# Kumar2421/scrfd_arcface_facerecognition

Hardware: AMD Instinct MI355X
Metric: faces/sec end-to-end (det+align+embed+match) (higher is better)
Workload: dtype f16; 1 GPU; BASELINE configs[1]: SCRFD-10G + ArcFace-R50, 64 synthetic 640x640 frames per GPU per step, F=1 face/frame (max_num), 1000-entry gallery, random-init weights (seed 0); frames_per_gpu=64, gallery=1000, kernel_plan=plans/mi355x.plan, rec_group=2

## Files before the change

scrfd_arcface_facerecognition_amd/csrc/conv.h:

```cpp
#pragma once
#include "common.h"

namespace fid {

enum : int { ACT_NONE = 0, ACT_RELU = 1, ACT_PRELU = 2 };
enum : int {
    CF_RES_UP2 = 1,
    CF_BORDER = 2,
    CF_OUT_F32 = 4,
    CF_ARGMAX = 8,
};

struct ConvArgs {
    const void *in;
    const void *w;
    const void *w_alt;
    const float *bias;
    const float *slope;
    const void *res;
    void *out;
    void *out2;
    float *partial;
    const void *in2;
    unsigned in2_bytes;
    int H2, W2, Cin2_p, T2, kw2, s2, nchunk2, krow;
    unsigned long long *amax;
    int amax_col0;
    int H, W, Cin_p, Ho, Wo, Cout_p, w_rows;
    int kh, kw, stride, pad;
    int M, T, nchunk, ksteps, ksplit, ksteps_per_split;
    int act, flags, nsig;
    int res_H, res_W, res_Cp;
    int tiles_m, tiles_n;
    int rev;
    int tm_fast;
    unsigned in_bytes, w_bytes;
};

struct ConvPlan {
    int bm, bn, bk, ksplit;
    int gen;
    int ns;
    size_t partial_bytes;
};
ConvPlan conv_plan(const ConvArgs &a, int num_cus, bool allow_split);
#include <vector>
std::vector<ConvPlan> conv_candidates(const ConvArgs &a, int num_cus, bool allow_split);
int conv_launch(fid_ctx *ctx, ConvArgs a, const ConvPlan &plan);
float conv_plan_cu_share(const ConvArgs &a, const ConvPlan &plan, int num_cus);
inline bool conv_walks_reverse(const ConvPlan &plan) { return plan.gen == 9; }
int plan_alt_kind(const ConvPlan &plan);
size_t repack_bytes(int kind, int Cout_p, int Cin_p, int taps = 9);
int repack_weights(fid_ctx *ctx, int kind, const void *src, void *dst, int Cout_p, int Cin_p, int taps = 9);

bool conv_direct_applicable(const ConvArgs &a);
int conv_direct_launch(fid_ctx *ctx, const ConvArgs &a);

bool conv_chunked_applicable(const ConvArgs &a);
int conv_chunked_launch(fid_ctx *ctx, const ConvArgs &a, int cb);

bool conv_pp_applicable(const ConvArgs &a);
int conv_pp_launch(fid_ctx *ctx, const ConvArgs &a, int cb);

bool conv_pc_applicable(const ConvArgs &a);
int conv_pc_launch(fid_ctx *ctx, const ConvArgs &a, int cb, int ring);

bool conv_pc2_applicable(const ConvArgs &a);
int conv_pc2_launch(fid_ctx *ctx, const ConvArgs &a);
bool conv_pcr_applicable(const ConvArgs &a);
int conv_pcr_launch(fid_ctx *ctx, const ConvArgs &a);

bool conv_wr_applicable(const ConvArgs &a);
bool conv_wr_resident_ok(const ConvArgs &a);
int conv_wr_launch(fid_ctx *ctx, const ConvArgs &a, int nt, int cb, int resident, int ring, bool strip = false);

bool mbf_block_applicable(int H, int W, int Cin_p, int Gp, int Cout_p, int stride, bool res);
int mbf_block_launch(fid_ctx *ctx, const void *x, const void *w1, const float *b1, const float *s1, int act1, const float *dww, const float *dwb,
                     const float *dws, int dw_act, const void *w2, const float *b2, const float *s2, int act2, bool res, void *out, int B, int H, int W,
                     int Cin_p, int Gp, int Cout_p, int stride);
bool conv_ks_applicable(const ConvArgs &a);
bool conv_ks_mosaic(const ConvArgs &a);
int conv_ks_launch(fid_ctx *ctx, const ConvArgs &a, int per_wg = 1, bool strip = false);
int conv_ks_items(const ConvArgs &a, bool strip = false);
bool conv_strip_ok(const ConvArgs &a);
int conv_strip_rows(const ConvArgs &a);
bool conv_ks_strip_applicable(const ConvArgs &a);

bool conv_s2_applicable(const ConvArgs &a);
int conv_s2_launch(fid_ctx *ctx, const ConvArgs &a);

bool conv_gw_applicable(const ConvArgs &a);
int conv_gw_launch(fid_ctx *ctx, const ConvArgs &a, int bm, int bn);

int conv_bb_launch(fid_ctx *ctx, const void *in, const void *w1, const float *b1, int ncls1, int act1, const float *s1, const void *w2, const float *b2,
                   void *out, int B, int H, int W, int act2, int rev, int Cp = 64);

bool dwpw_applicable(int Gp, int Cout_p);
int dwpw_launch(fid_ctx *ctx, const void *in, const float *dw_w, const float *dw_b, const float *dw_s, int dw_act, const void *pw_w, const float *pw_b,
                const float *pw_s, int pw_act, const void *res, void *out, int B, int H, int W, int Ho, int Wo, int Gp, int Cout_p, int stride);

bool stem_block_applicable(int H, int W);
int stem_block_launch(fid_ctx *ctx, const uint8_t *img, int B, int H, int W, const float *w0, const float *b0, const float *s0, int act0, const void *w1,
                      const float *b1, int ncls1, const float *s1, int act1, void *out, void *xe);

bool lat_fpn_applicable(int Cin_p, int H, int W, int rH, int rW, bool has_res);
int lat_fpn_launch(fid_ctx *ctx, const void *in, int B, int H, int W, int Cin_p, const void *w0, const float *b0, const void *res, int rH, int rW, const void *w1,
                   const float *b1, void *out, void *lat);
bool match_scan256_applicable(int n, int Gp, int dim, int num_cus);
int match_scan256_launch(fid_ctx *ctx, const void *q, const void *g, int n, int Gp, int dim, int col0, unsigned long long *amax);

int stem_fused_launch(fid_ctx *ctx, const uint8_t *img, int B, int H, int W, const void *w0, const float *b0, const void *w1,
                      const float *b1, const void *w2, const float *b2, void *out, int C2p);

int stem_rows_launch(fid_ctx *ctx, const uint8_t *img, int B, int H, int W, const void *w0, const float *b0, const void *w1,
                     const float *b1, const void *w2, const float *b2, void *out, int C2p);

}
```

scrfd_arcface_facerecognition_amd/csrc/conv_pc.hip:

```cpp
#include "epilogue.h"

namespace fid {
namespace {

typedef _Float16 half8 __attribute__((ext_vector_type(8)));
typedef float f32x4 __attribute__((ext_vector_type(4)));
typedef unsigned int u32x4 __attribute__((ext_vector_type(4)));

constexpr unsigned OOB = 0x7FFFFFF0u;
constexpr int TH = 16, TW = 16, PW = TW + 2, NPIX = (TH + 2) * PW;
constexpr int CK = 32;
constexpr int P_BLKS = 21, P_BYTES = P_BLKS * 1024;
constexpr int N_CONS = 8, N_PROD = 4;

__device__ __forceinline__ int swz64(int lin) { return (lin >> 1) & 3; }
__device__ __forceinline__ void raw_barrier() { asm volatile("s_barrier" ::: "memory"); }

struct PCArgs {
    const void *in;
    const void *w;
    const float *bias;
    const float *slope;
    const void *res;
    void *out;
    int H, W, Cin_p, Cout_p;
    int act, flags, res_Cp, nsig;
    int tiles_x, tiles_per_img, n_cblk, n_items, n_chunks;
    FastDiv d_cblk, d_tpi, d_tx;
    unsigned in_bytes, w_bytes;
    int ablate;
};

#ifdef FID_PC_STAMPS
constexpr int STAMP_STEPS = 16, STAMP_K = 6;
__device__ unsigned long long g_pc_stamps[3 * STAMP_STEPS * STAMP_K];
#define STAMP(who, k)                                                                                      \
    do {                                                                                                   \
        if (blockIdx.x == 0 && s < STAMP_STEPS && (wave <= N_CONS)) {                                                          \
            unsigned long long t_;                                                                         \
            __builtin_amdgcn_sched_barrier(0);                                                             \
            asm volatile("s_memtime %0\n\ts_waitcnt lgkmcnt(0)" : "=s"(t_)::"memory");                     \
            __builtin_amdgcn_sched_barrier(0);                                                             \
            if (lane == 0) g_pc_stamps[((who) * STAMP_STEPS + s) * STAMP_K + (k)] = t_;                     \
        }                                                                                                  \
    } while (0)
#else
#define STAMP(who, k)
#endif

template <int N>
__device__ __forceinline__ void wait_vmcnt_n() {
    asm volatile("s_waitcnt vmcnt(%0)" ::"n"(N) : "memory");
}

__device__ __forceinline__ void wait_vmcnt_dyn(int n) {
    switch (n) {
#define FID_W(k) case k: wait_vmcnt_n<k>(); break;
        FID_W(1) FID_W(2) FID_W(3) FID_W(4) FID_W(5) FID_W(6) FID_W(7) FID_W(8) FID_W(9) FID_W(10) FID_W(11) FID_W(12)
        FID_W(13) FID_W(14) FID_W(15) FID_W(16) FID_W(17) FID_W(18) FID_W(19) FID_W(20) FID_W(21) FID_W(22) FID_W(23) FID_W(24)
#undef FID_W
        default: wait_vmcnt_n<0>(); break;
    }
}

template <int NI, int WD, int PD, bool F32 = false, bool RS = false>
__global__ void __launch_bounds__((N_CONS + N_PROD) * 64, 3) conv3x3_pc(const PCArgs a) {
    constexpr int CB = 2 * NI * 16, MI = 4;
    constexpr int W_BLKS = 9 * CB * 64 / 1024, W_BYTES = W_BLKS * 1024;
    constexpr int AW = WD - 1, AP = PD - 1;
    static_assert(WD * W_BYTES + PD * P_BYTES <= 160 * 1024 && !(WD == 3 && PD == 3), "LDS budget");
    extern __shared__ __attribute__((aligned(16))) char smem[];
    char *sWr = smem, *sPr = smem + WD * W_BYTES;

    const int tid = threadIdx.x, lane = tid & 63, wave = __builtin_amdgcn_readfirstlane(tid >> 6);
    const int bid = (a.ablate & 256) ? (int)blockIdx.x : xcd_major_id(blockIdx.x, gridDim.x);
    const int my_items = bid < a.n_items ? (a.n_items - 1 - bid) / gridDim.x + 1 : 0;
    const int n_steps = my_items * a.n_chunks;
    if (n_steps == 0) return;

    auto decode_item = [&](int item, int &n, int &ty, int &tx, int &cb) {
        const int tile = fastdiv(item, a.d_cblk);
        cb = item - tile * a.n_cblk;
        n = fastdiv(tile, a.d_tpi);
        const int r = tile - n * a.tiles_per_img;
        ty = fastdiv(r, a.d_tx); tx = r - ty * a.tiles_x;
    };

    if (wave >= N_CONS) {
        const int pw = wave - N_CONS;
        __builtin_assume(pw >= 0 && pw < N_PROD);
        if (a.ablate & 512) __builtin_amdgcn_s_setprio(3);
        constexpr int MAX_W = (W_BLKS + N_PROD - 1) / N_PROD, MAX_P = (P_BLKS + N_PROD - 1) / N_PROD;
        const auto rs_in = __builtin_amdgcn_make_buffer_rsrc((void *)a.in, 0, a.in_bytes, 0x00020000);
        const auto rs_w = __builtin_amdgcn_make_buffer_rsrc((void *)a.w, 0, a.w_bytes, 0x00020000);
        int w_off[MAX_W];
#pragma unroll
        for (int k = 0; k < MAX_W; k++) {
            const int j = pw + N_PROD * k;
            const int row = j * 16 + (lane >> 2);
            const int t = row / CB, co = row - t * CB;
            w_off[k] = ((co * 9 + t) * a.Cin_p + ((lane & 3) ^ swz64(row)) * 8) * 2;
            if (a.ablate & 4) w_off[k] = j * 1024 + lane * 16;
        }
        constexpr bool KEEP_PK = NI <= 2 && !RS;
        auto patch_pk_calc = [&](int k) {
            int lo = lane;
            asm volatile("" : "+v"(lo));
            const int row = (pw + N_PROD * k) * 16 + (lo >> 2);
            int py = row / PW;
            const int px = row - py * PW;
            if (row >= NPIX) py = 255;
            return py | (px << 8) | ((((lo & 3) ^ swz64(row)) * 8) << 16);
        };
        int p_pk[KEEP_PK ? MAX_P : 1];
        if (KEEP_PK) {
#pragma unroll
            for (int k = 0; k < MAX_P; k++) p_pk[KEEP_PK ? k : 0] = patch_pk_calc(k);
        }
        auto patch_pk = [&](int k) {
            if (!KEEP_PK) return patch_pk_calc(k);
            int pk = p_pk[KEEP_PK ? k : 0];
            asm volatile("" : "+v"(pk));
            return pk;
        };
        const int my_p = (P_BLKS - pw + N_PROD - 1) / N_PROD;
        int p_off[MAX_P];
#pragma unroll
        for (int k = 0; k < (RS ? 0 : MAX_P); k++) {
            const int pk = patch_pk(k), py = pk & 255, px = (pk >> 8) & 255;
            p_off[k] = py == 255 ? -1 : ((py * a.W + px) * (a.Cin_p + ((a.ablate & 32) ? 32 : 0) + ((a.ablate & 64) ? 64 : 0)) + (pk >> 16)) * 2;
        }
        constexpr int OCPP = NI * 2, SK = OCPP, S_BLKS = N_CONS * SK, MAX_S = (S_BLKS + N_PROD - 1) / N_PROD;
        constexpr int OMASK = (OCPP & (OCPP - 1)) == 0 ? OCPP - 1 : 0;
        auto stage_pk_calc = [&](int k) {
            int lo = lane;
            asm volatile("" : "+v"(lo));
            const int b = pw + N_PROD * k, wv = b / SK;
            const int gl = (b - wv * SK) * 64 + lo;
            const int p = gl / OCPP, c = (gl - p * OCPP) ^ (p & OMASK);
            return p | (c << 8) | (wv << 16);
        };
        int s_pk[KEEP_PK ? MAX_S : 1];
        if (KEEP_PK) {
#pragma unroll
            for (int k = 0; k < MAX_S; k++) s_pk[KEEP_PK ? k : 0] = stage_pk_calc(k);
        }
        auto stage_pk = [&](int k) {
            if (!KEEP_PK) return stage_pk_calc(k);
            int pk = s_pk[KEEP_PK ? k : 0];
            asm volatile("" : "+v"(pk));
            return pk;
        };
        int s_off[MAX_S];
#pragma unroll
        for (int k = 0; k < MAX_S; k++) {
            const int pk = stage_pk(k), p = pk & 255, c = (pk >> 8) & 255, wv = pk >> 16;
            s_off[k] = ((((wv & 3) * MI + (p >> 4)) * a.W + (p & 15)) * a.Cout_p + (wv >> 2) * NI * 16 + c * 8) * 2;
        }
        u32x4 sv[MAX_S];
        auto read_tile = [&](char *slot) {
#pragma unroll
            for (int k = 0; k < MAX_S; k++)
                if (pw + N_PROD * k < S_BLKS) sv[k] = *(const u32x4 *)(slot + (pw + N_PROD * k) * 1024 + lane * 16);
            asm volatile("s_waitcnt lgkmcnt(0)" ::: "memory");
        };
        const bool has_res = a.res != nullptr;
        u32x4 rv[MAX_S];
        auto load_residual = [&](int item) {
            int n, ty, tx, cb;
            decode_item(item, n, ty, tx, cb);
            if (ty * TH + TH <= a.H && tx * TW + TW <= a.W && cb * CB + CB <= a.Cout_p) {
                const char *base = (const char *)a.res + ((((size_t)n * a.H + ty * TH) * a.W + tx * TW) * a.Cout_p + cb * CB) * 2;
#pragma unroll
                for (int k = 0; k < MAX_S; k++) rv[k] = *(const u32x4 *)(base + (unsigned)s_off[k]);
                return;
            }
#pragma unroll
            for (int k = 0; k < MAX_S; k++) {
                const int pk = stage_pk(k);
                const int p = pk & 255, c = (pk >> 8) & 255, wv = pk >> 16;
                const int oy = ty * TH + (wv & 3) * MI + (p >> 4), ox = tx * TW + (p & 15);
                const int co = cb * CB + (wv >> 2) * NI * 16 + c * 8;
                rv[k] = u32x4{0u, 0u, 0u, 0u};
                if (oy < a.H && ox < a.W && co < a.Cout_p)
                    rv[k] = *(const u32x4 *)((const char *)a.res + ((((size_t)n * a.H + oy) * a.W + ox) * a.Cout_p + co) * 2);
            }
        };
        auto write_residual = [&](char *slot) {
#pragma unroll
            for (int k = 0; k < MAX_S; k++) *(u32x4 *)(slot + (pw + N_PROD * k) * 1024 + lane * 16) = rv[k];
            asm volatile("s_waitcnt lgkmcnt(0)" ::: "memory");
        };
        static_assert(S_BLKS % N_PROD == 0, "every producer stores the same number of blocks");
        auto store_tile = [&](int item) {
            int n, ty, tx, cb;
            decode_item(item, n, ty, tx, cb);
            if (ty * TH + TH <= a.H && tx * TW + TW <= a.W && cb * CB + CB <= a.Cout_p) {
                char *base = (char *)a.out + ((((size_t)n * a.H + ty * TH) * a.W + tx * TW) * a.Cout_p + cb * CB) * 2;
#pragma unroll
                for (int k = 0; k < MAX_S; k++)
                    if (pw + N_PROD * k < S_BLKS) *(u32x4 *)(base + (unsigned)s_off[k]) = sv[k];
                return true;
            }
#pragma unroll
            for (int k = 0; k < MAX_S; k++) {
                if (pw + N_PROD * k >= S_BLKS) continue;
                const int pk = stage_pk(k);
                const int p = pk & 255, c = (pk >> 8) & 255, wv = pk >> 16;
                const int oy = ty * TH + (wv & 3) * MI + (p >> 4), ox = tx * TW + (p & 15);
                const int co = cb * CB + (wv >> 2) * NI * 16 + c * 8;
                if (oy < a.H && ox < a.W && co < a.Cout_p)
                    *(u32x4 *)((char *)a.out + ((((size_t)n * a.H + oy) * a.W + ox) * a.Cout_p + co) * 2) = sv[k];
            }
            return false;
        };
        struct Cursor {
            int item, ck;
            int w_base;
            int n, y0, x0;
        };
        auto cursor_decode = [&](Cursor &c) {
            int n, ty, tx, cb;
            decode_item(c.item, n, ty, tx, cb);
            c.w_base = cb * CB * 9 * a.Cin_p * 2;
            c.n = (a.ablate & 8) ? 0 : n; c.y0 = ty * TH - 1; c.x0 = tx * TW - 1;
        };
        auto cursor_next = [&](Cursor &c) {
            if (++c.ck == a.n_chunks) {
                c.ck = 0;
                c.item += gridDim.x;
                cursor_decode(c);
            }
        };
        auto issue_weights = [&](const Cursor &c, int slot) {
            if (a.ablate & 1) return;
            const int ubase = (a.ablate & 4) ? c.ck * W_BYTES : c.w_base + c.ck * CK * 2;
            char *dst = sWr + slot * W_BYTES;
#pragma unroll
            for (int k = 0; k < MAX_W; k++) {
                const int j = pw + N_PROD * k;
                if (j < W_BLKS)
                    __builtin_amdgcn_raw_ptr_buffer_load_lds(rs_w, (__attribute__((address_space(3))) void *)(dst + j * 1024), 16,
                                                             (unsigned)(w_off[k] + ubase), 0, 0, 0);
            }
        };
        auto issue_patch = [&](const Cursor &c, int slot) {
            if (a.ablate & 2) return;
            const int c0 = c.ck * CK;
            char *dst = sPr + slot * P_BYTES;
            if ((a.ablate & 16) || (c.y0 >= 0 && c.x0 >= 0 && c.y0 + TH + 2 <= a.H && c.x0 + TW + 2 <= a.W)) {
                const int base = (((c.n * a.H + c.y0) * a.W + c.x0) * a.Cin_p + c0) * 2;
#pragma unroll
                for (int k = 0; k < MAX_P; k++) {
                    const int j = pw + N_PROD * k;
                    if (j >= P_BLKS) continue;
                    const unsigned vo = p_off[k] < 0 ? OOB : (unsigned)(p_off[k] + base);
                    __builtin_amdgcn_raw_ptr_buffer_load_lds(rs_in, (__attribute__((address_space(3))) void *)(dst + j * 1024), 16, vo, 0, 0, 0);
                }
                return;
            }
#pragma unroll
            for (int k = 0; k < MAX_P; k++) {
                const int j = pw + N_PROD * k;
                if (j >= P_BLKS) continue;
                const int pk = patch_pk(k);
                const int py = pk & 255, iy = c.y0 + py, ix = c.x0 + ((pk >> 8) & 255);
                const bool in = py != 255 && (unsigned)iy < (unsigned)a.H && (unsigned)ix < (unsigned)a.W;
                const unsigned vo = in ? (unsigned)((((c.n * a.H + iy) * a.W + ix) * a.Cin_p + c0 + (pk >> 16)) * 2) : OOB;
                __builtin_amdgcn_raw_ptr_buffer_load_lds(rs_in, (__attribute__((address_space(3))) void *)(dst + j * 1024), 16, vo, 0, 0, 0);
            }
        };

        u32x4 wreg[RS ? MAX_W : 1], preg[RS ? MAX_P : 1];
        auto load_weights = [&](const Cursor &c) {
            if (a.ablate & 1) return;
            const int ubase = c.w_base + c.ck * CK * 2;
#pragma unroll
            for (int k = 0; k < MAX_W; k++)
                if (pw + N_PROD * k < W_BLKS) wreg[RS ? k : 0] = __builtin_amdgcn_raw_buffer_load_b128(rs_w, (unsigned)(w_off[k] + ubase), 0, 0);
        };
        auto load_patch = [&](const Cursor &c) {
            if (a.ablate & 2) return;
            const int c0 = c.ck * CK;
            if (c.y0 >= 0 && c.x0 >= 0 && c.y0 + TH + 2 <= a.H && c.x0 + TW + 2 <= a.W) {
                const int base = (((c.n * a.H + c.y0) * a.W + c.x0) * a.Cin_p + c0) * 2;
#pragma unroll
                for (int k = 0; k < MAX_P; k++) {
                    if (pw + N_PROD * k >= P_BLKS) continue;
                    const int pk = patch_pk(k), py = pk & 255;
                    const unsigned vo = py == 255 ? OOB : (unsigned)(((py * a.W + ((pk >> 8) & 255)) * a.Cin_p + (pk >> 16)) * 2 + base);
                    preg[RS ? k : 0] = __builtin_amdgcn_raw_buffer_load_b128(rs_in, vo, 0, 0);
                }
                return;
            }
#pragma unroll
            for (int k = 0; k < MAX_P; k++) {
                if (pw + N_PROD * k >= P_BLKS) continue;
                const int pk = patch_pk(k);
                const int py = pk & 255, iy = c.y0 + py, ix = c.x0 + ((pk >> 8) & 255);
                const bool in = py != 255 && (unsigned)iy < (unsigned)a.H && (unsigned)ix < (unsigned)a.W;
                const unsigned vo = in ? (unsigned)((((c.n * a.H + iy) * a.W + ix) * a.Cin_p + c0 + (pk >> 16)) * 2) : OOB;
                preg[RS ? k : 0] = __builtin_amdgcn_raw_buffer_load_b128(rs_in, vo, 0, 0);
            }
        };
        auto commit_weights = [&](int slot) {
            char *dst = sWr + slot * W_BYTES + lane * 16;
#pragma unroll
            for (int k = 0; k < MAX_W; k++)
                if (pw + N_PROD * k < W_BLKS) *(u32x4 *)(dst + (pw + N_PROD * k) * 1024) = wreg[RS ? k : 0];
        };
        auto commit_patch = [&](int slot) {
            char *dst = sPr + slot * P_BYTES + lane * 16;
#pragma unroll
            for (int k = 0; k < MAX_P; k++)
                if (pw + N_PROD * k < P_BLKS) *(u32x4 *)(dst + (pw + N_PROD * k) * 1024) = preg[RS ? k : 0];
        };
        auto lds_done = [&]() { asm volatile("s_waitcnt lgkmcnt(0)" ::: "memory"); };

        const int my_w = (W_BLKS - pw + N_PROD - 1) / N_PROD;
        Cursor cw, cp;
        cw.item = bid; cw.ck = 0;
        cursor_decode(cw);
        cp = cw;
        if constexpr (RS) {
            auto fetch = [&](bool w, int wslot, bool p_, int pslot) {
                if (p_) { load_patch(cp); cursor_next(cp); }
                if (w) { load_weights(cw); cursor_next(cw); }
                if (w) commit_weights(wslot);
                if (p_) commit_patch(pslot);
            };
            fetch(true, 0, true, 0);
            if (n_steps > 1) fetch(AW == 2, 1, AP == 2, 1);
            lds_done();
            int ck = 0, item = bid;
            for (int s = 0; s < n_steps; s++) {
                STAMP(0, 0);
                STAMP(0, 1);
                raw_barrier();
                STAMP(0, 2);
                if (!F32 && ck == 0 && s > 0) {
                    char *stage = sWr + ((s + WD - 1) % WD) * W_BYTES;
                    if (has_res) {
                        write_residual(stage);
                        raw_barrier();
                    }
                    raw_barrier();
                    read_tile(stage);
                    store_tile(item - gridDim.x);
                }
                STAMP(0, 3);
                fetch(s + AW < n_steps, (s + AW) % WD, s + AP < n_steps, (s + AP) % PD);
                if (has_res && ck == a.n_chunks - 1) load_residual(item);
                lds_done();
                STAMP(0, 4);
                if (++ck == a.n_chunks) { ck = 0; item += gridDim.x; }
            }
            if (F32) return;
            raw_barrier();
            if (has_res) {
                write_residual(sWr + ((n_steps - 1) % WD) * W_BYTES);
                raw_barrier();
            }
            raw_barrier();
            read_tile(sWr + ((n_steps - 1) % WD) * W_BYTES);
            store_tile(item - gridDim.x);
            return;
        }
        issue_weights(cw, 0);
        issue_patch(cp, 0);
        cursor_next(cw);
        cursor_next(cp);
        int young = 0;
        if (n_steps > 1) {
            if (AP == 2) { issue_patch(cp, 1); cursor_next(cp); young = my_p; }
            if (AW == 2) { issue_weights(cw, 1); cursor_next(cw); young = my_w; }
        }
        int ck = 0, item = bid;
        for (int s = 0; s < n_steps; s++) {
            STAMP(0, 0);
            wait_vmcnt_dyn(young);
            STAMP(0, 1);
            raw_barrier();
            STAMP(0, 2);
            const bool flush = !F32 && ck == 0 && s > 0;
            const bool have_w = s + AW < n_steps, have_p = s + AP < n_steps;
            char *stage = sWr + ((s + WD - 1) % WD) * W_BYTES;
            young = 0;
            if (flush) {
                if (has_res) {
                    write_residual(stage);
                    raw_barrier();
                }
                if (have_p) issue_patch(cp, (s + AP) % PD);
                raw_barrier();
                read_tile(stage);
                if (have_w) issue_weights(cw, (s + AW) % WD);
                const bool all_stores = store_tile(item - gridDim.x);
                if (all_stores) young = MAX_S + ((AW == 2 && have_w) ? my_w : 0);
            } else {
                if (AW == 2) {
                    if (have_p) issue_patch(cp, (s + AP) % PD);
                    if (have_w) { issue_weights(cw, (s + AW) % WD); young = my_w; }
                } else {
                    if (have_w) issue_weights(cw, (s + AW) % WD);
                    if (have_p) { issue_patch(cp, (s + AP) % PD); young = AP == 2 ? my_p : 0; }
                }
            }
            if (has_res && ck == a.n_chunks - 1) {
                load_residual(item);
                young = 0;
            }
            STAMP(0, 3);
            if (have_w && s + AW + 1 < n_steps) cursor_next(cw);
            if (have_p && s + AP + 1 < n_steps) cursor_next(cp);
            STAMP(0, 4);
            if (++ck == a.n_chunks) { ck = 0; item += gridDim.x; }
        }
        if (F32) return;
        raw_barrier();
        if (has_res) {
            wait_vmcnt_n<0>();
            write_residual(sWr + ((n_steps - 1) % WD) * W_BYTES);
            raw_barrier();
        }
        raw_barrier();
        read_tile(sWr + ((n_steps - 1) % WD) * W_BYTES);
        store_tile(item - gridDim.x);
        return;
    }

    const int grp = wave >> 2, wg = wave & 3;
    const int frow = lane & 15, fq = lane >> 4;
    const int lin0 = (wg * MI) * PW + frow;
    EpiArgs ep{a.bias, a.slope, a.res, a.out, a.Cout_p, a.H, a.W, a.act, a.flags, 0, a.H, a.W, a.res_Cp};

    constexpr int OROWB = NI * 32, OCPP = NI * 2;
    constexpr int OMASK = (OCPP & (OCPP - 1)) == 0 ? OCPP - 1 : 0;
    static_assert(F32 || N_CONS * 64 * OROWB <= W_BYTES, "staging must fit a weight slot");
    EpiPix px[MI];
    int co0[NI];
    EpiRegs<NI, MI> R;
    ep_half4 hv[NI][MI];
    int bias_cb = -1;
    auto epi_prefetch = [&](int item) {
        int n, ty, tx, cb;
        decode_item(item, n, ty, tx, cb);
        int lo = lane;
        asm volatile("" : "+v"(lo));
        const int frow = lo & 15, fq = lo >> 4;
        const int co_w = cb * CB + grp * NI * 16;
        if (a.flags & CF_BORDER) {
#pragma unroll
            for (int mi = 0; mi < MI; mi++) {
                const int oy = ty * TH + wg * MI + mi, ox = tx * TW + frow;
                px[mi].valid = oy < a.H && ox < a.W;
                px[mi].n = n; px[mi].oy = oy; px[mi].ox = ox;
                px[mi].m = px[mi].valid ? ((long long)n * a.H + oy) * a.W + ox : 0;
            }
        }
#pragma unroll
        for (int ni = 0; ni < NI; ni++) co0[ni] = co_w + ni * 16 + fq * 4;
        if (cb != bias_cb) {
            bias_cb = cb;
#pragma unroll
            for (int ni = 0; ni < NI; ni++) {
                const int c = co0[ni] < a.Cout_p ? co0[ni] : 0;
                R.bb[ni] = (a.bias != nullptr && !(a.flags & CF_BORDER)) ? *(const ep_f32x4 *)(a.bias + c) : ep_f32x4{0.f, 0.f, 0.f, 0.f};
                if (a.act == ACT_PRELU) R.sl[ni] = *(const ep_f32x4 *)(a.slope + c);
            }
        }
    };
    f32x4 acc[NI][MI];
    const bool has_res = a.res != nullptr;
    auto epi_residual_values = [&](char *slot) {
        int lo = lane;
        asm volatile("" : "+v"(lo));
        const int frow = lo & 15, fq = lo >> 4;
        const char *sS = slot + wave * (64 * OROWB);
#pragma unroll
        for (int mi = 0; mi < MI; mi++)
#pragma unroll
            for (int ni = 0; ni < NI; ni++) {
                const int p = mi * 16 + frow, c = ni * 2 + (fq >> 1);
                R.rr[ni][mi] = *(const ep_half4 *)(sS + p * OROWB + ((c ^ (p & OMASK)) << 4) + (fq & 1) * 8);
            }
        epilogue_values_fast<NI, MI>(ep, acc, px, co0, R, hv);
    };
    auto epi_stage = [&](char *slot) {
        int lo = lane;
        asm volatile("" : "+v"(lo));
        const int frow = lo & 15, fq = lo >> 4;
        char *sS = slot + wave * (64 * OROWB);
#pragma unroll
        for (int mi = 0; mi < MI; mi++)
#pragma unroll
            for (int ni = 0; ni < NI; ni++) {
                const int p = mi * 16 + frow, c = ni * 2 + (fq >> 1);
                *(ep_half4 *)(sS + p * OROWB + ((c ^ (p & OMASK)) << 4) + (fq & 1) * 8) = hv[ni][mi];
            }
        asm volatile("s_waitcnt lgkmcnt(0)" ::: "memory");
    };

    int li = 0, ck = 0;
    for (int s = 0; s < n_steps; s++) {
        const int item = bid + li * gridDim.x;
        [[maybe_unused]] const int who = wave == 0 ? 1 : 2;
        if (wave == 0 || wave == 7) STAMP(who, 0);
        raw_barrier();
        if (wave == 0 || wave == 7) STAMP(who, 1);
        if (!F32 && ck == 0 && s > 0) {
            char *slot = sWr + ((s + WD - 1) % WD) * W_BYTES;
            if (has_res) {
                raw_barrier();
                epi_residual_values(slot);
            }
            epi_stage(slot);
            raw_barrier();
        }
        if (wave == 0 || wave == 7) STAMP(who, 2);
        const bool last_chunk = ck == a.n_chunks - 1;
        if (last_chunk && !F32) epi_prefetch(item);
        if (wave == 0 || wave == 7) STAMP(who, 3);
        if (ck == 0) {
#pragma unroll
            for (int ni = 0; ni < NI; ni++)
#pragma unroll
                for (int mi = 0; mi < MI; mi++) acc[ni][mi] = f32x4{0.f, 0.f, 0.f, 0.f};
        }
        const char *sW = sWr + (s % WD) * W_BYTES, *sP = sPr + (s % PD) * P_BYTES;
        {
            int plin = lin0, wlane = ((grp * NI) * 16 + frow) * 64 + ((fq ^ swz64(frow)) << 4);
            asm volatile("" : "+v"(plin), "+v"(wlane));
            half8 wq[3][NI], pq[3];
            auto load_w = [&](int dy, int dx) {
#pragma unroll
                for (int ni = 0; ni < NI; ni++) wq[dy][ni] = *(const half8 *)(sW + wlane + ((dy * 3 + dx) * CB + ni * 16) * 64);
            };
            auto load_p = [&](int q, int set) {
                const int lin = plin + (q % 6) * PW + q / 6;
                pq[set] = *(const half8 *)(sP + lin * 64 + ((fq ^ swz64(lin)) << 4));
            };
            load_w(0, 0); load_p(0, 0); load_w(1, 0); load_p(1, 1); load_w(2, 0);
#pragma unroll
            for (int q = 0; q < 18; q++) {
                const int dx = q / 6, r = q % 6;
                if (q + 2 < 18) load_p(q + 2, (q + 2) % 3);
                __builtin_amdgcn_sched_barrier(0);
#pragma unroll
                for (int dy = 0; dy < 3; dy++) {
                    const int mi = r - dy;
                    if (mi < 0 || mi >= MI) continue;
#pragma unroll
                    for (int ni = 0; ni < NI; ni++)
                        acc[ni][mi] = __builtin_amdgcn_mfma_f32_16x16x32_f16(wq[dy][ni], pq[q % 3], acc[ni][mi], 0, 0, 0);
                }
                __builtin_amdgcn_sched_barrier(0);
                if (dx < 2 && r >= 3) load_w(r - 3, dx + 1);
            }
        }
        if (wave == 0 || wave == 7) STAMP(who, 4);
        if (F32) {
            if (last_chunk) {
                int n, ty, tx, cb;
                decode_item(item, n, ty, tx, cb);
                int lo = lane;
                asm volatile("" : "+v"(lo));
                const int frow = lo & 15, fq = lo >> 4;
#pragma unroll
                for (int ni = 0; ni < NI; ni++) {
                    const int co = cb * CB + (grp * NI + ni) * 16 + fq * 4;
                    const f32x4 b = (a.bias != nullptr && co < a.Cout_p) ? *(const f32x4 *)(a.bias + co) : f32x4{0.f, 0.f, 0.f, 0.f};
#pragma unroll
                    for (int mi = 0; mi < MI; mi++) {
                        f32x4 v = acc[ni][mi] + b;
                        if (co < a.nsig) {
#pragma unroll
                            for (int i = 0; i < 4; i++)
                                if (co + i < a.nsig) v[i] = 1.f / (1.f + expf(-v[i]));
                        }
                        const int oy = ty * TH + wg * MI + mi, ox = tx * TW + frow;
                        if (oy < a.H && ox < a.W && co < a.Cout_p)
                            *(f32x4 *)((float *)a.out + (((size_t)n * a.H + oy) * a.W + ox) * a.Cout_p + co) = v;
                    }
                }
            }
        } else if (last_chunk && !has_res) epilogue_values_fast<NI, MI>(ep, acc, px, co0, R, hv);
        if (wave == 0 || wave == 7) STAMP(who, 5);
        if (++ck == a.n_chunks) { ck = 0; li++; }
    }
    if (F32) return;
    raw_barrier();
    if (has_res) {
        raw_barrier();
        epi_residual_values(sWr + ((n_steps - 1) % WD) * W_BYTES);
    }
    epi_stage(sWr + ((n_steps - 1) % WD) * W_BYTES);
    raw_barrier();
}

template <int NI, int WD, int PD, bool F32 = false, bool RS = false>
int launch_pc(fid_ctx *ctx, const PCArgs &a) {
    constexpr size_t lds = (size_t)WD * 9 * 2 * NI * 16 * 64 + (size_t)PD * P_BYTES;
    FID_TRY(ensure_dyn_lds(ctx, (const void *)conv3x3_pc<NI, WD, PD, F32, RS>, (int)((int)lds)));
    const int grid = std::min(a.n_items, ctx->num_cus);
    hipLaunchKernelGGL((conv3x3_pc<NI, WD, PD, F32, RS>), dim3(grid), dim3((N_CONS + N_PROD) * 64), lds, ctx->stream, a);
    FID_HIP(hipGetLastError());
#ifdef FID_PC_STAMPS
    if (const char *e = getenv("FID_PC_STAMP_DUMP")) {
        static int countdown = atoi(e);
        if (--countdown == 0) {
            FID_HIP(hipStreamSynchronize(ctx->stream));
            static unsigned long long h[3 * STAMP_STEPS * STAMP_K];
            FID_HIP(hipMemcpyFromSymbol(h, HIP_SYMBOL(g_pc_stamps), sizeof(h)));
            const int steps = std::min(STAMP_STEPS, ((a.n_items - 1) / grid + 1) * a.n_chunks);
            fprintf(stderr, "[pc-stamps] NI=%d H=%d W=%d Cin_p=%d Cout_p=%d items=%d chunks=%d\n", NI, a.H, a.W, a.Cin_p, a.Cout_p, a.n_items, a.n_chunks);
            const unsigned long long t0 = h[0];
            for (int s = 0; s < steps; s++) {
                const unsigned long long *p = h + s * STAMP_K, *c0 = h + (STAMP_STEPS + s) * STAMP_K, *c7 = h + (2 * STAMP_STEPS + s) * STAMP_K;
                fprintf(stderr, "[pc-stamps] step %2d | producer: +%6lld wait %5lld barrier %5lld issue %5lld next %4lld | cons0: arrive +%6lld barrier %5lld flush %5lld pref %5lld mfma %5lld values %5lld | cons7: arrive +%6lld barrier %5lld mfma %5lld\n",
                        s, (long long)(p[0] - t0), (long long)(p[1] - p[0]), (long long)(p[2] - p[1]), (long long)(p[3] - p[2]), (long long)(p[4] - p[3]),
                        (long long)(c0[0] - t0), (long long)(c0[1] - c0[0]), (long long)(c0[2] - c0[1]), (long long)(c0[3] - c0[2]), (long long)(c0[4] - c0[3]), (long long)(c0[5] - c0[4]),
                        (long long)(c7[0] - t0), (long long)(c7[1] - c7[0]), (long long)(c7[4] - c7[3]));
            }
        }
    }
#endif
    return FID_OK;
}

}

bool conv_pc_applicable(const ConvArgs &a) {
    if (getenv("FID_NO_PC")) return false;
    const bool shape = a.kh == 3 && a.kw == 3 && a.stride == 1 && a.pad == 1 && a.Cin_p % 32 == 0 && a.Cin_p >= 64 &&
                       a.w_rows == a.Cout_p && a.H == a.Ho && a.W == a.Wo && a.H >= 12 && a.W >= 12 && !(a.flags & (CF_RES_UP2 | CF_ARGMAX));
    if (!shape) return false;
    if (a.flags & CF_OUT_F32)
        return a.Cout_p == 32 && a.act == ACT_NONE && a.res == nullptr && !(a.flags & CF_BORDER);
    return a.Cout_p >= 64 && a.nsig == 0 && (a.res == nullptr || (a.res_H == a.Ho && a.res_W == a.Wo));
}

int conv_pc_launch(fid_ctx *ctx, const ConvArgs &c, int cb, int ring) {
    PCArgs a{};
    a.in = c.in; a.w = c.w; a.bias = c.bias; a.slope = c.slope; a.res = c.res; a.out = c.out;
    a.H = c.H; a.W = c.W; a.Cin_p = c.Cin_p; a.Cout_p = c.Cout_p;
    a.act = c.act; a.flags = c.flags; a.res_Cp = c.res_Cp; a.nsig = c.nsig;
    const int B = c.M / (c.Ho * c.Wo);
    a.tiles_x = cdiv(c.W, TW);
    a.tiles_per_img = a.tiles_x * cdiv(c.H, TH);
    a.n_cblk = cdiv(c.Cout_p, cb);
    a.n_items = B * a.tiles_per_img * a.n_cblk;
    a.n_chunks = c.Cin_p / CK;
    a.d_cblk = fastdiv_make(a.n_cblk); a.d_tpi = fastdiv_make(a.tiles_per_img); a.d_tx = fastdiv_make(a.tiles_x);
    a.in_bytes = c.in_bytes;
    a.w_bytes = (unsigned)std::min<size_t>(c.w_bytes, (size_t)c.w_rows * 9 * c.Cin_p * 2);
    if (const char *e = getenv("FID_PC_ABLATE")) a.ablate = atoi(e);
    FID_REQUIRE(a.in_bytes <= OOB && a.w_bytes <= OOB, "conv: tensor larger than 2 GiB");
    const bool dma = getenv("FID_PC_RS") == nullptr;
    if (cb == 32) return dma ? launch_pc<1, 2, 3, true>(ctx, a) : launch_pc<1, 2, 3, true, true>(ctx, a);
    if (cb == 64 && ring == 1) return launch_pc<2, 3, 2>(ctx, a);
    if (cb == 64) return dma ? launch_pc<2, 2, 3>(ctx, a) : launch_pc<2, 2, 3, false, true>(ctx, a);
    if (cb == 96) return launch_pc<3, 2, 2>(ctx, a);
    set_error("producer/consumer conv: cb=%d unsupported", cb);
    return FID_E_INVALID;
}

}
```

scrfd_arcface_facerecognition_amd/csrc/net.h:

```cpp
#pragma once
#include "conv.h"

namespace fid {

enum : int { OP_STEM = 1, OP_CONV = 2, OP_MAXPOOL = 3, OP_DWCONV = 4, OP_STEMFUSED = 5, OP_BBLOCK = 6, OP_DWPW = 7, OP_MBBLOCK = 8, OP_STEMBLOCK = 9, OP_LATFPN = 10 };

enum : int {
    W_TYPE = 0,
    W_SRC = 1,
    W_DST = 2,
    W_RES = 3,
    W_KH = 4,
    W_KW = 5,
    W_STRIDE = 6,
    W_PAD = 7,
    W_CIN = 8,
    W_COUT = 9,
    W_ACT = 10,
    W_FLAGS = 11,
    W_NSIG = 12,
    W_WOFF = 13,
    W_WBYTES = 14,
    W_BOFF = 15,
    W_SOFF = 16,
    W_WROWS = 17,
    W_GROUPS = 18,
    W_F_W0 = 20, W_F_B0 = 21, W_F_W1 = 22, W_F_B1 = 23, W_F_W2 = 24, W_F_B2 = 25,
    W_F_MACS_LO = 26, W_F_MACS_HI = 27,
    W_B_W1 = 20, W_B_B1 = 21, W_B_W2 = 22, W_B_B2 = 23, W_B_S1 = 24, W_B_ACT1 = 25,
    W_D_WOFF = 20, W_D_BOFF = 21, W_D_SOFF = 22, W_D_ACT = 23,
    W_M_W1 = 20, W_M_B1 = 21, W_M_S1 = 22, W_M_ACT1 = 23, W_M_DW = 24, W_M_DWB = 25, W_M_DWS = 28, W_M_DWACT = 29, W_M_GP = 30,
    W_S_W1 = 20, W_S_B1 = 21, W_S_S1 = 22, W_S_ACT0 = 23, W_S_DST2 = 24,
    W_L_W0 = 20, W_L_B0 = 21, W_L_LAT = 22,
    W_X_DST2 = 20, W_X_ACT2 = 21, W_X_COUT1P = 22,
    W_X_SRC2 = 23, W_X_T2 = 24, W_X_KW2 = 25, W_X_S2 = 28,
    W_X_W2OFF = 29, W_X_B2OFF = 30, W_X_SCOP = 31,
};

enum : int { T_C = 0, T_CP = 1, T_H = 2, T_W = 3, T_DTYPE = 4, T_SLOT = 5, T_FLAGS = 6 };

}
```

scrfd_arcface_facerecognition_amd/csrc/net.hip:

```cpp
#include "net.h"

#include <map>
#include <set>

struct fid_net {
    int n_ops = 0, n_tensors = 0, in_h = 0, in_w = 0, max_batch = 0;
    std::vector<int32_t> ops, tensors;
    void *blob = nullptr;
    size_t blob_bytes = 0;
    std::vector<void *> slots;
    std::vector<size_t> slot_bytes_per_image;
    double macs_per_image = 0;
    int sub_batch = 0;
    std::vector<std::map<int, fid::ConvPlan>> tuned;
    std::vector<char> tdir;
    int alternate = 1;
    std::vector<std::set<int>> plan_ok;
    int autotune = 1;
    bool tuned_now = false;
    size_t partial_cap = 0;
    hipEvent_t *prof_events = nullptr;
    int n_prof_events = 0;
    struct Replay { hipGraphExec_t exec = nullptr; int seen = 0; unsigned long long last_use = 0; const void *partial = nullptr; };
    std::map<std::pair<const void *, int>, Replay> replays;
    unsigned long long run_counter = 0;
    int graphs = 0;
    unsigned long long table_hash = 0;
    std::string device_key, plan_path;
    std::map<std::pair<int, int>, void *> alt_w;
};

namespace fid {
namespace {

typedef _Float16 half8 __attribute__((ext_vector_type(8)));

template <int CPW, int SPLIT = 4>
__global__ void __launch_bounds__(256) stem_conv3x3(const uint8_t *__restrict__ img, const float *__restrict__ w,
                                                    const float *__restrict__ bias, const float *__restrict__ slope,
                                                    _Float16 *__restrict__ out, int H, int W, int Ho, int Wo, int Cout_p,
                                                    int stride, int act, long long total_pix) {
    const int wv = __builtin_amdgcn_readfirstlane(threadIdx.x >> 6);
    const long long pix = ((long long)blockIdx.x * (4 / SPLIT) + wv / SPLIT) * 64 + (threadIdx.x & 63);
    const int cg = wv % SPLIT;
    if (pix >= total_pix) return;
    const int hw = Ho * Wo;
    const int n = (int)(pix / hw);
    const int r = (int)(pix - (long long)n * hw);
    const int oy = r / Wo, ox = r - oy * Wo;
    const int iy0 = oy * stride - 1, ix0 = ox * stride - 1;
    float x[27];
    const uint8_t *base = img + (size_t)n * H * W * 3;
#pragma unroll
    for (int dy = 0; dy < 3; dy++) {
#pragma unroll
        for (int dx = 0; dx < 3; dx++) {
            const int iy = iy0 + dy, ix = ix0 + dx;
            const bool in = (unsigned)iy < (unsigned)H && (unsigned)ix < (unsigned)W;
            const uint8_t *p = base + ((size_t)(in ? iy : 0) * W + (in ? ix : 0)) * 3;
#pragma unroll
            for (int c = 0; c < 3; c++) x[(dy * 3 + dx) * 3 + c] = in ? (float)(2 * (int)p[c] - 255) : 0.f;
        }
    }
    _Float16 res[CPW];
#pragma unroll
    for (int c = 0; c < CPW; c++) {
        const int co = cg * CPW + c;
        const float *wr = w + co * 27;
        float acc = bias[co];
#pragma unroll
        for (int k = 0; k < 27; k++) acc = fmaf(x[k], wr[k], acc);
        if (act == ACT_RELU) acc = fmaxf(acc, 0.f);
        else if (act == ACT_PRELU) acc = acc > 0.f ? acc : acc * slope[co];
        res[c] = (_Float16)acc;
    }
    _Float16 *o = out + (size_t)pix * Cout_p + cg * CPW;
#pragma unroll
    for (int c = 0; c < CPW; c += 8) *(half8 *)(o + c) = *(half8 *)(res + c);
}

typedef _Float16 sm_half8 __attribute__((ext_vector_type(8)));
typedef _Float16 sm_half4 __attribute__((ext_vector_type(4)));
typedef float sm_f32x4 __attribute__((ext_vector_type(4)));
typedef unsigned int sm_u32x4 __attribute__((ext_vector_type(4)));

template <int NI, int STRIDE>
__global__ void __launch_bounds__(256) stem_conv_mfma(const uint8_t *__restrict__ img, const float *__restrict__ w,
                                                      const float *__restrict__ bias, const float *__restrict__ slope,
                                                      _Float16 *__restrict__ out, int H, int W, int Ho, int Wo, int act,
                                                      int tiles_x, int tiles_y, int n_tiles, int ablate) {
    constexpr int CP = NI * 16, TS = 16;
    constexpr int PR = (TS - 1) * STRIDE + 3;
    constexpr int ND = (PR * 3 + 1 + 3) / 4;
    constexpr int RSH = ND * 4;
    constexpr int OROWB = CP * 2, CPP = OROWB / 16;
    __shared__ __attribute__((aligned(16))) _Float16 sIn[PR * RSH + 8];
    __shared__ __attribute__((aligned(16))) _Float16 sWt[CP * 32];
    __shared__ __attribute__((aligned(16))) char sSt[4 * 4 * TS * OROWB];
    const int tid = threadIdx.x, lane = tid & 63, wave = __builtin_amdgcn_readfirstlane(tid >> 6);
    const int frow = lane & 15, fq = lane >> 4;

    for (int i = tid; i < CP * 32; i += 256) {
        const int co = i >> 5, k = i & 31;
        sWt[i] = k < 27 ? (_Float16)w[co * 27 + k] : (_Float16)0.f;
    }
    if (tid < 8) sIn[PR * RSH + tid] = (_Float16)0.f;
    __syncthreads();
    sm_half8 wf[NI];
    sm_f32x4 bv[NI], sl[NI];
#pragma unroll
    for (int ni = 0; ni < NI; ni++) {
        wf[ni] = *(const sm_half8 *)(sWt + (ni * 16 + frow) * 32 + fq * 8);
        bv[ni] = bias ? *(const sm_f32x4 *)(bias + ni * 16 + fq * 4) : sm_f32x4{0.f, 0.f, 0.f, 0.f};
        sl[ni] = act == ACT_PRELU ? *(const sm_f32x4 *)(slope + ni * 16 + fq * 4) : sm_f32x4{1.f, 1.f, 1.f, 1.f};
    }
    int koff[8];
#pragma unroll
    for (int j = 0; j < 8; j++) {
        const int k = fq * 8 + j, dy = k / 9, rem = k - dy * 9;
        koff[j] = k < 27 ? dy * RSH + rem : -1;
    }
    const int tiles_per_img = tiles_x * tiles_y, rowbytes = W * 3;
    for (int tile = blockIdx.x; tile < n_tiles; tile += gridDim.x) {
        const int n = tile / tiles_per_img, r = tile - n * tiles_per_img;
        const int ty = r / tiles_x, tx = r - ty * tiles_x;
        const int iy0 = ty * TS * STRIDE - 1, ix0 = tx * TS * STRIDE - 1;
        const int bx0 = ix0 * 3 - 1;
        const uint8_t *base = img + (size_t)n * H * rowbytes;
        const int elo = 1 + 3 * max(0, -ix0), ehi = 1 + 3 * min(PR, W - ix0);
        for (int d = tid; d < PR * ND; d += 256) {
            const int pr = d / ND, dc = d - pr * ND;
            const int iy = iy0 + pr, bx = bx0 + dc * 4;
            const bool rin = (unsigned)iy < (unsigned)H;
            unsigned v4 = 0u;
            if (rin && bx >= 0 && bx + 4 <= rowbytes && !(ablate & 2)) v4 = *(const unsigned *)(base + (size_t)iy * rowbytes + bx);
            sm_half4 h;
#pragma unroll
            for (int j = 0; j < 4; j++) {
                const int e = dc * 4 + j, v = (v4 >> (8 * j)) & 0xFF;
                h[j] = (rin && e >= elo && e < ehi) ? (_Float16)(float)(2 * v - 255) : (_Float16)0.f;
            }
            *(sm_half4 *)(sIn + pr * RSH + dc * 4) = h;
        }
        __syncthreads();
        char *sS = sSt + wave * (4 * TS * OROWB);
        sm_half8 pf[4];
#pragma unroll
        for (int rr = 0; rr < 4; rr++) {
            const int pbase = ((wave * 4 + rr) * STRIDE) * RSH + 1 + frow * STRIDE * 3;
#pragma unroll
            for (int j = 0; j < 8; j++) pf[rr][j] = sIn[koff[j] >= 0 ? pbase + koff[j] : PR * RSH];
        }
#pragma unroll
        for (int rr = 0; rr < 4; rr++) {
#pragma unroll
            for (int ni = 0; ni < NI; ni++) {
                sm_f32x4 acc = {0.f, 0.f, 0.f, 0.f};
                acc = __builtin_amdgcn_mfma_f32_16x16x32_f16(wf[ni], pf[rr], acc, 0, 0, 0);
                sm_f32x4 v = acc + bv[ni];
                if (act == ACT_RELU) {
#pragma unroll
                    for (int i = 0; i < 4; i++) v[i] = fmaxf(v[i], 0.f);
                } else if (act == ACT_PRELU) {
#pragma unroll
                    for (int i = 0; i < 4; i++) v[i] = v[i] > 0.f ? v[i] : v[i] * sl[ni][i];
                }
                const int ch = ni * 2 + (fq >> 1);
                *(sm_half4 *)(sS + (rr * TS + frow) * OROWB + (((ch + frow) % CPP) << 4) + (fq & 1) * 8) = __builtin_convertvector(v, sm_half4);
            }
        }
        asm volatile("s_waitcnt lgkmcnt(0)" ::: "memory");
#pragma unroll
        for (int g = lane; g < 4 * TS * CPP; g += 64) {
            const int p = g / CPP, c = g - p * CPP;
            const sm_u32x4 o = *(const sm_u32x4 *)(sS + p * OROWB + (((c + (p & 15)) % CPP) << 4));
            const int oy = ty * TS + wave * 4 + (p >> 4), ox = tx * TS + (p & 15);
            if (oy < Ho && ox < Wo && !(ablate & 1)) *(sm_u32x4 *)((char *)out + (((size_t)n * Ho + oy) * Wo + ox) * OROWB + c * 16) = o;
        }
        __syncthreads();
    }
}

__global__ void __launch_bounds__(256) maxpool_nhwc(const _Float16 *__restrict__ in, _Float16 *__restrict__ out, int H, int W,
                                                    int Ho, int Wo, int Cp, int k, int stride, int pad, long long total) {
    const long long idx = (long long)blockIdx.x * blockDim.x + threadIdx.x;
    if (idx >= total) return;
    const int c8 = Cp >> 3;
    const int cg = (int)(idx % c8);
    const long long pix = idx / c8;
    const int hw = Ho * Wo;
    const int n = (int)(pix / hw);
    const int r = (int)(pix - (long long)n * hw);
    const int oy = r / Wo, ox = r - oy * Wo;
    half8 m;
#pragma unroll
    for (int i = 0; i < 8; i++) m[i] = (_Float16)(-65504.f);
    for (int dy = 0; dy < k; dy++) {
        const int iy = oy * stride - pad + dy;
        if ((unsigned)iy >= (unsigned)H) continue;
        for (int dx = 0; dx < k; dx++) {
            const int ix = ox * stride - pad + dx;
            if ((unsigned)ix >= (unsigned)W) continue;
            const half8 v = *(const half8 *)(in + ((size_t)(n * H + iy) * W + ix) * Cp + cg * 8);
#pragma unroll
            for (int i = 0; i < 8; i++) m[i] = v[i] > m[i] ? v[i] : m[i];
        }
    }
    *(half8 *)(out + (size_t)pix * Cp + cg * 8) = m;
}

__global__ void __launch_bounds__(256) dwconv_nhwc(const _Float16 *__restrict__ in, const float *__restrict__ w,
                                                   const float *__restrict__ bias, const float *__restrict__ slope,
                                                   _Float16 *__restrict__ out, int H, int W, int Ho, int Wo, int Cp, int k,
                                                   int stride, int pad, int act, long long total) {
    const long long idx = (long long)blockIdx.x * blockDim.x + threadIdx.x;
    if (idx >= total) return;
    const int c8 = Cp >> 3;
    const int cg = (int)(idx % c8);
    const long long pix = idx / c8;
    const int hw = Ho * Wo;
    const int n = (int)(pix / hw);
    const int r = (int)(pix - (long long)n * hw);
    const int oy = r / Wo, ox = r - oy * Wo;
    float acc[8];
#pragma unroll
    for (int i = 0; i < 8; i++) acc[i] = bias[cg * 8 + i];
    for (int dy = 0; dy < k; dy++) {
        const int iy = oy * stride - pad + dy;
        if ((unsigned)iy >= (unsigned)H) continue;
        for (int dx = 0; dx < k; dx++) {
            const int ix = ox * stride - pad + dx;
            if ((unsigned)ix >= (unsigned)W) continue;
            const half8 v = *(const half8 *)(in + ((size_t)(n * H + iy) * W + ix) * Cp + cg * 8);
            const float *wr = w + (size_t)(dy * k + dx) * Cp + cg * 8;
#pragma unroll
            for (int i = 0; i < 8; i++) acc[i] = fmaf((float)v[i], wr[i], acc[i]);
        }
    }
    half8 o;
#pragma unroll
    for (int i = 0; i < 8; i++) {
        float a = acc[i];
        if (act == ACT_RELU) a = fmaxf(a, 0.f);
        else if (act == ACT_PRELU) a = a > 0.f ? a : a * slope[cg * 8 + i];
        o[i] = (_Float16)a;
    }
    *(half8 *)(out + (size_t)pix * Cp + cg * 8) = o;
}

constexpr int DW_TR = 14, DW_TC = 16, DW_PR = DW_TR + 2, DW_PC = DW_TC + 2;
__global__ void __launch_bounds__(256) dwconv3x3_lds(const _Float16 *__restrict__ in, const float *__restrict__ w, const float *__restrict__ bias,
                                                     const float *__restrict__ slope, _Float16 *__restrict__ out, int H, int W, int Cp, int act,
                                                     int tiles_x, int tiles_y, int cblks) {
    __shared__ __attribute__((aligned(16))) char sP[DW_PR * DW_PC * 128];
    const int tid = threadIdx.x;
    int item = blockIdx.x;
    const int cb = item % cblks; item /= cblks;
    const int tx = item % tiles_x; item /= tiles_x;
    const int ty = item % tiles_y, n = item / tiles_y;
    const int y0 = ty * DW_TR - 1, x0 = tx * DW_TC - 1, c0 = cb * 64;
    for (int i = tid; i < DW_PR * DW_PC * 8; i += 256) {
        const int p = i >> 3, c = i & 7;
        const int py = p / DW_PC, px = p - py * DW_PC;
        const int iy = y0 + py, ix = x0 + px;
        if ((unsigned)iy < (unsigned)H && (unsigned)ix < (unsigned)W)
            *(uint4 *)(sP + p * 128 + c * 16) = *(const uint4 *)(in + ((size_t)(n * H + iy) * W + ix) * Cp + c0 + c * 8);
    }
    const int cg = tid & 7, col = (tid >> 3) & 15, rh = tid >> 7;
    float wv[9][8], bv[8], sv[8];
#pragma unroll
    for (int t = 0; t < 9; t++)
#pragma unroll
        for (int i = 0; i < 8; i++) wv[t][i] = w[(size_t)t * Cp + c0 + cg * 8 + i];
#pragma unroll
    for (int i = 0; i < 8; i++) {
        bv[i] = bias[c0 + cg * 8 + i];
        sv[i] = act == ACT_PRELU ? slope[c0 + cg * 8 + i] : 1.f;
    }
    __syncthreads();
    const int ox = tx * DW_TC + col;
    const bool okc[3] = {(unsigned)(ox - 1) < (unsigned)W, ox < W, (unsigned)(ox + 1) < (unsigned)W};
    if (ox >= W) return;
    half8 win[3][3];
    const char *base = sP + col * 128 + cg * 16;
    auto load_row = [&](int pr, int slot) {
#pragma unroll
        for (int dx = 0; dx < 3; dx++) win[slot][dx] = *(const half8 *)(base + (pr * DW_PC + dx) * 128);
    };
    const int r0 = rh * (DW_TR / 2);
    load_row(r0, 0); load_row(r0 + 1, 1);
#pragma unroll
    for (int r = 0; r < DW_TR / 2; r++) {
        load_row(r0 + r + 2, (r + 2) % 3);
        const int oy = ty * DW_TR + r0 + r;
        if (oy >= H) break;
        float acc[8];
#pragma unroll
        for (int i = 0; i < 8; i++) acc[i] = bv[i];
#pragma unroll
        for (int dy = 0; dy < 3; dy++) {
            if ((unsigned)(oy - 1 + dy) >= (unsigned)H) continue;
#pragma unroll
            for (int dx = 0; dx < 3; dx++) {
                if (!okc[dx]) continue;
                const half8 v = win[(r + dy) % 3][dx];
#pragma unroll
                for (int i = 0; i < 8; i++) acc[i] = fmaf((float)v[i], wv[dy * 3 + dx][i], acc[i]);
            }
        }
        half8 o;
#pragma unroll
        for (int i = 0; i < 8; i++) {
            float a = acc[i];
            if (act == ACT_RELU) a = fmaxf(a, 0.f);
            else if (act == ACT_PRELU) a = a > 0.f ? a : a * sv[i];
            o[i] = (_Float16)a;
        }
        *(half8 *)(out + ((size_t)(n * H + oy) * W + ox) * Cp + c0 + cg * 8) = o;
    }
}

__global__ void __launch_bounds__(256) gdc_rows(const _Float16 *__restrict__ in, const float *__restrict__ w, const float *__restrict__ bias,
                                                const float *__restrict__ slope, _Float16 *__restrict__ out, int k, int Cp, int act, int total) {
    const int idx = blockIdx.x * blockDim.x + threadIdx.x;
    const int g = idx >> 3, r = idx & 7;
    const int c8 = Cp >> 3;
    const bool live = g < total;
    const int n = live ? g / c8 : 0, cg = live ? g - n * c8 : 0;
    float acc[8];
#pragma unroll
    for (int i = 0; i < 8; i++) acc[i] = 0.f;
    if (live && r < k) {
        for (int dx = 0; dx < k; dx++) {
            const half8 v = *(const half8 *)(in + ((size_t)(n * k + r) * k + dx) * Cp + cg * 8);
            const float *wr = w + (size_t)(r * k + dx) * Cp + cg * 8;
#pragma unroll
            for (int i = 0; i < 8; i++) acc[i] = fmaf((float)v[i], wr[i], acc[i]);
        }
    }
    float sum[8];
#pragma unroll
    for (int i = 0; i < 8; i++) sum[i] = live ? bias[cg * 8 + i] : 0.f;
    for (int rr = 0; rr < k; rr++)
#pragma unroll
        for (int i = 0; i < 8; i++) sum[i] += __shfl(acc[i], (threadIdx.x & 63 & ~7) + rr, 64);
    if (live && r == 0) {
        half8 o;
#pragma unroll
        for (int i = 0; i < 8; i++) {
            float a = sum[i];
            if (act == ACT_RELU) a = fmaxf(a, 0.f);
            else if (act == ACT_PRELU) a = a > 0.f ? a : a * slope[cg * 8 + i];
            o[i] = (_Float16)a;
        }
        *(half8 *)(out + (size_t)n * Cp + cg * 8) = o;
    }
}

__global__ void __launch_bounds__(256) touch_kernel(const uint4 *__restrict__ p, size_t n16, unsigned *sink) {
    unsigned acc = 0;
    for (size_t i = (size_t)blockIdx.x * 256 + threadIdx.x; i < n16; i += (size_t)gridDim.x * 256) {
        const uint4 v = p[i];
        acc ^= v.x ^ v.y ^ v.z ^ v.w;
    }
    if (acc == 0x9E3779B9u && sink) *sink = acc;
}

struct TensorView {
    void *ptr;
    int C, Cp, H, W, dtype;
};

TensorView view(const fid_net *net, int id, int first = 0) {
    const int32_t *t = &net->tensors[(size_t)id * FID_TENSOR_WORDS];
    const size_t per_image = (size_t)t[T_H] * t[T_W] * t[T_CP] * (t[T_DTYPE] == 1 ? 4 : 2);
    return TensorView{(char *)net->slots[t[T_SLOT]] + per_image * first, t[T_C], t[T_CP], t[T_H], t[T_W], t[T_DTYPE]};
}

constexpr int FID_PLAN_REV = 5;

unsigned long long fnv1a(const void *p, size_t n, unsigned long long h = 1469598103934665603ull) {
    const unsigned char *b = (const unsigned char *)p;
    for (size_t i = 0; i < n; i++) { h ^= b[i]; h *= 1099511628211ull; }
    return h;
}

void plan_line(const fid_net *net, int oi, int batch, const ConvPlan &c, char *buf, size_t cap) {
    snprintf(buf, cap, "%s|%016llx|%d|%d|%d %d %d %d %d %d %zu\n", net->device_key.c_str(), net->table_hash, oi, batch, c.gen, c.bm, c.bn,
             c.bk, c.ksplit, c.ns, c.partial_bytes);
}

int plan_load(fid_net *net, const char *path, int *n_loaded) {
    FILE *f = fopen(path, "r");
    int n = 0;
    if (f) {
        char line[512];
        while (fgets(line, sizeof(line), f)) {
            char dev[256];
            unsigned long long h = 0;
            int oi = 0, batch = 0;
            ConvPlan c{};
            if (sscanf(line, "%255[^|]|%llx|%d|%d|%d %d %d %d %d %d %zu", dev, &h, &oi, &batch, &c.gen, &c.bm, &c.bn, &c.bk, &c.ksplit, &c.ns,
                       &c.partial_bytes) != 11)
                continue;
            if (h != net->table_hash || net->device_key != dev || oi < 0 || oi >= net->n_ops || batch <= 0) continue;
            net->tuned[oi][batch] = c;
            net->plan_ok[oi].erase(batch);
            n++;
        }
        fclose(f);
    }
    if (n_loaded) *n_loaded = n;
    return FID_OK;
}

bool same_kernel(const ConvPlan &x, const ConvPlan &y) {
    return x.gen == y.gen && x.bm == y.bm && x.bn == y.bn && x.bk == y.bk && x.ksplit == y.ksplit && x.ns == y.ns;
}

void drop_unused_alt_weights(fid_ctx *ctx, fid_net *net, int oi) {
    bool used[4] = {false, false, false, false};
    for (const auto &kv : net->tuned[oi]) used[plan_alt_kind(kv.second) & 3] = true;
    bool synced = false;
    for (auto it = net->alt_w.begin(); it != net->alt_w.end();) {
        if (it->first.first == oi && !used[it->first.second & 3]) {
            if (!synced) { (void)hipStreamSynchronize(ctx->stream); synced = true; }
            (void)hipFree(it->second);
            it = net->alt_w.erase(it);
        } else ++it;
    }
}

int set_alt_weights(fid_ctx *ctx, fid_net *net, int oi, ConvArgs &a, const ConvPlan &plan) {
    const int kind = plan_alt_kind(plan);
    a.w_alt = nullptr;
    if (kind == 0) return FID_OK;
    auto key = std::make_pair(oi, kind);
    auto it = net->alt_w.find(key);
    if (it == net->alt_w.end()) {
        void *p = nullptr;
        FID_HIP(hipMalloc(&p, repack_bytes(kind, a.w_rows, a.Cin_p, a.kh * a.kw) + 256));
        const int rc = repack_weights(ctx, kind, a.w, p, a.w_rows, a.Cin_p, a.kh * a.kw);
        if (rc != FID_OK) { (void)hipFree(p); return rc; }
        it = net->alt_w.emplace(key, p).first;
    }
    a.w_alt = it->second;
    return FID_OK;
}

int run_op(fid_ctx *ctx, fid_net *net, int oi, const uint8_t *images, int first, int batch, void *partial_ws) {
    const int32_t *op = &net->ops[(size_t)oi * FID_OP_WORDS];
    const char *blob = (const char *)net->blob;
    static const bool klog = getenv("FID_KLOG") != nullptr;
    if (klog) fprintf(stderr, "[klog] op %d\n", oi);
    const TensorView dst = view(net, op[W_DST], first);
    images += (size_t)first * net->in_h * net->in_w * 3;
    const float *bias = op[W_BOFF] >= 0 ? (const float *)(blob + op[W_BOFF]) : nullptr;
    const float *slope = op[W_SOFF] >= 0 ? (const float *)(blob + op[W_SOFF]) : nullptr;
    if (op[W_TYPE] != OP_CONV && op[W_TYPE] != OP_BBLOCK) net->tdir[op[W_DST]] = 0;
    switch (op[W_TYPE]) {
        case OP_STEM: {
            const long long total = (long long)batch * dst.H * dst.W;
            const int cpw = dst.Cp / 4;
            const float *w = (const float *)(blob + op[W_WOFF]);
            dim3 grid((unsigned)cdiv64(total, 64));
            static const bool valu = getenv("FID_STEM_VALU") != nullptr;
            const int st = op[W_STRIDE];
            if (!valu && net->in_w % 4 == 0 && (st == 1 || st == 2) && (dst.Cp == 16 || dst.Cp == 32 || dst.Cp == 64 || dst.Cp == 128)) {
                const int tx = cdiv(dst.W, 16), ty = cdiv(dst.H, 16), nt = batch * tx * ty;
                static const int abl = getenv("FID_STEMM_ABLATE") ? atoi(getenv("FID_STEMM_ABLATE")) : 0;
                const int g = std::min(nt, ctx->num_cus * (dst.Cp == 128 ? 2 : (dst.Cp == 64 ? 3 : 4)));
#define STEMM(NI, ST) hipLaunchKernelGGL((stem_conv_mfma<NI, ST>), dim3(g), dim3(256), 0, ctx->stream, images, w, bias, slope, (_Float16 *)dst.ptr, net->in_h, net->in_w, dst.H, dst.W, op[W_ACT], tx, ty, nt, abl)
                if (dst.Cp == 128) { if (st == 1) STEMM(8, 1); else STEMM(8, 2); }
                else if (dst.Cp == 64) { if (st == 1) STEMM(4, 1); else STEMM(4, 2); }
                else if (dst.Cp == 32) { if (st == 1) STEMM(2, 1); else STEMM(2, 2); }
                else { if (st == 1) STEMM(1, 1); else STEMM(1, 2); }
#undef STEMM
                break;
            }
            static const int split = getenv("FID_STEM_SPLIT") ? atoi(getenv("FID_STEM_SPLIT")) : 2;
#define STEM(CPW) hipLaunchKernelGGL(stem_conv3x3<CPW>, grid, dim3(256), 0, ctx->stream, images, w, bias, slope, (_Float16 *)dst.ptr, net->in_h, net->in_w, dst.H, dst.W, dst.Cp, op[W_STRIDE], op[W_ACT], total)
#define STEMS(CPW, SP) hipLaunchKernelGGL((stem_conv3x3<CPW, SP>), dim3((unsigned)cdiv64(total, 64 * (4 / SP))), dim3(256), 0, ctx->stream, images, w, bias, slope, (_Float16 *)dst.ptr, net->in_h, net->in_w, dst.H, dst.W, dst.Cp, op[W_STRIDE], op[W_ACT], total)
            if (split == 1 && dst.Cp == 64) STEMS(64, 1);
            else if (split == 2 && dst.Cp == 64) STEMS(32, 2);
            else if (split == 1 && dst.Cp == 32) STEMS(32, 1);
            else if (cpw == 8) STEM(8);
            else if (cpw == 16) STEM(16);
            else if (cpw == 32) STEM(32);
            else { set_error("stem: Cout_p=%d unsupported", dst.Cp); return FID_E_INVALID; }
#undef STEM
#undef STEMS
            break;
        }
        case OP_CONV: {
            if (op[W_X_SRC2] == 0 && op[W_X_W2OFF] > 0) {
                const int cons = op[W_X_W2OFF] - 1;
                auto itc = net->tuned[cons].find(batch);
                if (itc != net->tuned[cons].end() && itc->second.gen == 12 && net->plan_ok[cons].count(batch)) break;
            }
            const TensorView src = view(net, op[W_SRC], first);
            ConvArgs a{}, af{};
            bool has_sc = false;
            a.in = src.ptr;
            a.w = blob + op[W_WOFF];
            a.bias = bias;
            a.slope = slope;
            a.out = dst.ptr;
            if (op[W_X_DST2] > 0) {
                const TensorView d2 = view(net, op[W_X_DST2] - 1, first);
                FID_REQUIRE(d2.H == dst.H && d2.W == dst.W && d2.Cp == dst.Cp && d2.dtype == dst.dtype && op[W_X_ACT2] == ACT_NONE &&
                            op[W_X_COUT1P] == dst.Cp, "op %d: bad fused shortcut record", oi);
                a.out2 = d2.ptr;
            }
            a.H = src.H; a.W = src.W; a.Cin_p = src.Cp;
            a.Ho = dst.H; a.Wo = dst.W; a.Cout_p = dst.Cp;
            a.w_rows = op[W_WROWS];
            a.kh = op[W_KH]; a.kw = op[W_KW]; a.stride = op[W_STRIDE]; a.pad = op[W_PAD];
            a.M = batch * dst.H * dst.W;
            a.act = op[W_ACT]; a.flags = op[W_FLAGS]; a.nsig = op[W_NSIG];
            if (dst.dtype == 1) a.flags |= CF_OUT_F32;
            if (op[W_RES] >= 0) {
                const TensorView r = view(net, op[W_RES], first);
                a.res = r.ptr; a.res_H = r.H; a.res_W = r.W; a.res_Cp = r.Cp;
            }
            a.in_bytes = (unsigned)((size_t)batch * src.H * src.W * src.Cp * 2);
            a.w_bytes = (unsigned)op[W_WBYTES];
            if (op[W_X_SRC2] > 0) {
                const TensorView x2 = view(net, op[W_X_SRC2] - 1, first);
                FID_REQUIRE(x2.dtype == 0 && op[W_X_T2] >= 1 && op[W_X_KW2] >= 1 && op[W_X_S2] >= 1 && op[W_X_DST2] == 0 &&
                            (dst.H - 1) * op[W_X_S2] + (op[W_X_T2] / op[W_X_KW2] - 1) < x2.H && (dst.W - 1) * op[W_X_S2] + op[W_X_KW2] - 1 < x2.W,
                            "op %d: bad fused shortcut-conv record", oi);
                FID_REQUIRE(op[W_X_W2OFF] > 0 && op[W_X_B2OFF] > 0 && op[W_X_SCOP] > 0 && op[W_X_SCOP] <= oi && op[W_RES] >= 0, "op %d: fused shortcut-conv record without its second image", oi);
                af = a;
                af.in2 = x2.ptr; af.H2 = x2.H; af.W2 = x2.W; af.Cin2_p = x2.Cp; af.T2 = op[W_X_T2]; af.kw2 = op[W_X_KW2]; af.s2 = op[W_X_S2];
                af.in2_bytes = (unsigned)((size_t)batch * x2.H * x2.W * x2.Cp * 2);
                af.w = blob + op[W_X_W2OFF];
                af.bias = (const float *)(blob + op[W_X_B2OFF]);
                af.w_bytes = (unsigned)((size_t)op[W_WROWS] * (op[W_KH] * op[W_KW] * src.Cp + op[W_X_T2] * x2.Cp) * 2);
                af.res = nullptr;
                has_sc = true;
            }
            a.partial = af.partial = (float *)partial_ws;
            a.rev = af.rev = net->alternate && op[W_SRC] >= 0 && !net->tdir[op[W_SRC]];
            auto all_candidates = [&]() {
                std::vector<ConvPlan> v = conv_candidates(a, ctx->num_cus, true);
                static const bool no_sc = getenv("FID_NO_SC_RUNTIME") != nullptr;
                if (has_sc && !no_sc)
                    for (ConvPlan c : conv_candidates(af, ctx->num_cus, true)) { c.gen = 12; v.push_back(c); }
                return v;
            };
            auto launch_plan = [&](const ConvPlan &c) -> int {
                if (c.gen != 12) return conv_launch(ctx, a, c);
                ConvPlan c2 = c;
                c2.gen = c.ns == 10 ? 10 : 2;
                af.w_alt = a.w_alt;
                return conv_launch(ctx, af, c2);
            };
            ConvPlan plan;
            auto &cache = net->tuned[oi];
            auto it = cache.find(batch);
            if (it != cache.end() && !net->plan_ok[oi].count(batch)) {
                bool ok = false;
                for (const ConvPlan &c : all_candidates())
                    if (same_kernel(c, it->second) && c.partial_bytes <= net->partial_cap && (c.ksplit == 1 || partial_ws)) { it->second = c; ok = true; break; }
                if (!ok && it->second.ksplit == 1) {
                    const ConvPlan h = conv_plan(a, ctx->num_cus, false);
                    if (same_kernel(h, it->second)) { it->second = h; ok = true; }
                }
                if (ok) net->plan_ok[oi].insert(batch);
                else { cache.erase(it); it = cache.end(); }
            }
            if (it != cache.end()) {
                plan = it->second;
            } else if (net->autotune && partial_ws) {
                std::vector<ConvPlan> cands = all_candidates();
                if (const char *fg = getenv("FID_FORCE_GEN")) {
                    std::vector<ConvPlan> only;
                    for (const ConvPlan &c : cands)
                        if (c.gen == atoi(fg)) only.push_back(c);
                    if (!only.empty()) cands = only;
                }
                if (const char *fn = getenv("FID_FORCE_NS")) {
                    std::vector<ConvPlan> only;
                    for (const ConvPlan &c : cands)
                        if (((c.gen == 2 || c.gen == 5 || c.gen == 12) && c.ns == atoi(fn)) || (c.gen == 9 && (c.ns == 1 ? 3 : (c.ns == 4 ? 4 : (c.ns == 6 ? (c.bm == 512 ? 7 : 6) : (c.ns >= 7 ? c.ns + 1 + (c.ns == 8 && c.bm == 512 ? 20 : 0) + (c.ns == 8 && c.bm == 256 && c.bn == 128 ? 30 : 0) : c.bm / 256)))) == atoi(fn))) only.push_back(c);
                    if (!only.empty()) cands = only;
                }
                const float pc2_bias = getenv("FID_PC2_BIAS") ? (float)atof(getenv("FID_PC2_BIAS")) : 1.f;
                hipEvent_t e0, e1;
                FID_HIP(hipEventCreate(&e0));
                FID_HIP(hipEventCreate(&e1));
                static const bool cold_tune = !getenv("FID_TUNE_HOT");
                void *flush = nullptr;
                constexpr size_t FLUSH_BYTES = 320ull << 20;
                if (cold_tune) { FID_TRY(get_scratch(ctx, 4, FLUSH_BYTES, &flush)); net->tuned_now = true; }
                float best = 1e30f;
                if (cands.empty()) { set_error("op %d: no kernel candidate", oi); return FID_E_STATE; }
                plan = cands[0];
                float t_sc = 0.f;
                if (has_sc) {
                    t_sc = 1e30f;
                    for (int rep = 0; rep < 4; rep++) {
                        if (flush) {
                            FID_HIP(hipMemsetAsync(flush, rep & 1, FLUSH_BYTES, ctx->stream));
                            if (af.in2_bytes <= (128u << 20))
                                hipLaunchKernelGGL(touch_kernel, dim3(ctx->num_cus * 4), dim3(256), 0, ctx->stream, (const uint4 *)af.in2, (size_t)af.in2_bytes / 16, (unsigned *)nullptr);
                        }
                        FID_HIP(hipEventRecord(e0, ctx->stream));
                        FID_TRY(run_op(ctx, net, op[W_X_SCOP] - 1, images - (size_t)first * net->in_h * net->in_w * 3, first, batch, partial_ws));
                        FID_HIP(hipEventRecord(e1, ctx->stream));
                        FID_HIP(hipEventSynchronize(e1));
                        float ms = 0;
                        FID_HIP(hipEventElapsedTime(&ms, e0, e1));
                        if (rep > 0 || !flush) t_sc = std::min(t_sc, ms);
                    }
                }
                for (const ConvPlan &c : cands) {
                    if (c.partial_bytes > net->partial_cap) continue;
                    float tmin = 1e30f;
                    static const int tune_reps = getenv("FID_TUNE_REPS") ? std::max(2, atoi(getenv("FID_TUNE_REPS"))) : 5;
                    for (int rep = 0; rep < tune_reps; rep++) {
                        FID_TRY(set_alt_weights(ctx, net, oi, a, c));
                        if (flush) {
                            FID_HIP(hipMemsetAsync(flush, rep & 1, FLUSH_BYTES, ctx->stream));
                            if (a.in_bytes <= (128u << 20))
                                hipLaunchKernelGGL(touch_kernel, dim3(ctx->num_cus * 4), dim3(256), 0, ctx->stream, (const uint4 *)a.in, (size_t)a.in_bytes / 16, (unsigned *)nullptr);
                        }
                        FID_HIP(hipEventRecord(e0, ctx->stream));
                        FID_TRY(launch_plan(c));
                        FID_HIP(hipEventRecord(e1, ctx->stream));
                        FID_HIP(hipEventSynchronize(e1));
                        float ms = 0;
                        FID_HIP(hipEventElapsedTime(&ms, e0, e1));
                        if (rep > 0) tmin = std::min(tmin, ms);
                    }
                    float score = c.ksplit > 1 ? tmin * 1.1f : tmin;
                    if (has_sc && c.gen != 12) score += t_sc;
                    static const float tune_share = getenv("FID_TUNE_SHARE") ? (float)atof(getenv("FID_TUNE_SHARE")) : 0.f;
                    if (tune_share > 0.f) score *= 1.f - tune_share * (1.f - conv_plan_cu_share(a, c, ctx->num_cus));
                    if (c.gen == 8) score *= pc2_bias;
                    static const int tune_verbose = getenv("FID_TUNE_LOG") ? atoi(getenv("FID_TUNE_LOG")) : 0;
                    if (tune_verbose >= 2)
                        fprintf(stderr, "[cand] op %d gen %d tile %dx%dx%d ns %d split %d: %.1f us\n", oi, c.gen, c.bm, c.bn, c.bk, c.ns, c.ksplit, tmin * 1e3f);
                    if (score < best) { best = score; plan = c; }
                }
                (void)hipEventDestroy(e0);
                (void)hipEventDestroy(e1);
                cache[batch] = plan;
                net->plan_ok[oi].insert(batch);
                drop_unused_alt_weights(ctx, net, oi);
                if (!net->plan_path.empty()) {
                    if (FILE *pf = fopen(net->plan_path.c_str(), "a")) {
                        char line[512];
                        plan_line(net, oi, batch, plan, line, sizeof(line));
                        fputs(line, pf);
                        fclose(pf);
                    }
                }
                if (getenv("FID_TUNE_LOG"))
                    fprintf(stderr, "[tune] op %d M=%d Cin_p=%d Cout_p=%d k=%d s=%d -> gen %d tile %dx%dx%d ns %d split %d (%.1f us)\n", oi, a.M,
                            a.Cin_p, a.Cout_p, a.kh, a.stride, plan.gen, plan.bm, plan.bn, plan.bk, plan.ns, plan.ksplit, best * 1e3f);
            } else {
                plan = conv_direct_applicable(a) ? ConvPlan{} : conv_plan(a, ctx->num_cus, partial_ws != nullptr);
                if (conv_direct_applicable(a)) { plan.gen = 0; plan.ksplit = 1; }
            }
            FID_TRY(set_alt_weights(ctx, net, oi, a, plan));
            FID_TRY(launch_plan(plan));
            net->tdir[op[W_DST]] = (char)(a.rev && conv_walks_reverse(plan));
            if (op[W_X_DST2] > 0) net->tdir[op[W_X_DST2] - 1] = net->tdir[op[W_DST]];
            break;
        }
        case OP_STEMFUSED: {
            const bool old_stem = getenv("FID_STEM_OLD") != nullptr;
            FID_TRY((old_stem ? stem_fused_launch : stem_rows_launch)(ctx, images, batch, net->in_h, net->in_w, blob + op[W_F_W0], (const float *)(blob + op[W_F_B0]),
                                      blob + op[W_F_W1], (const float *)(blob + op[W_F_B1]), blob + op[W_F_W2],
                                      (const float *)(blob + op[W_F_B2]), dst.ptr, dst.Cp));
            break;
        }
        case OP_STEMBLOCK: {
            FID_REQUIRE(dst.Cp == 64 && dst.dtype == 0 && dst.H == net->in_h && dst.W == net->in_w && stem_block_applicable(dst.H, dst.W), "op %d: bad fused stem-block record", oi);
            void *xe = nullptr;
            if (op[W_S_DST2] > 0) {
                const TensorView d2 = view(net, op[W_S_DST2] - 1, first);
                FID_REQUIRE(d2.Cp == 64 && d2.dtype == 0 && d2.H == (dst.H + 1) / 2 && d2.W == (dst.W + 1) / 2, "op %d: second output of the fused stem block", oi);
                xe = d2.ptr;
            }
            FID_TRY(stem_block_launch(ctx, images, batch, dst.H, dst.W, (const float *)(blob + op[W_WOFF]), bias, slope, op[W_S_ACT0], blob + op[W_S_W1],
                                      (const float *)(blob + op[W_S_B1]), (op[W_FLAGS] & CF_BORDER) ? 9 : 1,
                                      op[W_S_S1] >= 0 ? (const float *)(blob + op[W_S_S1]) : nullptr, op[W_ACT], dst.ptr, xe));
            break;
        }
        case OP_LATFPN: {
            const TensorView src = view(net, op[W_SRC], first);
            const void *res = nullptr;
            int rH = 0, rW = 0;
            if (op[W_RES] >= 0) {
                const TensorView r = view(net, op[W_RES], first);
                FID_REQUIRE(r.Cp == 64 && r.dtype == 0, "op %d: coarser lateral", oi);
                res = r.ptr; rH = r.H; rW = r.W;
            }
            FID_REQUIRE(src.dtype == 0 && dst.dtype == 0 && dst.Cp == 64 && src.H == dst.H && src.W == dst.W && lat_fpn_applicable(src.Cp, src.H, src.W, rH, rW, res != nullptr),
                        "op %d: bad fused lateral + fpn record", oi);
            void *lat = nullptr;
            if (op[W_L_LAT] > 0) {
                const TensorView l = view(net, op[W_L_LAT] - 1, first);
                FID_REQUIRE(l.Cp == 64 && l.dtype == 0 && l.H == dst.H && l.W == dst.W, "op %d: lateral output of the fused lateral + fpn op", oi);
                lat = l.ptr;
            }
            FID_TRY(lat_fpn_launch(ctx, src.ptr, batch, src.H, src.W, src.Cp, blob + op[W_L_W0], (const float *)(blob + op[W_L_B0]), res, rH, rW, blob + op[W_WOFF], bias, dst.ptr, lat));
            break;
        }
        case OP_BBLOCK: {
            const TensorView src = view(net, op[W_SRC], first);
            FID_REQUIRE((src.Cp == 64 || src.Cp == 32) && dst.Cp == src.Cp && src.H == dst.H && src.W == dst.W && src.dtype == 0 && dst.dtype == 0, "op %d: bad fused block record", oi);
            const int rev = net->alternate && !net->tdir[op[W_SRC]];
            FID_TRY(conv_bb_launch(ctx, src.ptr, blob + op[W_B_W1], (const float *)(blob + op[W_B_B1]), (op[W_FLAGS] & CF_BORDER) ? 9 : 1, op[W_B_ACT1],
                                   op[W_B_S1] >= 0 ? (const float *)(blob + op[W_B_S1]) : nullptr, blob + op[W_B_W2], (const float *)(blob + op[W_B_B2]), dst.ptr,
                                   batch, dst.H, dst.W, op[W_ACT], rev, src.Cp));
            net->tdir[op[W_DST]] = (char)rev;
            break;
        }
        case OP_DWPW: {
            const TensorView src = view(net, op[W_SRC], first);
            const void *res = nullptr;
            if (op[W_RES] >= 0) {
                const TensorView r = view(net, op[W_RES], first);
                FID_REQUIRE(r.H == dst.H && r.W == dst.W && r.Cp == dst.Cp && r.dtype == 0, "op %d: residual shape", oi);
                res = r.ptr;
            }
            FID_REQUIRE(src.dtype == 0 && dst.dtype == 0 && op[W_D_WOFF] >= 0 && op[W_D_BOFF] >= 0 && op[W_WOFF] >= 0, "op %d: bad depthwise + pointwise record", oi);
            FID_TRY(dwpw_launch(ctx, src.ptr, (const float *)(blob + op[W_D_WOFF]), (const float *)(blob + op[W_D_BOFF]),
                                op[W_D_SOFF] >= 0 ? (const float *)(blob + op[W_D_SOFF]) : nullptr, op[W_D_ACT], blob + op[W_WOFF], bias, slope, op[W_ACT], res,
                                dst.ptr, batch, src.H, src.W, dst.H, dst.W, src.Cp, dst.Cp, op[W_STRIDE]));
            break;
        }
        case OP_MBBLOCK: {
            const TensorView src = view(net, op[W_SRC], first);
            FID_REQUIRE(src.dtype == 0 && dst.dtype == 0 && op[W_M_W1] >= 0 && op[W_M_B1] >= 0 && op[W_M_DW] >= 0 && op[W_M_DWB] >= 0 && op[W_WOFF] >= 0 &&
                        op[W_M_GP] > 0 && (op[W_RES] < 0 || op[W_RES] == op[W_SRC]), "op %d: bad bottleneck record", oi);
            FID_REQUIRE(dst.H == (src.H - 1) / op[W_STRIDE] + 1 && dst.W == (src.W - 1) / op[W_STRIDE] + 1, "op %d: bottleneck output shape", oi);
            FID_TRY(mbf_block_launch(ctx, src.ptr, blob + op[W_M_W1], (const float *)(blob + op[W_M_B1]),
                                     op[W_M_S1] >= 0 ? (const float *)(blob + op[W_M_S1]) : nullptr, op[W_M_ACT1], (const float *)(blob + op[W_M_DW]),
                                     (const float *)(blob + op[W_M_DWB]), op[W_M_DWS] >= 0 ? (const float *)(blob + op[W_M_DWS]) : nullptr, op[W_M_DWACT],
                                     blob + op[W_WOFF], bias, slope, op[W_ACT], op[W_RES] >= 0, dst.ptr, batch, src.H, src.W, src.Cp, op[W_M_GP], dst.Cp,
                                     op[W_STRIDE]));
            break;
        }
        case OP_MAXPOOL: {
            const TensorView src = view(net, op[W_SRC], first);
            const long long total = (long long)batch * dst.H * dst.W * (dst.Cp / 8);
            hipLaunchKernelGGL(maxpool_nhwc, dim3((unsigned)cdiv64(total, 256)), dim3(256), 0, ctx->stream, (const _Float16 *)src.ptr,
                               (_Float16 *)dst.ptr, src.H, src.W, dst.H, dst.W, dst.Cp, op[W_KH], op[W_STRIDE], op[W_PAD], total);
            break;
        }
        case OP_DWCONV: {
            const TensorView src = view(net, op[W_SRC], first);
            const long long total = (long long)batch * dst.H * dst.W * (dst.Cp / 8);
            static const bool gdc_serial = getenv("FID_GDC_SERIAL") != nullptr;
            if (op[W_KH] == op[W_KW] && op[W_KH] <= 8 && op[W_PAD] == 0 && src.H == op[W_KH] && src.W == op[W_KW] && dst.H == 1 && dst.W == 1 && !gdc_serial) {
                const int groups = batch * (dst.Cp / 8);
                hipLaunchKernelGGL(gdc_rows, dim3((unsigned)cdiv(groups * 8, 256)), dim3(256), 0, ctx->stream, (const _Float16 *)src.ptr,
                                   (const float *)(blob + op[W_WOFF]), bias, slope, (_Float16 *)dst.ptr, op[W_KH], dst.Cp, op[W_ACT], groups);
                break;
            }
            static const bool dw_global = getenv("FID_DW_GLOBAL") != nullptr;
            if (!dw_global && op[W_KH] == 3 && op[W_KW] == 3 && op[W_STRIDE] == 1 && op[W_PAD] == 1 && dst.Cp % 64 == 0 && src.H >= 12 && src.W >= 12 &&
                (long long)batch * src.H * src.W >= 50000) {
                const int tx = cdiv(src.W, DW_TC), ty = cdiv(src.H, DW_TR), cbs = dst.Cp / 64;
                hipLaunchKernelGGL(dwconv3x3_lds, dim3((unsigned)(batch * ty * tx * cbs)), dim3(256), 0, ctx->stream, (const _Float16 *)src.ptr,
                                   (const float *)(blob + op[W_WOFF]), bias, slope, (_Float16 *)dst.ptr, src.H, src.W, dst.Cp, op[W_ACT], tx, ty, cbs);
                break;
            }
            hipLaunchKernelGGL(dwconv_nhwc, dim3((unsigned)cdiv64(total, 256)), dim3(256), 0, ctx->stream, (const _Float16 *)src.ptr,
                               (const float *)(blob + op[W_WOFF]), bias, slope, (_Float16 *)dst.ptr, src.H, src.W, dst.H, dst.W,
                               dst.Cp, op[W_KH], op[W_STRIDE], op[W_PAD], op[W_ACT], total);
            break;
        }
        default:
            set_error("net: unknown op type %d at %d", op[W_TYPE], oi);
            return FID_E_INVALID;
    }
    return FID_OK;
}

size_t partial_need(fid_ctx *ctx, fid_net *net, int batch) {
    size_t need = 0;
    for (int oi = 0; oi < net->n_ops; oi++) {
        const int32_t *op = &net->ops[(size_t)oi * FID_OP_WORDS];
        if (op[W_TYPE] != OP_CONV || op[W_X_DST2] > 0) continue;
        const TensorView src = view(net, op[W_SRC]), dst = view(net, op[W_DST]);
        ConvArgs a{};
        a.Cin_p = src.Cp; a.Cout_p = dst.Cp; a.kh = op[W_KH]; a.kw = op[W_KW];
        a.M = batch * dst.H * dst.W; a.flags = op[W_FLAGS];
        need = std::max(need, conv_plan(a, ctx->num_cus, true).partial_bytes);
        a.H = src.H; a.W = src.W; a.Ho = dst.H; a.Wo = dst.W; a.stride = op[W_STRIDE]; a.pad = op[W_PAD]; a.w_rows = op[W_WROWS];
        for (const ConvPlan &c : conv_candidates(a, ctx->num_cus, true)) need = std::max(need, c.partial_bytes);
    }
    return std::max<size_t>(need, 256);
}

static int run_all_impl(fid_ctx *ctx, fid_net *net, const uint8_t *images, int batch, float *op_ms);

int run_all(fid_ctx *ctx, fid_net *net, const uint8_t *images, int batch, float *op_ms) {
    const int rc = run_all_impl(ctx, net, images, batch, op_ms);
    if (rc != FID_OK && ctx && net && net->tuned_now) {
        net->tuned_now = false;
        (void)release_scratch(ctx, 4);
    }
    return rc;
}

static int run_all_impl(fid_ctx *ctx, fid_net *net, const uint8_t *images, int batch, float *op_ms) {
    FID_REQUIRE(ctx && net && images, "NULL argument");
    FID_REQUIRE(batch > 0 && batch <= net->max_batch, "batch %d outside [1, %d]", batch, net->max_batch);
    FID_REQUIRE((int)net->tuned.size() == net->n_ops, "net: plan table has %zu entries for %d ops", net->tuned.size(), net->n_ops);
    std::lock_guard<std::mutex> lk(ctx->mu);
    FID_HIP(hipSetDevice(ctx->device));
    void *partial_ws = nullptr;
    const int sbq = (!op_ms && net->sub_batch > 0) ? std::min(net->sub_batch, batch) : batch;
    const size_t need = std::max(partial_need(ctx, net, sbq), partial_need(ctx, net, batch % sbq ? batch % sbq : sbq));
    if (need) FID_TRY(get_scratch(ctx, 1, need, &partial_ws));
    net->partial_cap = need;
    if (op_ms) {
        if (net->n_prof_events < net->n_ops + 1) {
            net->prof_events = new hipEvent_t[net->n_ops + 1];
            for (int i = 0; i <= net->n_ops; i++) FID_HIP(hipEventCreate(&net->prof_events[i]));
            net->n_prof_events = net->n_ops + 1;
        }
        FID_HIP(hipEventRecord(net->prof_events[0], ctx->stream));
    }
    if (op_ms) {
        for (int oi = 0; oi < net->n_ops; oi++) {
            FID_TRY(run_op(ctx, net, oi, images, 0, batch, need ? partial_ws : nullptr));
            FID_HIP(hipEventRecord(net->prof_events[oi + 1], ctx->stream));
        }
    } else {
        const int sb = net->sub_batch > 0 ? net->sub_batch : batch;
        auto issue = [&]() -> int {
            for (int first = 0; first < batch; first += sb) {
                const int nb = std::min(sb, batch - first);
                for (int oi = 0; oi < net->n_ops; oi++) FID_TRY(run_op(ctx, net, oi, images, first, nb, need ? partial_ws : nullptr));
            }
            return FID_OK;
        };
        constexpr int MAX_REPLAYS = 8;
        net->run_counter++;
        fid_net::Replay *rp = nullptr;
        if (net->graphs) {
            auto key = std::make_pair((const void *)images, batch);
            auto it = net->replays.find(key);
            if (it == net->replays.end()) {
                if ((int)net->replays.size() >= MAX_REPLAYS) {
                    auto victim = net->replays.begin();
                    for (auto j = net->replays.begin(); j != net->replays.end(); ++j)
                        if (j->second.last_use < victim->second.last_use) victim = j;
                    if (victim->second.exec) (void)hipGraphExecDestroy(victim->second.exec);
                    net->replays.erase(victim);
                }
                it = net->replays.emplace(key, fid_net::Replay{}).first;
            }
            rp = &it->second;
            rp->last_use = net->run_counter;
            rp->seen++;
            if (rp->exec && rp->partial != partial_ws) {
                (void)hipGraphExecDestroy(rp->exec);
                rp->exec = nullptr;
            }
        }
        if (rp && rp->exec) {
            FID_HIP(hipGraphLaunch(rp->exec, ctx->stream));
        } else if (rp && rp->seen > 2) {
            hipGraph_t g = nullptr;
            FID_HIP(hipStreamBeginCapture(ctx->stream, hipStreamCaptureModeRelaxed));
            const int rc = issue();
            const hipError_t ce = hipStreamEndCapture(ctx->stream, &g);
            if (rc != FID_OK) {
                if (g) (void)hipGraphDestroy(g);
                return rc;
            }
            FID_HIP(ce);
            FID_HIP(hipGraphInstantiate(&rp->exec, g, nullptr, nullptr, 0));
            (void)hipGraphDestroy(g);
            rp->partial = partial_ws;
            FID_HIP(hipGraphLaunch(rp->exec, ctx->stream));
        } else {
            FID_TRY(issue());
        }
    }
    FID_HIP(hipGetLastError());
    if (op_ms) {
        FID_HIP(hipEventSynchronize(net->prof_events[net->n_ops]));
        for (int oi = 0; oi < net->n_ops; oi++) FID_HIP(hipEventElapsedTime(&op_ms[oi], net->prof_events[oi], net->prof_events[oi + 1]));
    }
    if (net->tuned_now) {
        net->tuned_now = false;
        FID_TRY(release_scratch(ctx, 4));
    }
    return FID_OK;
}

}
}

extern "C" {

int fid_net_create(fid_ctx *ctx, const int32_t *ops, int n_ops, const int32_t *tensors, int n_tensors, const void *blob,
                   size_t blob_bytes, int in_h, int in_w, int max_batch, fid_net **out) {
    using namespace fid;
    FID_REQUIRE(ctx && ops && tensors && blob && out, "NULL argument");
    FID_REQUIRE(n_ops > 0 && n_tensors > 0 && max_batch > 0 && in_h > 0 && in_w > 0, "bad sizes");
    std::lock_guard<std::mutex> lk(ctx->mu);
    FID_HIP(hipSetDevice(ctx->device));
    fid_net *net = new fid_net();
    net->n_ops = n_ops; net->n_tensors = n_tensors; net->in_h = in_h; net->in_w = in_w; net->max_batch = max_batch;
    net->ops.assign(ops, ops + (size_t)n_ops * FID_OP_WORDS);
    net->tensors.assign(tensors, tensors + (size_t)n_tensors * FID_TENSOR_WORDS);
    int n_slots = 0;
    for (int t = 0; t < n_tensors; t++) {
        const int32_t *tt = &net->tensors[(size_t)t * FID_TENSOR_WORDS];
        if (tt[T_SLOT] < 0 || tt[T_CP] % 8 != 0 || tt[T_H] <= 0 || tt[T_W] <= 0) {
            delete net;
            set_error("tensor %d: bad record", t);
            return FID_E_INVALID;
        }
        n_slots = std::max(n_slots, tt[T_SLOT] + 1);
    }
    net->slot_bytes_per_image.assign(n_slots, 0);
    for (int t = 0; t < n_tensors; t++) {
        const int32_t *tt = &net->tensors[(size_t)t * FID_TENSOR_WORDS];
        const size_t b = (size_t)tt[T_H] * tt[T_W] * tt[T_CP] * (tt[T_DTYPE] == 1 ? 4 : 2);
        net->slot_bytes_per_image[tt[T_SLOT]] = std::max(net->slot_bytes_per_image[tt[T_SLOT]], b);
    }
    for (int oi = 0; oi < n_ops; oi++) {
        const int32_t *op = &net->ops[(size_t)oi * FID_OP_WORDS];
        auto in_blob = [&](long long off, size_t bytes) { return off >= 0 && (size_t)off + bytes <= blob_bytes; };
        auto opt_in_blob = [&](long long off, size_t bytes) { return off < 0 || (size_t)off + bytes <= blob_bytes; };
        bool ok = op[W_DST] >= 0 && op[W_DST] < n_tensors && op[W_SRC] >= -1 && op[W_SRC] < n_tensors && op[W_RES] >= -1 && op[W_RES] < n_tensors &&
                  op[W_WOFF] >= -1 && opt_in_blob(op[W_WOFF], (size_t)std::max(0, op[W_WBYTES])) &&
                  (op[W_TYPE] == OP_STEM || op[W_TYPE] == OP_STEMFUSED || op[W_TYPE] == OP_STEMBLOCK) == (op[W_SRC] == -1) && op[W_WROWS] >= 0;
        if (ok) {
            const int cp_src = op[W_SRC] >= 0 ? net->tensors[(size_t)op[W_SRC] * FID_TENSOR_WORDS + T_CP] : 0;
            const int cp_dst = net->tensors[(size_t)op[W_DST] * FID_TENSOR_WORDS + T_CP];
            const size_t rows = (size_t)op[W_WROWS];
            switch (op[W_TYPE]) {
            case OP_CONV: {
                const int ncls = (op[W_FLAGS] & CF_BORDER) ? 9 : 1;
                ok = opt_in_blob(op[W_BOFF], (size_t)ncls * rows * 4) && opt_in_blob(op[W_SOFF], rows * 4);
                if (ok && op[W_X_SRC2] != 0) {
                    ok = op[W_X_SRC2] > 0 && op[W_X_SRC2] <= n_tensors && op[W_X_T2] >= 1 && op[W_X_KW2] >= 1 && op[W_X_T2] % op[W_X_KW2] == 0 &&
                         op[W_X_S2] >= 1 && op[W_X_DST2] == 0 && op[W_X_W2OFF] > 0 && op[W_X_B2OFF] > 0 && op[W_X_SCOP] >= 1 && op[W_X_SCOP] <= oi;
                    if (ok) {
                        const int cp2 = net->tensors[(size_t)(op[W_X_SRC2] - 1) * FID_TENSOR_WORDS + T_CP];
                        const size_t row_halfs = (size_t)op[W_KH] * op[W_KW] * cp_src + (size_t)op[W_X_T2] * cp2;
                        ok = in_blob(op[W_X_W2OFF], rows * row_halfs * 2) && in_blob(op[W_X_B2OFF], rows * 4);
                    }
                } else if (ok && op[W_X_W2OFF] != 0) {
                    ok = op[W_X_W2OFF] > oi + 1 && op[W_X_W2OFF] <= n_ops;
                }
                break;
            }
            case OP_STEM:
            case OP_DWCONV:
                ok = opt_in_blob(op[W_BOFF], rows * 4) && opt_in_blob(op[W_SOFF], rows * 4);
                break;
            case OP_STEMBLOCK:
                ok = cp_dst == 64 && op[W_WOFF] >= 0 && (size_t)op[W_WBYTES] >= 64 * 27 * 4 && in_blob(op[W_BOFF], 64 * 4) && opt_in_blob(op[W_SOFF], 64 * 4) &&
                     in_blob(op[W_S_W1], (size_t)2 * 73728) && in_blob(op[W_S_B1], (size_t)((op[W_FLAGS] & CF_BORDER) ? 9 : 1) * 64 * 4) &&
                     opt_in_blob(op[W_S_S1], 64 * 4) && (op[W_S_ACT0] == ACT_RELU || (op[W_S_ACT0] == ACT_PRELU && op[W_SOFF] >= 0)) &&
                     (op[W_ACT] == ACT_RELU || (op[W_ACT] == ACT_PRELU && op[W_S_S1] >= 0)) && op[W_S_DST2] >= 0 && op[W_S_DST2] <= n_tensors &&
                     (op[W_S_DST2] == 0 || net->tensors[(size_t)(op[W_S_DST2] - 1) * FID_TENSOR_WORDS + T_CP] == 64);
                break;
            case OP_LATFPN:
                ok = cp_dst == 64 && (cp_src == 64 || cp_src == 96) && op[W_WOFF] >= 0 && (size_t)op[W_WBYTES] >= (size_t)2 * 73728 && in_blob(op[W_BOFF], 64 * 4) &&
                     in_blob(op[W_L_W0], (size_t)64 * cp_src * 2) && in_blob(op[W_L_B0], 64 * 4) && op[W_L_LAT] >= 0 && op[W_L_LAT] <= n_tensors &&
                     (op[W_L_LAT] == 0 || net->tensors[(size_t)(op[W_L_LAT] - 1) * FID_TENSOR_WORDS + T_CP] == 64) &&
                     (op[W_RES] < 0 || net->tensors[(size_t)op[W_RES] * FID_TENSOR_WORDS + T_CP] == 64);
                break;
            case OP_STEMFUSED:
                ok = in_blob(op[W_F_W0], 32 * 32 * 2) && in_blob(op[W_F_B0], 32 * 4) && in_blob(op[W_F_W1], (size_t)32 * 9 * 32 * 2) && in_blob(op[W_F_B1], 32 * 4) &&
                     in_blob(op[W_F_W2], (size_t)cp_dst * 9 * 32 * 2) && in_blob(op[W_F_B2], (size_t)cp_dst * 4);
                break;
            case OP_BBLOCK: {
                const size_t image = (size_t)(cp_src / 32) * 73728;
                ok = (cp_src == 32 || cp_src == 64) && in_blob(op[W_B_W1], image) && in_blob(op[W_B_W2], image) &&
                     in_blob(op[W_B_B1], (size_t)((op[W_FLAGS] & CF_BORDER) ? 9 : 1) * cp_src * 4) && in_blob(op[W_B_B2], (size_t)cp_src * 4) &&
                     (op[W_B_ACT1] == ACT_RELU || (op[W_B_ACT1] == ACT_PRELU && in_blob(op[W_B_S1], (size_t)cp_src * 4)));
                break;
            }
            case OP_DWPW:
                ok = op[W_WOFF] >= 0 && in_blob(op[W_D_WOFF], (size_t)9 * cp_src * 4) && in_blob(op[W_D_BOFF], (size_t)cp_src * 4) &&
                     (op[W_D_ACT] != ACT_PRELU || in_blob(op[W_D_SOFF], (size_t)cp_src * 4)) && opt_in_blob(op[W_BOFF], rows * 4) && opt_in_blob(op[W_SOFF], rows * 4);
                break;
            case OP_MBBLOCK: {
                const size_t gp = (size_t)std::max(0, op[W_M_GP]);
                ok = op[W_WOFF] >= 0 && gp > 0 && gp % 32 == 0 && (op[W_STRIDE] == 1 || op[W_STRIDE] == 2) && in_blob(op[W_M_W1], gp * cp_src * 2) &&
                     in_blob(op[W_M_B1], gp * 4) && (op[W_M_ACT1] != ACT_PRELU || in_blob(op[W_M_S1], gp * 4)) && in_blob(op[W_M_DW], 9 * gp * 4) &&
                     in_blob(op[W_M_DWB], gp * 4) && (op[W_M_DWACT] != ACT_PRELU || in_blob(op[W_M_DWS], gp * 4)) && (size_t)op[W_WBYTES] >= rows * gp * 2 &&
                     opt_in_blob(op[W_BOFF], rows * 4) && opt_in_blob(op[W_SOFF], rows * 4);
                break;
            }
            default: break;
            }
        }
        if (!ok) {
            delete net;
            set_error("op %d: bad record", oi);
            return FID_E_INVALID;
        }
        const int32_t *dt = &net->tensors[(size_t)op[W_DST] * FID_TENSOR_WORDS];
        if (op[W_TYPE] == OP_STEMFUSED || op[W_TYPE] == OP_BBLOCK || op[W_TYPE] == OP_DWPW || op[W_TYPE] == OP_MBBLOCK || op[W_TYPE] == OP_STEMBLOCK || op[W_TYPE] == OP_LATFPN)
            net->macs_per_image += (double)(((unsigned long long)(unsigned)op[W_F_MACS_HI] << 32) | (unsigned)op[W_F_MACS_LO]);
        if (op[W_TYPE] == OP_CONV && op[W_X_DST2] > 0) net->macs_per_image += (double)(unsigned)op[W_F_MACS_LO];
        if (op[W_TYPE] == OP_CONV || op[W_TYPE] == OP_STEM || op[W_TYPE] == OP_DWCONV)
            net->macs_per_image += (double)dt[T_H] * dt[T_W] * op[W_COUT] * (op[W_CIN] / std::max(1, op[W_GROUPS])) * op[W_KH] * op[W_KW];
    }
    for (int s = 0; s < n_slots; s++) {
        const size_t bytes = net->slot_bytes_per_image[s] * (size_t)max_batch;
        if (bytes > 0x7FFFFFF0ull) {
            delete net;
            set_error("activation slot %d needs %zu bytes at max_batch=%d (> 2 GiB addressable per tensor): lower max_batch", s, bytes, max_batch);
            return FID_E_INVALID;
        }
    }
    net->slots.assign(n_slots, nullptr);
    for (int s = 0; s < n_slots; s++) FID_HIP(hipMalloc(&net->slots[s], net->slot_bytes_per_image[s] * (size_t)max_batch + 256));
    FID_HIP(hipMalloc(&net->blob, blob_bytes + 256));
    net->blob_bytes = blob_bytes;
    FID_HIP(hipMemcpy(net->blob, blob, blob_bytes, hipMemcpyHostToDevice));
    if (const char *e = getenv("FID_SUB_BATCH")) net->sub_batch = atoi(e);
    if (const char *e = getenv("FID_AUTOTUNE")) net->autotune = atoi(e);
    if (const char *e = getenv("FID_GRAPH")) net->graphs = atoi(e);
    net->tuned.resize(n_ops);
    net->plan_ok.resize(n_ops);
    net->tdir.assign(n_tensors, 0);
    if (getenv("FID_NO_REV")) net->alternate = 0;
    {
        hipDeviceProp_t prop;
        FID_HIP(hipGetDeviceProperties(&prop, ctx->device));
        char arch[128];
        snprintf(arch, sizeof(arch), "%s", prop.gcnArchName);
        if (char *c = strchr(arch, ':')) *c = 0;
        char key[256];
        snprintf(key, sizeof(key), "%s/cus%d", arch, prop.multiProcessorCount);
        for (char *c = key; *c; c++)
            if (*c == '|' || *c == '\n') *c = '_';
        net->device_key = key;
        unsigned long long h = fnv1a(net->ops.data(), net->ops.size() * sizeof(int32_t));
        h = fnv1a(net->tensors.data(), net->tensors.size() * sizeof(int32_t), h);
        h = fnv1a(&blob_bytes, sizeof(blob_bytes), h);
        const int rev = FID_PLAN_REV;
        h = fnv1a(&rev, sizeof(rev), h);
        net->table_hash = h;
    }
    int n_plan = -1;
    const char *plan_file = nullptr;
    if (const char *e = getenv("FID_PLAN")) {
        net->plan_path = e;
        plan_file = e;
        (void)plan_load(net, e, &n_plan);
    } else if (const char *e = getenv("FID_PLAN_RO")) {
        plan_file = e;
        (void)plan_load(net, e, &n_plan);
    }
    if (getenv("FID_TUNE_LOG"))
        fprintf(stderr, "[plan] device key %s, table %016llx: %d picks from %s\n", net->device_key.c_str(), net->table_hash, n_plan, plan_file ? plan_file : "(no plan file)");
    *out = net;
    return FID_OK;
}

int fid_net_plan_save(fid_net *net, const char *path) {
    FID_REQUIRE(net && path, "NULL argument");
    FILE *f = fopen(path, "a");
    FID_REQUIRE(f, "cannot open %s for appending", path);
    char line[512];
    for (int oi = 0; oi < net->n_ops; oi++)
        for (const auto &kv : net->tuned[oi]) {
            fid::plan_line(net, oi, kv.first, kv.second, line, sizeof(line));
            fputs(line, f);
        }
    fclose(f);
    return FID_OK;
}

int fid_net_plan_load(fid_net *net, const char *path, int *n_loaded) {
    FID_REQUIRE(net && path, "NULL argument");
    for (auto &kv : net->replays)
        if (kv.second.exec) (void)hipGraphExecDestroy(kv.second.exec);
    net->replays.clear();
    return fid::plan_load(net, path, n_loaded);
}

int fid_net_set_sub_batch(fid_net *net, int sub_batch) {
    FID_REQUIRE(net && sub_batch >= 0, "bad args");
    net->sub_batch = sub_batch;
    for (auto &kv : net->replays)
        if (kv.second.exec) (void)hipGraphExecDestroy(kv.second.exec);
    net->replays.clear();
    return FID_OK;
}

int fid_net_destroy(fid_ctx *ctx, fid_net *net) {
    if (!net) return FID_OK;
    if (ctx) (void)hipStreamSynchronize(ctx->stream);
    for (void *p : net->slots)
        if (p) (void)hipFree(p);
    if (net->blob) (void)hipFree(net->blob);
    for (auto &kv : net->alt_w)
        if (kv.second) (void)hipFree(kv.second);
    for (auto &kv : net->replays)
        if (kv.second.exec) (void)hipGraphExecDestroy(kv.second.exec);
    if (net->prof_events) {
        for (int i = 0; i < net->n_prof_events; i++) (void)hipEventDestroy(net->prof_events[i]);
        delete[] net->prof_events;
    }
    delete net;
    return FID_OK;
}

int fid_net_run(fid_ctx *ctx, fid_net *net, const uint8_t *images_dev, int batch) {
    return fid::run_all(ctx, net, images_dev, batch, nullptr);
}

int fid_net_run_profiled(fid_ctx *ctx, fid_net *net, const uint8_t *images_dev, int batch, float *op_ms) {
    FID_REQUIRE(op_ms, "op_ms is NULL");
    return fid::run_all(ctx, net, images_dev, batch, op_ms);
}

int fid_net_tensor(fid_net *net, int tensor_id, void **dptr, int dims[4], int *dtype) {
    FID_REQUIRE(net && tensor_id >= 0 && tensor_id < net->n_tensors, "bad tensor id %d", tensor_id);
    const fid::TensorView v = fid::view(net, tensor_id);
    if (dptr) *dptr = v.ptr;
    if (dims) { dims[0] = v.H; dims[1] = v.W; dims[2] = v.C; dims[3] = v.Cp; }
    if (dtype) *dtype = v.dtype;
    return FID_OK;
}

int fid_net_macs(fid_net *net, double *macs_per_image) {
    FID_REQUIRE(net && macs_per_image, "NULL argument");
    *macs_per_image = net->macs_per_image;
    return FID_OK;
}

}
```

scrfd_arcface_facerecognition_amd/engine.py:

```python
from __future__ import annotations

import ctypes as C
from typing import Dict, List, Optional, Sequence

import numpy as np

from . import _lib
from ._lib import Context, DeviceBuffer, check
from .archs import ARCHS, ONNX_BASENAMES, Net, synth_params
from .lower import Lowered, lower


class CompiledNet:

    def __init__(self, ctx: Context, net: Net, params: Dict[str, np.ndarray], max_batch: int = 64):
        self.ctx = ctx
        self.net = net
        self.low: Lowered = lower(net, params)
        self.max_batch = int(max_batch)
        ops = np.ascontiguousarray(self.low.ops, dtype=np.int32)
        tens = np.ascontiguousarray(self.low.tensors, dtype=np.int32)
        h = C.c_void_p()
        blob = self.low.blob
        check(ctx.lib.fid_net_create(ctx.handle, ops.ctypes.data_as(_lib.c_i32_p), ops.shape[0],
                                     tens.ctypes.data_as(_lib.c_i32_p), tens.shape[0], blob, len(blob),
                                     net.in_hw[0], net.in_hw[1], self.max_batch, C.byref(h)))
        self.handle = h
        self.in_hw = tuple(net.in_hw)
        self._in_buf: Optional[DeviceBuffer] = None

    def run_device(self, images_dev, batch: int):
        check(self.ctx.lib.fid_net_run(self.ctx.handle, self.handle, _lib._ptr(images_dev), int(batch)))

    def run(self, images: np.ndarray):
        images = np.ascontiguousarray(images, dtype=np.uint8)
        assert images.ndim == 4 and images.shape[1:3] == self.in_hw and images.shape[3] == 3, images.shape
        if self._in_buf is None or self._in_buf.nbytes < images.nbytes:
            self._in_buf = self.ctx.empty((self.max_batch,) + images.shape[1:], np.uint8)
        check(self.ctx.lib.fid_memcpy_h2d(self.ctx.handle, C.c_void_p(self._in_buf.ptr),
                                          images.ctypes.data_as(C.c_void_p), images.nbytes))
        self.ctx.sync()
        self.run_device(self._in_buf, images.shape[0])
        return images.shape[0]

    def run_profiled(self, images_dev, batch: int) -> np.ndarray:
        ms = np.zeros(len(self.low.op_names), dtype=np.float32)
        check(self.ctx.lib.fid_net_run_profiled(self.ctx.handle, self.handle, _lib._ptr(images_dev), int(batch),
                                                ms.ctypes.data_as(_lib.c_f32_p)))
        return ms

    def tensor(self, name: str):
        p = C.c_void_p()
        dims = (C.c_int * 4)()
        dt = C.c_int()
        check(self.ctx.lib.fid_net_tensor(self.handle, self.low.tensor_id[name], C.byref(p), dims, C.byref(dt)))
        return p.value, tuple(dims), (np.float32 if dt.value == 1 else np.float16)

    def read(self, name: str, batch: int) -> np.ndarray:
        ptr, (H, W, Cc, Cp), dt = self.tensor(name)
        buf = self.ctx.borrow(ptr, (batch, H, W, Cp), dt)
        return buf.download()[..., :Cc].astype(np.float32)

    def save_plan(self, path: str):
        check(self.ctx.lib.fid_net_plan_save(self.handle, str(path).encode()))

    def load_plan(self, path: str) -> int:
        n = C.c_int()
        check(self.ctx.lib.fid_net_plan_load(self.handle, str(path).encode(), C.byref(n)))
        return n.value

    def plans(self) -> List[dict]:
        import os
        import tempfile
        fd, path = tempfile.mkstemp(suffix=".plan")
        os.close(fd)
        try:
            self.save_plan(path)
            out = []
            with open(path) as f:
                for line in f:
                    parts = line.rstrip("\n").split("|")
                    if len(parts) != 5:
                        continue
                    v = [int(x) for x in parts[4].split()]
                    oi = int(parts[2])
                    out.append(dict(op=oi, name=self.low.op_names[oi], batch=int(parts[3]), gen=v[0], bm=v[1], bn=v[2], bk=v[3],
                                    ksplit=v[4], ns=v[5]))
            return out
        finally:
            os.unlink(path)

    def macs_per_image(self) -> float:
        v = C.c_double()
        check(self.ctx.lib.fid_net_macs(self.handle, C.byref(v)))
        return v.value

    def close(self):
        if self.handle:
            self.ctx.lib.fid_net_destroy(self.ctx.handle, self.handle)
            self.handle = None


def resolve_model(model_path: str, in_hw=None):
    import os
    if model_path is None:
        raise ValueError("model_path is required")
    if model_path.startswith("synthetic:"):
        spec = model_path[len("synthetic:"):]
        arch, _, q = spec.partition("?")
        seed = 0
        for kv in q.split("&"):
            if kv.startswith("seed="):
                seed = int(kv[5:])
        if arch not in ARCHS:
            raise ValueError(f"unknown architecture {arch!r}; known: {sorted(ARCHS)}")
        net = ARCHS[arch](in_hw) if in_hw else ARCHS[arch]()
        return net, synth_params(net, seed)
    if not os.path.exists(model_path):
        raise FileNotFoundError(f"model file not found: {model_path}")
    if model_path.endswith(".npz"):
        z = np.load(model_path, allow_pickle=False)
        arch = str(z["__arch__"])
        net = ARCHS[arch](in_hw) if in_hw else ARCHS[arch]()
        return net, {k: z[k] for k in z.files if k != "__arch__"}
    if model_path.endswith(".onnx"):
        from .onnx_reader import load_onnx_model
        return load_onnx_model(model_path, in_hw)
    raise ValueError(f"unsupported model file {model_path}")


def save_params(path: str, arch: str, params: Dict[str, np.ndarray]):
    np.savez(path, __arch__=np.array(arch), **params)


class HeadViews:

    def __init__(self, ptrs: Sequence[int], pix: Sequence[int], anc: Sequence[int], bstride: Sequence[int]):
        self.ptrs = (C.c_void_p * 9)(*[C.c_void_p(int(p)) for p in ptrs])
        self.pix = (C.c_int32 * 9)(*[int(v) for v in pix])
        self.anc = (C.c_int32 * 9)(*[int(v) for v in anc])
        self.bstride = (C.c_int64 * 9)(*[int(v) for v in bstride])

    @staticmethod
    def from_onnx_layout(bufs: Sequence[DeviceBuffer], A: int = 2):
        ptrs, pix, anc, bs = [], [], [], []
        for k, b in enumerate(bufs):
            c = (1, 4, 10)[k // 3]
            ptrs.append(b.ptr)
            pix.append(A * c)
            anc.append(c)
            bs.append(b.shape[1] * c)
        return HeadViews(ptrs, pix, anc, bs)

    @staticmethod
    def from_fused(cnet: CompiledNet):
        ptrs, pix, anc, bs = [None] * 9, [0] * 9, [0] * 9, [0] * 9
        for li, name in enumerate(cnet.low.outputs):
            h = cnet.low.heads[name]
            base, (H, W, _, Cp), dt = cnet.tensor(name)
            assert dt == np.float32
            for part, (off, c) in enumerate((h["score"], h["bbox"], h["kps"])):
                k = part * 3 + li
                ptrs[k] = base + off * 4
                pix[k] = Cp
                anc[k] = c
                bs[k] = H * W * Cp
        return HeadViews(ptrs, pix, anc, bs)


class PostProcessor:

    def __init__(self, ctx: Context, max_batch: int, cap: int = 256, cand_cap: int = 4096):
        self.ctx, self.cap, self.max_batch = ctx, int(cap), int(max_batch)
        self.det = ctx.empty((max_batch, cap, 5), np.float32)
        self.kps = ctx.empty((max_batch, cap, 10), np.float32)
        self.counts = ctx.empty((max_batch,), np.int32)
        self.cand_cap = int(cand_cap)
        check(ctx.lib.fid_scrfd_set_candidate_capacity(ctx.handle, self.cand_cap))

    def run(self, hv: HeadViews, B, in_hw, img_hw, conf, iou, max_num=0, metric=0, A=2):
        assert B <= self.max_batch
        check(self.ctx.lib.fid_scrfd_postprocess(
            self.ctx.handle, C.cast(hv.ptrs, _lib.c_void_pp), hv.pix, hv.anc, hv.bstride, int(B), int(in_hw[0]),
            int(in_hw[1]), int(A), int(img_hw[0]), int(img_hw[1]), float(conf), float(iou), int(max_num),
            int(metric), C.c_void_p(self.det.ptr), C.c_void_p(self.kps.ptr), C.c_void_p(self.counts.ptr), self.cap))

    def check(self) -> int:
        m = C.c_int()
        check(self.ctx.lib.fid_scrfd_check(self.ctx.handle, C.byref(m)))
        return m.value

    def fetch(self, B) -> List:
        self.check()
        counts = self.counts.download()[:B]
        det = self.det.download()
        kps = self.kps.download()
        return [(det[b, :counts[b]].copy(), kps[b, :counts[b]].reshape(-1, 5, 2).copy()) for b in range(B)]


class Gallery:

    def __init__(self, ctx: Context, embeddings: np.ndarray, names: Optional[Sequence[str]] = None):
        emb = np.ascontiguousarray(embeddings, dtype=np.float32)
        assert emb.ndim == 2
        self.ctx = ctx
        self.G, self.dim = emb.shape
        self.names = list(names) if names is not None else [str(i) for i in range(self.G)]
        h = C.c_void_p()
        check(ctx.lib.fid_gallery_create(ctx.handle, emb.ctypes.data_as(C.c_void_p), self.G, self.dim, C.byref(h)))
        self.handle = h
        gp = C.c_int()
        check(ctx.lib.fid_gallery_info(h, None, C.byref(gp), None))
        self.Gp = gp.value

    def match_device(self, q_f16_dev, n, thresh, idx_dev, score_dev):
        check(self.ctx.lib.fid_match(self.ctx.handle, self.handle, _lib._ptr(q_f16_dev), int(n), float(thresh),
                                     _lib._ptr(idx_dev), _lib._ptr(score_dev)))

    def close(self):
        if self.handle:
            self.ctx.lib.fid_gallery_destroy(self.ctx.handle, self.handle)
            self.handle = None


class VectorGallery:

    def __init__(self, ctx: Context, dim: int = 512, capacity: int = 1024):
        self.ctx, self.dim = ctx, int(dim)
        self._gal = Gallery(ctx, np.zeros((int(capacity), dim), np.float32))
        self.row_of: Dict[object, int] = {}
        self.id_of: Dict[int, object] = {}
        self._free = list(range(int(capacity) - 1, -1, -1))

    def __len__(self):
        return len(self.row_of)

    def _grow(self):
        old = self._gal
        cap = old.G * 2
        rows = self.ctx.borrow(_gallery_ptr(old), (old.Gp, self.dim), np.float16).download()[:old.G].astype(np.float32)
        new = Gallery(self.ctx, np.concatenate([rows, np.zeros((cap - old.G, self.dim), np.float32)]))
        self._free = list(range(cap - 1, old.G - 1, -1)) + self._free
        old.close()
        self._gal = new

    def upsert(self, ids, embeddings):
        emb = np.ascontiguousarray(embeddings, dtype=np.float32).reshape(len(ids), self.dim)
        rows = []
        for i in ids:
            if i not in self.row_of:
                if not self._free:
                    self._grow()
                r = self._free.pop()
                self.row_of[i], self.id_of[r] = r, i
            rows.append(self.row_of[i])
        rows = np.asarray(rows, dtype=np.int32)
        check(self.ctx.lib.fid_gallery_set_rows(self.ctx.handle, self._gal.handle, rows.ctypes.data_as(_lib.c_i32_p),
                                                emb.ctypes.data_as(C.c_void_p), len(rows)))

    def delete(self, ids):
        rows = np.asarray([self.row_of.pop(i) for i in ids], dtype=np.int32)
        for r in rows:
            self.id_of.pop(int(r))
            self._free.append(int(r))
        zeros = np.zeros((len(rows), self.dim), np.float32)
        check(self.ctx.lib.fid_gallery_set_rows(self.ctx.handle, self._gal.handle, rows.ctypes.data_as(_lib.c_i32_p),
                                                zeros.ctypes.data_as(C.c_void_p), len(rows)))

    def search(self, embeddings, k: int = 5, score_threshold: float = 0.0):
        emb = np.ascontiguousarray(embeddings, dtype=np.float32).reshape(-1, self.dim)
        n = emb.shape[0]
        e = self.ctx.to_device(emb)
        q = self.ctx.empty((n, self.dim), np.float16)
        check(self.ctx.lib.fid_l2_normalize_f16(self.ctx.handle, C.c_void_p(e.ptr), n, self.dim, C.c_void_p(q.ptr)))
        idx, sc = self.ctx.empty((n, k), np.int32), self.ctx.empty((n, k), np.float32)
        check(self.ctx.lib.fid_gallery_topk(self.ctx.handle, self._gal.handle, C.c_void_p(q.ptr), n, int(k), float(score_threshold),
                                            C.c_void_p(idx.ptr), C.c_void_p(sc.ptr)))
        I, S = idx.download(), sc.download()
        return [[(self.id_of[int(j)], float(s)) for j, s in zip(I[r], S[r]) if j >= 0] for r in range(n)]


    def is_duplicate(self, embedding, duplicate_threshold: float = 0.95) -> bool:
        return len(self) > 0 and len(self.search(np.asarray(embedding, np.float32).reshape(1, self.dim), k=1, score_threshold=duplicate_threshold)[0]) > 0

    def similarity_rows(self, ids) -> np.ndarray:
        gal = self._gal
        base = _gallery_ptr(gal)
        out = np.empty((len(ids), gal.G), np.float32)
        rows = np.asarray([self.row_of[i] for i in ids], dtype=np.int64)
        stage = self.ctx.empty((min(1024, max(1, len(ids))), self.dim), np.float16)
        cm = self.ctx.empty((stage.shape[0], gal.Gp), np.float32)
        unit = self.ctx.borrow(base, (gal.Gp, self.dim), np.float16).download()
        for c0 in range(0, len(ids), stage.shape[0]):
            blk = rows[c0:c0 + stage.shape[0]]
            q = np.zeros(stage.shape, np.float16)
            q[:len(blk)] = unit[blk]
            stage.upload(q)
            check(self.ctx.lib.fid_cosine_matrix(self.ctx.handle, gal.handle, C.c_void_p(stage.ptr), len(blk), C.c_void_p(cm.ptr)))
            out[c0:c0 + len(blk)] = cm.download()[:len(blk), :gal.G]
        return out

    def find_and_merge_duplicates(self, similarity_threshold: float = 0.8):
        ids = sorted(self.row_of)
        if len(ids) < 2:
            return []
        sims = self.similarity_rows(ids)
        col = np.asarray([self.row_of[i] for i in ids])
        alive = {i: True for i in ids}
        merges = []
        for a, p1 in enumerate(ids):
            if not alive[p1]:
                continue
            s = sims[a, col]
            for b in np.argsort(-s, kind="stable"):
                if s[b] < similarity_threshold:
                    break
                p2 = ids[int(b)]
                if p2 <= p1 or not alive[p2]:
                    continue
                alive[p2] = False
                merges.append((p1, p2, float(s[b])))
        if merges:
            self.delete([m[1] for m in merges])
        return merges


def _gallery_ptr(gal: Gallery) -> int:
    p = C.c_void_p()
    check(gal.ctx.lib.fid_gallery_data(gal.handle, C.byref(p)))
    return int(p.value)
```

scrfd_arcface_facerecognition_amd/lower.py:

```python
from __future__ import annotations

from typing import Dict, List, Tuple

import numpy as np

from .archs import BN_EPS, Net, infer_shapes

OP_WORDS, TENSOR_WORDS = 32, 8
OP_STEM, OP_CONV, OP_MAXPOOL, OP_DWCONV, OP_STEMFUSED, OP_BBLOCK, OP_DWPW, OP_MBBLOCK, OP_STEMBLOCK, OP_LATFPN = 1, 2, 3, 4, 5, 6, 7, 8, 9, 10
ACT = {"none": 0, "relu": 1, "prelu": 2}
CF_RES_UP2, CF_BORDER, CF_OUT_F32 = 1, 2, 4
CPAD = 32


def _rup(x, m):
    return (x + m - 1) // m * m


def _bn_affine(P, prefix):
    a = P[prefix + ".gamma"].astype(np.float64) / np.sqrt(P[prefix + ".var"].astype(np.float64) + BN_EPS)
    b = P[prefix + ".beta"].astype(np.float64) - P[prefix + ".mean"].astype(np.float64) * a
    return a, b


class _Blob:
    def __init__(self):
        self.parts: List[bytes] = []
        self.size = 0

    def add(self, arr: np.ndarray) -> Tuple[int, int]:
        raw = np.ascontiguousarray(arr).tobytes()
        off = self.size
        pad = (-len(raw)) % 256
        self.parts.append(raw + b"\0" * pad)
        self.size += len(raw) + pad
        return off, len(raw)

    def bytes(self) -> bytes:
        return b"".join(self.parts)


class Lowered:

    def __init__(self):
        self.ops: np.ndarray = None
        self.tensors: np.ndarray = None
        self.blob: bytes = b""
        self.tensor_id: Dict[str, int] = {}
        self.op_names: List[str] = []
        self.op_nodes: List[List[str]] = []
        self.outputs: List[str] = []
        self.in_hw = (0, 0)
        self.macs = 0
        self.heads: Dict[str, dict] = {}
        self.fused_groups: Dict[str, list] = {}


def _dual_ok(net, i, tensors, tid, shp):
    import os
    n = net.nodes[i]
    nxt = net.nodes[i + 1] if i + 1 < len(net.nodes) else None
    return (n.kind == "conv" and n.groups == 1 and n.pre_avgpool and not os.environ.get("FID_NO_DOWN_FUSE")
            and nxt is not None and nxt.kind == "conv" and nxt.groups == 1 and nxt.src == n.src and nxt.k == 3 and nxt.stride == 2
            and nxt.pad == 1 and nxt.res is None and not nxt.pre_bn and not n.pre_bn and not nxt.pre_avgpool
            and nxt.act in ("none", "relu") and n.act == "none" and n.res is None and not n.res_up2 and not nxt.res_up2
            and tensors[tid[n.src]][1] == 64 and _rup(n.cout, CPAD) == 96 and _rup(nxt.cout, CPAD) == 96
            and shp[n.name][1:] == shp[nxt.name][1:])


def _shortcut_target(net, i, tensors, tid, shp):
    n = net.nodes[i]
    if not (n.k == 1 and n.pad == 0 and n.act == "none" and n.res is None and not n.pre_bn and not n.res_up2 and n.src != "input"
            and n.name not in net.outputs and n.groups == 1):
        return None
    avg = bool(n.pre_avgpool)
    if (avg and n.stride != 1) or (not avg and n.stride not in (1, 2)) or (avg and _dual_ok(net, i, tensors, tid, shp)):
        return None
    s_eff, taps = (2, 2) if avg else (n.stride, 1)
    users = [x for x in net.nodes if getattr(x, "src", None) == n.name or getattr(x, "res", None) == n.name]
    if len(users) != 1:
        return None
    m = users[0]
    if not (m.kind == "conv" and m.res == n.name and m.src != n.name and m.groups == 1 and m.k == 3 and m.pad == 1 and not m.pre_bn
            and m.stride == (1 if avg else 2) and not m.pre_avgpool and not m.res_up2 and net.nodes.index(m) > i and shp[m.name] == shp[n.name]):
        return None
    x_t = tensors[tid[n.src]]
    if m.src not in tid:
        src_node = next(x for x in net.nodes if x.name == m.src)
        cin_p = _rup(src_node.cout, CPAD)
    else:
        cin_p = tensors[tid[m.src]][1]
    _, ho, wo = shp[m.name]
    if x_t[4] != 0 or x_t[1] % 32 or cin_p % 32 or (ho - 1) * s_eff + taps - 1 >= x_t[2] or (wo - 1) * s_eff + taps - 1 >= x_t[3]:
        return None
    if not avg and n.stride != m.stride and not getattr(n, "_even_src", False):
        return None
    return m


def _mbf_block(net, i, tensors, tid, shp):
    if i + 2 >= len(net.nodes):
        return None
    n, d, m = net.nodes[i], net.nodes[i + 1], net.nodes[i + 2]
    if not (d.kind == "conv" and m.kind == "conv" and n.k == 1 and n.pad == 0 and n.stride == 1 and n.src != "input" and n.res is None
            and not n.pre_bn and not n.pre_avgpool and not n.res_up2
            and d.groups == d.cin == d.cout == n.cout and d.groups > 1 and d.k == 3 and d.pad == 1 and d.stride in (1, 2) and d.src == n.name
            and d.res is None and not d.pre_bn and not d.pre_avgpool
            and m.groups == 1 and m.k == 1 and m.pad == 0 and m.stride == 1 and m.src == d.name and m.res in (None, n.src)
            and not m.pre_bn and not m.pre_avgpool and not m.res_up2):
        return None
    if n.name in net.outputs or d.name in net.outputs:
        return None
    for x in net.nodes:
        if x is not d and (getattr(x, "src", None) == n.name or getattr(x, "res", None) == n.name):
            return None
        if x is not m and (getattr(x, "src", None) == d.name or getattr(x, "res", None) == d.name):
            return None
    src_t = tensors[tid[n.src]]
    cin_p, gp, cout_p, H, W = src_t[1], _rup(n.cout, CPAD), _rup(m.cout, CPAD), src_t[2], src_t[3]
    if src_t[4] != 0 or cin_p % 32 or cin_p > 256 or gp % 32 or cout_p % 16 or cout_p > 256:
        return None
    if m.res is not None and (d.stride != 1 or cin_p != cout_p):
        return None
    if gp > 512:
        return None
    to = 7 if d.stride == 1 else 4
    rup = lambda v: (v + 1023) // 1024 * 1024
    if rup(81 * (cin_p * 2 + 16)) + rup(81 * (gp * 2 + 16)) + ((to * to + 15) // 16 * 16) * (gp * 2 + 16) > 160 * 1024:
        return None
    return d, m


def _latfpn(net, i, tensors, tid):
    import os
    n = net.nodes[i]
    if os.environ.get("FID_NO_LATFPN_FUSE") or not (n.kind == "conv" and n.k == 1 and n.pad == 0 and n.stride == 1 and n.groups == 1 and n.act == "none"
                                                    and not n.pre_bn and not n.pre_avgpool and n.src != "input" and n.name not in net.outputs
                                                    and (n.res is None or n.res_up2) and _rup(n.cout, CPAD) == 64):
        return None
    src_t = tensors[tid[n.src]]
    if src_t[4] != 0 or src_t[1] not in (64, 96) or src_t[2] < 3 or src_t[3] < 3:
        return None
    if n.res is not None:
        r_t = tensors[tid[n.res]]
        if r_t[4] != 0 or r_t[1] != 64 or src_t[2] != 2 * r_t[2] or src_t[3] != 2 * r_t[3]:
            return None
    convs, adders = [], 0
    for j, x in enumerate(net.nodes):
        if getattr(x, "src", None) == n.name:
            convs.append((j, x))
        if getattr(x, "res", None) == n.name:
            if not (x.kind == "conv" and x.res_up2 and x.src != n.name):
                return None
            adders += 1
    if len(convs) != 1:
        return None
    j, m = convs[0]
    if not (j > i and m.kind == "conv" and m.k == 3 and m.stride == 1 and m.pad == 1 and m.groups == 1 and m.act == "none" and m.res is None and not m.pre_bn
            and not m.pre_avgpool and m.cin == n.cout and _rup(m.cout, CPAD) == 64):
        return None
    return j, m, adders > 0


def lower(net: Net, P: Dict[str, np.ndarray]) -> Lowered:
    shp = infer_shapes(net)
    blob = _Blob()
    ops: List[List[int]] = []
    op_names: List[str] = []
    op_nodes: List[List[str]] = []
    tensors: List[List[int]] = []
    tid: Dict[str, int] = {}
    out = Lowered()

    def new_tensor(name, C, H, W, dtype=0, Cp=None):
        Cp = _rup(C, CPAD) if Cp is None else Cp
        tid[name] = len(tensors)
        tensors.append([C, Cp, H, W, dtype, -1, 0, 0])
        return tid[name]

    def emit(name, **kw):
        rec = [0] * OP_WORDS
        rec[3] = -1
        rec[13] = rec[15] = rec[16] = -1
        rec[18] = 1
        idx = dict(type=0, src=1, dst=2, res=3, kh=4, kw=5, stride=6, pad=7, cin=8, cout=9, act=10, flags=11,
                   nsig=12, woff=13, wbytes=14, boff=15, soff=16, wrows=17, groups=18)
        for k, v in kw.items():
            rec[idx[k]] = int(v)
        ops.append(rec)
        op_names.append(name)
        op_nodes.append([name])

    def pack_weights(W4, cin_p, cout_p):
        cout, cin, kh, kw = W4.shape
        Wp = np.zeros((cout_p, kh * kw, cin_p), dtype=np.float32)
        Wp[:cout, :, :cin] = W4.transpose(0, 2, 3, 1).reshape(cout, kh * kw, cin)
        h = Wp.astype(np.float16)
        if not np.isfinite(h).all():
            raise ValueError("weights overflow fp16")
        return h

    def repack_kind2(Wp):
        cout_p, taps, cin_p = Wp.shape
        assert taps == 9 and cout_p <= 128 and cin_p % 32 == 0
        full = np.zeros((128, 9, cin_p), dtype=np.float16)
        full[:cout_p] = Wp
        x = full.reshape(8, 16, 3, 3, cin_p // 32, 4, 8)
        return np.ascontiguousarray(x.transpose(4, 0, 3, 2, 5, 1, 6))

    def padded(vec, n, fill=0.0):
        o = np.full(n, fill, dtype=np.float32)
        o[: len(vec)] = vec
        return o

    def folded(n):
        W = P[n.wname + ".weight"].astype(np.float64)
        b = P[n.wname + ".bias"].astype(np.float64) if n.bias else np.zeros(n.cout)
        if n.post_bn:
            a2, b2 = _bn_affine(P, n.wname + ".post_bn")
            W = W * a2[:, None, None, None]
            b = b * a2 + b2
        return W, b

    def fold_conv(n, src_hw):
        W = P[n.wname + ".weight"].astype(np.float64)
        b = P[n.wname + ".bias"].astype(np.float64) if n.bias else np.zeros(n.cout)
        k, stride, pad = n.k, n.stride, n.pad
        if n.pre_avgpool:
            assert k == 1 and pad == 0 and stride == 1
            W = np.repeat(np.repeat(W, 2, axis=2), 2, axis=3) / 4.0
            k, stride = 2, 2
        bias_tab = None
        if n.pre_bn:
            a1, b1 = _bn_affine(P, n.wname + ".pre_bn")
            shift = np.einsum("oikl,i->okl", W, b1)
            W = W * a1[None, :, None, None]
            if pad == 0:
                b = b + shift.sum(axis=(1, 2))
            else:
                assert k == 3 and pad == 1 and stride == 1 and src_hw[0] >= 2 and src_hw[1] >= 2, n.name
                bias_tab = np.zeros((9, n.cout))
                for yc in range(3):
                    for xc in range(3):
                        m = np.ones((3, 3))
                        if yc == 0: m[0, :] = 0
                        if yc == 2: m[2, :] = 0
                        if xc == 0: m[:, 0] = 0
                        if xc == 2: m[:, 2] = 0
                        bias_tab[yc * 3 + xc] = b + (shift * m[None]).sum(axis=(1, 2))
        if bias_tab is None:
            bias_tab = b[None, :]
        if n.post_bn:
            a2, b2 = _bn_affine(P, n.wname + ".post_bn")
            W = W * a2[:, None, None, None]
            bias_tab = bias_tab * a2[None, :] + b2[None, :]
        return W, bias_tab, k, stride

    import os
    fused_upto = 0
    nd = net.nodes
    if (len(nd) >= 4 and not os.environ.get("FID_NO_STEM_FUSE") and nd[0].kind == "conv" and nd[0].src == "input"
            and all(x.kind == "conv" and x.k == 3 and x.pad == 1 and x.groups == 1 and x.act == "relu" and not x.pre_bn
                    and x.res is None and not x.pre_avgpool for x in nd[0:3])
            and nd[0].stride == 2 and nd[1].stride == 1 and nd[2].stride == 1 and nd[1].src == nd[0].name
            and nd[2].src == nd[1].name and nd[3].kind == "maxpool" and nd[3].src == nd[2].name
            and (nd[3].k, nd[3].stride, nd[3].pad) == (3, 2, 1) and nd[0].cout <= 32 and nd[1].cout <= 32
            and nd[2].cout <= 64 and net.in_hw[0] % 4 == 0 and net.in_hw[1] % 4 == 0
            and not any(getattr(x, "src", None) in (nd[0].name, nd[1].name, nd[2].name) or getattr(x, "res", None) in
                        (nd[0].name, nd[1].name, nd[2].name) for x in nd[4:])
            and not any(o in (nd[0].name, nd[1].name, nd[2].name) for o in net.outputs)):
        c0, c1, c2, pool = nd[0], nd[1], nd[2], nd[3]
        W0, b0 = folded(c0)
        W1, b1 = folded(c1)
        W2, b2 = folded(c2)
        w0 = np.zeros((32, 32), dtype=np.float32)
        w0[: c0.cout, :27] = (W0[:, ::-1] * (net.in_scale / 2.0)).transpose(0, 2, 3, 1).reshape(c0.cout, 27)
        c2p = _rup(c2.cout, CPAD)
        offs = [blob.add(w0.astype(np.float16))[0], blob.add(padded(b0, 32))[0],
                blob.add(pack_weights(W1, 32, 32))[0], blob.add(padded(b1, 32))[0],
                blob.add(pack_weights(W2, 32, c2p))[0], blob.add(padded(b2, c2p))[0]]
        _, hp, wp = shp[pool.name]
        dst = new_tensor(pool.name, c2.cout, hp, wp)
        rec = [0] * OP_WORDS
        rec[0], rec[1], rec[2], rec[3] = OP_STEMFUSED, -1, dst, -1
        rec[4] = rec[5] = 3
        rec[13] = rec[15] = rec[16] = -1
        rec[18] = 1
        rec[20:26] = offs
        macs = sum(shp[x.name][1] * shp[x.name][2] * x.cout * x.cin * 9 for x in (c0, c1, c2))
        rec[26], rec[27] = macs & 0xFFFFFFFF, macs >> 32
        if rec[26] >= 2 ** 31:
            rec[26] -= 2 ** 32
        ops.append(rec)
        op_names.append("stem.fused")
        op_nodes.append([c0.name, c1.name, c2.name, pool.name])
        out.fused_groups = {"stem.fused": [c0.name, c1.name, c2.name, pool.name]}
        fused_upto = 4

    skip = set()
    if fused_upto == 0 and not os.environ.get("FID_NO_STEMBLOCK_FUSE") and len(nd) >= 2:
        st = nd[0]
        users = [(i, x) for i, x in enumerate(nd) if getattr(x, "src", None) == st.name or getattr(x, "res", None) == st.name]
        c1s = [(i, x) for i, x in users if x.kind == "conv" and x.src == st.name and x.k == 3 and x.stride == 1 and x.pad == 1 and x.groups == 1
               and x.cin == 64 and x.cout == 64 and x.res is None and x.act in ("relu", "prelu") and not x.pre_avgpool and not x.res_up2]
        others = [(i, x) for i, x in users if not c1s or x is not c1s[0][1]]
        sc_ok = all(x.kind == "conv" and x.src == st.name and x.res != st.name and x.k == 1 and x.stride == 2 and x.pad == 0 and x.groups == 1
                    and not x.pre_bn and not x.pre_avgpool for _, x in others)
        H0, W0 = net.in_hw
        if (st.kind == "conv" and st.src == "input" and st.k == 3 and st.stride == 1 and st.pad == 1 and st.groups == 1 and st.cout == 64
                and st.act in ("relu", "prelu") and st.res is None and not st.pre_bn and len(c1s) == 1 and sc_ok and len(others) <= 1
                and st.name not in net.outputs and W0 % 4 == 0 and H0 >= 3 and abs(net.in_mean - 127.5) < 1e-12):
            import copy
            import dataclasses
            ci, c1 = c1s[0]
            W = P[st.wname + ".weight"].astype(np.float64)
            b = P[st.wname + ".bias"].astype(np.float64) if st.bias else np.zeros(64)
            if st.post_bn:
                a2, b2 = _bn_affine(P, st.wname + ".post_bn")
                W = W * a2[:, None, None, None]
                b = b * a2 + b2
            Wd = np.ascontiguousarray((W[:, ::-1] * (net.in_scale / 2.0)).transpose(0, 2, 3, 1), dtype=np.float32)
            w0off, w0bytes = blob.add(Wd)
            b0off = blob.add(padded(b, 64))[0]
            s0off = blob.add(padded(P[st.wname + ".prelu"], 64))[0] if st.act == "prelu" else -1
            W1, bt1, _, _ = fold_conv(c1, (H0, W0))
            for nm_, arr_ in (("stem weights", Wd), ("stem bias", b), ("conv1 weights", W1), ("conv1 bias", bt1)):
                if not np.isfinite(np.asarray(arr_, dtype=np.float64)).all() or np.abs(np.asarray(arr_, dtype=np.float64)).max() > 65504.0:
                    raise ValueError(f"{st.name} / {c1.name}: folded {nm_} are not finite fp16 values; the fused stem block cannot take them")
            b1t = np.zeros((bt1.shape[0], 64), dtype=np.float32)
            b1t[:, :64] = bt1
            w1off = blob.add(repack_kind2(pack_weights(W1, 64, 64)))[0]
            b1off = blob.add(b1t)[0]
            s1off = blob.add(padded(P[c1.wname + ".prelu"], 64))[0] if c1.act == "prelu" else -1
            dst = new_tensor(c1.name, 64, H0, W0)
            dst2 = 0
            if others:
                even = st.name + ".even"
                dst2 = new_tensor(even, 64, (H0 + 1) // 2, (W0 + 1) // 2) + 1
                shp[even] = (64, (H0 + 1) // 2, (W0 + 1) // 2)
                oi_, sc_node = others[0]
                sc2 = dataclasses.replace(sc_node, src=even, stride=1)
                sc2._even_src = True
                net = copy.copy(net)
                net.nodes = list(nd)
                net.nodes[oi_] = sc2
                nd = net.nodes
            rec = [0] * OP_WORDS
            rec[0], rec[1], rec[2], rec[3] = OP_STEMBLOCK, -1, dst, -1
            rec[4] = rec[5] = 3
            rec[6], rec[7], rec[8], rec[9], rec[10] = 1, 1, 3, 64, ACT[c1.act]
            rec[11] = CF_BORDER if bt1.shape[0] == 9 else 0
            rec[13], rec[14], rec[15], rec[16], rec[17], rec[18] = w0off, w0bytes, b0off, s0off, 64, 1
            rec[20], rec[21], rec[22], rec[23], rec[24] = w1off, b1off, s1off, ACT[st.act], dst2
            macs = H0 * W0 * 64 * 27 + H0 * W0 * 64 * 64 * 9
            rec[26], rec[27] = macs & 0xFFFFFFFF, macs >> 32
            if rec[26] >= 2 ** 31:
                rec[26] -= 2 ** 32
            ops.append(rec)
            op_names.append(c1.name)
            op_nodes.append([st.name, c1.name])
            out.fused_groups[c1.name] = [st.name, c1.name]
            skip.update({0, ci})
    pending_sc = {}
    for ni_, n in enumerate(net.nodes):
        if ni_ < fused_upto or ni_ in skip:
            continue
        nxt = net.nodes[ni_ + 1] if ni_ + 1 < len(net.nodes) else None
        if (n.kind == "conv" and n.groups == 1 and n.src != "input" and not os.environ.get("FID_NO_SC_FUSE")
                and _shortcut_target(net, ni_, tensors, tid, shp) is not None):
            pending_sc[_shortcut_target(net, ni_, tensors, tid, shp).name] = (n, len(ops))
        if n.kind == "conv" and n.src == "input":
            assert n.k == 3 and n.pad == 1 and n.groups == 1 and not n.pre_bn and n.res is None
            cout, (_, ho, wo) = n.cout, shp[n.name]
            cp = _rup(cout, CPAD)
            assert cp in (32, 64, 128), cp
            W = P[n.wname + ".weight"].astype(np.float64)
            b = P[n.wname + ".bias"].astype(np.float64) if n.bias else np.zeros(cout)
            if n.post_bn:
                a2, b2 = _bn_affine(P, n.wname + ".post_bn")
                W = W * a2[:, None, None, None]
                b = b * a2 + b2
            Wd = np.zeros((cp, 3, 3, 3), dtype=np.float32)
            Wd[:cout] = (W[:, ::-1] * (net.in_scale / 2.0)).transpose(0, 2, 3, 1)
            assert abs(net.in_mean - 127.5) < 1e-12
            woff, wbytes = blob.add(Wd)
            boff, _ = blob.add(padded(b, cp))
            soff = blob.add(padded(P[n.wname + ".prelu"], cp))[0] if n.act == "prelu" else -1
            dst = new_tensor(n.name, cout, ho, wo)
            emit(n.name, type=OP_STEM, src=-1, dst=dst, kh=3, kw=3, stride=n.stride, pad=1, cin=3, cout=cout,
                 act=ACT[n.act], woff=woff, wbytes=wbytes, boff=boff, soff=soff, wrows=cp)
        elif _dual_ok(net, ni_, tensors, tid, shp):
            m = nxt
            src_t = tensors[tid[n.src]]
            cin_p = src_t[1]
            _, ho, wo = shp[m.name]

            def folded_w(c, W):
                b = P[c.wname + ".bias"].astype(np.float64) if c.bias else np.zeros(c.cout)
                if c.post_bn:
                    a2, b2 = _bn_affine(P, c.wname + ".post_bn")
                    W = W * a2[:, None, None, None]
                    b = b * a2 + b2
                return W, b
            W1, b1 = folded_w(m, P[m.wname + ".weight"].astype(np.float64))
            Wd = P[n.wname + ".weight"].astype(np.float64)
            Wd = np.repeat(np.repeat(Wd, 2, axis=2), 2, axis=3) / 4.0
            Wd, b2 = folded_w(n, Wd)
            W2 = np.zeros((n.cout, n.cin, 3, 3))
            W2[:, :, 1:3, 1:3] = Wd
            Wp = np.concatenate([pack_weights(W1, cin_p, 96), pack_weights(W2, cin_p, 96)], axis=0)
            woff, wbytes = blob.add(Wp)
            bt = np.zeros((1, 192), dtype=np.float32)
            bt[0, :m.cout] = b1
            bt[0, 96:96 + n.cout] = b2
            boff, _ = blob.add(bt)
            dst2 = new_tensor(n.name, n.cout, ho, wo)
            dst = new_tensor(m.name, m.cout, ho, wo)
            emit(m.name, type=OP_CONV, src=tid[n.src], dst=dst, res=-1, kh=3, kw=3, stride=2, pad=1, cin=m.cin, cout=m.cout,
                 act=ACT[m.act], flags=0, woff=woff, wbytes=wbytes, boff=boff, soff=-1, wrows=192)
            ops[-1][20], ops[-1][21], ops[-1][22] = dst2 + 1, ACT[n.act], 96
            macs2 = ho * wo * n.cout * n.cin * 4
            assert macs2 < 2 ** 31
            ops[-1][26], ops[-1][27] = macs2, 0
            op_nodes[-1] = [n.name, m.name]
            out.fused_groups[m.name] = [n.name, m.name]
            skip.add(ni_ + 1)
        elif (n.kind == "conv" and n.groups == 1 and not os.environ.get("FID_NO_BB_FUSE") and nxt is not None and nxt.kind == "conv"
              and nxt.groups == 1 and n.k == 3 and nxt.k == 3 and n.stride == 1 and nxt.stride == 1 and n.pad == 1 and nxt.pad == 1
              and n.act in ("relu", "prelu") and nxt.act in ("relu", "none") and n.res is None and nxt.res == n.src and nxt.src == n.name
              and not n.res_up2 and not nxt.res_up2 and not nxt.pre_bn and not n.pre_avgpool and not nxt.pre_avgpool
              and n.src != "input" and tensors[tid[n.src]][1] in (32, 64) and tensors[tid[n.src]][4] == 0 and _rup(n.cout, CPAD) == tensors[tid[n.src]][1]
              and _rup(nxt.cout, CPAD) == tensors[tid[n.src]][1] and (tensors[tid[n.src]][1] == 64 or (n.act == "relu" and not n.pre_bn))
              and n.name not in net.outputs and tensors[tid[n.src]][2] >= 3 and tensors[tid[n.src]][3] >= 3
              and not any(getattr(x, "src", None) == n.name or getattr(x, "res", None) == n.name for x in net.nodes if x is not nxt)):
            m = nxt
            src_t = tensors[tid[n.src]]
            W1, bt1, _, _ = fold_conv(n, (src_t[2], src_t[3]))
            W2, bt2, _, _ = fold_conv(m, (src_t[2], src_t[3]))
            assert bt2.shape[0] == 1
            cpb = src_t[1]
            b1t = np.zeros((bt1.shape[0], cpb), dtype=np.float32)
            b1t[:, :n.cout] = bt1
            offs = [blob.add(repack_kind2(pack_weights(W1, cpb, cpb)))[0], blob.add(b1t)[0],
                    blob.add(repack_kind2(pack_weights(W2, cpb, cpb)))[0], blob.add(padded(bt2[0], cpb))[0]]
            s1_off = blob.add(padded(P[n.wname + ".prelu"], cpb))[0] if n.act == "prelu" else -1
            _, ho, wo = shp[m.name]
            dst = new_tensor(m.name, m.cout, ho, wo)
            rec = [0] * OP_WORDS
            rec[0], rec[1], rec[2], rec[3] = OP_BBLOCK, tid[n.src], dst, -1
            rec[4] = rec[5] = 3
            rec[6], rec[7] = 1, 1
            rec[8], rec[9], rec[10] = n.cin, m.cout, ACT[m.act]
            rec[13] = rec[15] = rec[16] = -1
            rec[18] = 1
            rec[20:24] = offs
            rec[24], rec[25] = s1_off, ACT[n.act]
            rec[11] = CF_BORDER if bt1.shape[0] == 9 else 0
            macs = ho * wo * 9 * (n.cout * n.cin + m.cout * m.cin)
            rec[26], rec[27] = macs & 0xFFFFFFFF, macs >> 32
            if rec[26] >= 2 ** 31:
                rec[26] -= 2 ** 32
            ops.append(rec)
            op_names.append(m.name)
            op_nodes.append([n.name, m.name])
            out.fused_groups[m.name] = [n.name, m.name]
            skip.add(ni_ + 1)
        elif (n.kind == "conv" and n.groups == 1 and not os.environ.get("FID_NO_MBF_FUSE") and _mbf_block(net, ni_, tensors, tid, shp) is not None):
            d, m = _mbf_block(net, ni_, tensors, tid, shp)
            src_t = tensors[tid[n.src]]
            cin_p, gp, cout_p = src_t[1], _rup(n.cout, CPAD), _rup(m.cout, CPAD)
            W1, b1 = folded(n)
            w1_off = blob.add(pack_weights(W1, cin_p, gp))[0]
            b1_off = blob.add(padded(b1, gp))[0]
            s1_off = blob.add(padded(P[n.wname + ".prelu"], gp))[0] if n.act == "prelu" else -1
            Wdw = P[d.wname + ".weight"].astype(np.float64)[:, 0]
            bdw = P[d.wname + ".bias"].astype(np.float64) if d.bias else np.zeros(d.cout)
            if d.post_bn:
                a2, b2 = _bn_affine(P, d.wname + ".post_bn")
                Wdw = Wdw * a2[:, None, None]
                bdw = bdw * a2 + b2
            Wd = np.zeros((9, gp), dtype=np.float32)
            Wd[:, :d.cout] = Wdw.reshape(d.cout, 9).T
            dw_off = blob.add(Wd)[0]
            dwb_off = blob.add(padded(bdw, gp))[0]
            dws_off = blob.add(padded(P[d.wname + ".prelu"], gp))[0] if d.act == "prelu" else -1
            W2, b2 = folded(m)
            w2_off, w2_bytes = blob.add(pack_weights(W2, gp, cout_p))
            b2_off = blob.add(padded(b2, cout_p)[None, :])[0]
            s2_off = blob.add(padded(P[m.wname + ".prelu"], cout_p))[0] if m.act == "prelu" else -1
            _, ho, wo = shp[m.name]
            dst = new_tensor(m.name, m.cout, ho, wo)
            emit(m.name, type=OP_MBBLOCK, src=tid[n.src], dst=dst, res=tid[m.res] if m.res else -1, kh=3, kw=3, stride=d.stride, pad=1, cin=n.cin,
                 cout=m.cout, act=ACT[m.act], flags=0, woff=w2_off, wbytes=w2_bytes, boff=b2_off, soff=s2_off, wrows=cout_p)
            r = ops[-1]
            r[20], r[21], r[22], r[23], r[24], r[25], r[28], r[29], r[30] = w1_off, b1_off, s1_off, ACT[n.act], dw_off, dwb_off, dws_off, ACT[d.act], gp
            _, h1, w1_ = shp[n.name]
            macs = h1 * w1_ * n.cout * n.cin + ho * wo * d.cout * 9 + ho * wo * m.cout * m.cin
            r[26], r[27] = macs & 0xFFFFFFFF, macs >> 32
            if r[26] >= 2 ** 31:
                r[26] -= 2 ** 32
            op_nodes[-1] = [n.name, d.name, m.name]
            out.fused_groups[m.name] = [n.name, d.name, m.name]
            skip.add(ni_ + 1)
            skip.add(ni_ + 2)
        elif n.kind == "conv" and n.groups == 1 and _latfpn(net, ni_, tensors, tid) is not None:
            mj, m, keep_lat = _latfpn(net, ni_, tensors, tid)
            src_t = tensors[tid[n.src]]
            W0, b0 = folded(n)
            w0off = blob.add(pack_weights(W0, src_t[1], 64).reshape(64, src_t[1]))[0]
            b0off = blob.add(padded(b0, 64))[0]
            W1, b1 = folded(m)
            w1off, w1bytes = blob.add(repack_kind2(pack_weights(W1, 64, 64)))
            b1off = blob.add(padded(b1, 64)[None, :])[0]
            _, ho, wo = shp[m.name]
            lat_t = new_tensor(n.name, n.cout, ho, wo) + 1 if keep_lat else 0
            dst = new_tensor(m.name, m.cout, ho, wo)
            emit(m.name, type=OP_LATFPN, src=tid[n.src], dst=dst, res=tid[n.res] if n.res else -1, kh=3, kw=3, stride=1, pad=1, cin=m.cin, cout=m.cout,
                 act=0, flags=0, woff=w1off, wbytes=w1bytes, boff=b1off, soff=-1, wrows=64)
            r = ops[-1]
            r[20], r[21], r[22] = w0off, b0off, lat_t
            macs = ho * wo * (n.cout * n.cin + m.cout * m.cin * 9)
            r[26], r[27] = macs & 0xFFFFFFFF, macs >> 32
            if r[26] >= 2 ** 31:
                r[26] -= 2 ** 32
            op_nodes[-1] = [n.name, m.name]
            out.fused_groups[m.name] = [n.name, m.name]
            skip.add(mj)
        elif n.kind == "conv" and n.groups == 1:
            cin, cout = n.cin, n.cout
            _, ho, wo = shp[n.name]
            src_t = tensors[tid[n.src]]
            cin_p, cout_p = src_t[1], _rup(cout, CPAD)
            W, bias_tab, k, stride = fold_conv(n, (src_t[2], src_t[3]))
            pad = n.pad
            ncls = bias_tab.shape[0]
            Wp = pack_weights(W, cin_p, cout_p)
            sc, sc_op = pending_sc.pop(n.name, (None, -1))
            woff, wbytes = blob.add(Wp)
            bt = np.zeros((ncls, cout_p), dtype=np.float32)
            bt[:, :cout] = bias_tab
            boff, _ = blob.add(bt)
            if sc is not None:
                Wsc, bsc = folded(sc)
                if sc.pre_avgpool:
                    Wsc = np.repeat(np.repeat(Wsc, 2, axis=2), 2, axis=3) / 4.0
                x_t = tensors[tid[sc.src]]
                assert ncls == 1 and ops[sc_op][2] == tid[sc.name]
                W2p = np.concatenate([Wp.reshape(cout_p, -1), pack_weights(Wsc, x_t[1], cout_p).reshape(cout_p, -1)], axis=1)
                w2off = blob.add(W2p)[0]
                bt2 = np.zeros((1, cout_p), dtype=np.float32)
                bt2[0, :cout] = bias_tab[0] + bsc
                b2off = blob.add(bt2)[0]
            soff = blob.add(padded(P[n.wname + ".prelu"], cout_p))[0] if n.act == "prelu" else -1
            flags = (CF_BORDER if ncls == 9 else 0) | (CF_RES_UP2 if n.res_up2 else 0)
            if n.res_up2:
                r_t = tensors[tid[n.res]]
                if (ho, wo) != (2 * r_t[2], 2 * r_t[3]):
                    raise ValueError(f"{n.name}: top-down add of a {r_t[2]}x{r_t[3]} level onto {ho}x{wo}: only exact 2x levels are supported "
                                     "(input sizes that are multiples of 32)")
            dst = new_tensor(n.name, cout, ho, wo)
            emit(n.name, type=OP_CONV, src=tid[n.src], dst=dst, res=tid[n.res] if n.res else -1, kh=k, kw=k,
                 stride=stride, pad=pad, cin=cin, cout=cout, act=ACT[n.act], flags=flags, woff=woff,
                 wbytes=wbytes, boff=boff, soff=soff, wrows=cout_p)
            if sc is not None:
                r = ops[-1]
                t2, kw2, s2 = (4, 2, 2) if sc.pre_avgpool else (1, 1, sc.stride)
                r[23], r[24], r[25], r[28], r[29], r[30], r[31] = tid[sc.src] + 1, t2, kw2, s2, w2off, b2off, sc_op + 1
                ops[sc_op][29] = len(ops)
        elif n.kind == "conv":
            assert n.groups == n.cin == n.cout and not n.pre_bn and not n.pre_avgpool and n.res is None
            c = n.cin
            _, ho, wo = shp[n.name]
            cp = tensors[tid[n.src]][1]
            W = P[n.wname + ".weight"].astype(np.float64)[:, 0]
            b = P[n.wname + ".bias"].astype(np.float64) if n.bias else np.zeros(c)
            if n.post_bn:
                a2, b2 = _bn_affine(P, n.wname + ".post_bn")
                W = W * a2[:, None, None]
                b = b * a2 + b2
            Wd = np.zeros((n.k * n.k, cp), dtype=np.float32)
            Wd[:, :c] = W.reshape(c, -1).T
            woff, wbytes = blob.add(Wd)
            boff, _ = blob.add(padded(b, cp))
            soff = blob.add(padded(P[n.wname + ".prelu"], cp))[0] if n.act == "prelu" else -1
            m = nxt
            if (os.environ.get("FID_DWPW_FUSE") and m is not None and m.kind == "conv" and m.groups == 1 and m.k == 1 and m.pad == 0
                    and m.stride == 1 and m.src == n.name and not m.pre_bn and not m.pre_avgpool and not m.res_up2 and n.k == 3 and n.pad == 1
                    and n.stride in (1, 2) and cp in (32, 64, 128, 256, 512) and n.name not in net.outputs and m.res != n.name
                    and not any(getattr(x, "src", None) == n.name or getattr(x, "res", None) == n.name for x in net.nodes if x is not m)):
                Wm, bm = folded(m)
                cout_p = _rup(m.cout, CPAD)
                pw_off, pw_bytes = blob.add(pack_weights(Wm, cp, cout_p))
                pb_off, _ = blob.add(padded(bm, cout_p)[None, :])
                ps_off = blob.add(padded(P[m.wname + ".prelu"], cout_p))[0] if m.act == "prelu" else -1
                _, mho, mwo = shp[m.name]
                dst = new_tensor(m.name, m.cout, mho, mwo)
                emit(m.name, type=OP_DWPW, src=tid[n.src], dst=dst, res=tid[m.res] if m.res else -1, kh=3, kw=3, stride=n.stride, pad=1, cin=c,
                     cout=m.cout, act=ACT[m.act], flags=0, woff=pw_off, wbytes=pw_bytes, boff=pb_off, soff=ps_off, wrows=cout_p)
                ops[-1][20], ops[-1][21], ops[-1][22], ops[-1][23] = woff, boff, soff, ACT[n.act]
                macs = ho * wo * c * n.k * n.k + mho * mwo * m.cout * m.cin
                ops[-1][26], ops[-1][27] = macs & 0xFFFFFFFF, macs >> 32
                if ops[-1][26] >= 2 ** 31:
                    ops[-1][26] -= 2 ** 32
                op_nodes[-1] = [n.name, m.name]
                out.fused_groups[m.name] = [n.name, m.name]
                skip.add(ni_ + 1)
                continue
            dst = new_tensor(n.name, c, ho, wo, Cp=cp)
            emit(n.name, type=OP_DWCONV, src=tid[n.src], dst=dst, kh=n.k, kw=n.k, stride=n.stride, pad=n.pad,
                 cin=c, cout=c, act=ACT[n.act], woff=woff, wbytes=wbytes, boff=boff, soff=soff, wrows=cp, groups=c)
        elif n.kind == "maxpool":
            c, ho, wo = shp[n.name]
            dst = new_tensor(n.name, c, ho, wo, Cp=tensors[tid[n.src]][1])
            emit(n.name, type=OP_MAXPOOL, src=tid[n.src], dst=dst, kh=n.k, kw=n.k, stride=n.stride, pad=n.pad,
                 cin=c, cout=c)
        elif n.kind == "fc":
            src_t = tensors[tid[n.src]]
            C_, Cp_, H_, W_ = src_t[0], src_t[1], src_t[2], src_t[3]
            assert (C_, H_, W_) == (n.c, n.h, n.w)
            Wm = P[n.wname + ".weight"].astype(np.float64).reshape(n.cout, n.c, n.h, n.w)
            b = P[n.wname + ".bias"].astype(np.float64) if n.bias else np.zeros(n.cout)
            if n.pre_bn:
                a1, b1 = _bn_affine(P, n.wname + ".pre_bn")
                b = b + np.einsum("ochw,c->o", Wm, b1)
                Wm = Wm * a1[None, :, None, None]
            if n.post_bn:
                a2, b2 = _bn_affine(P, n.wname + ".post_bn")
                Wm = Wm * a2[:, None, None, None]
                b = b * a2 + b2
            K = H_ * W_ * Cp_
            cout_p = _rup(n.cout, CPAD)
            Wk = np.zeros((cout_p, H_, W_, Cp_), dtype=np.float32)
            Wk[: n.cout, :, :, : n.c] = Wm.transpose(0, 2, 3, 1)
            h = Wk.reshape(cout_p, 1, K).astype(np.float16)
            woff, wbytes = blob.add(h)
            boff, _ = blob.add(padded(b, cout_p)[None, :])
            view = new_tensor(n.name + ".in_view", K, 1, 1, Cp=K)
            tensors[view][5] = -2 - tid[n.src]
            dst = new_tensor(n.name, n.cout, 1, 1, dtype=1)
            emit(n.name, type=OP_CONV, src=view, dst=dst, kh=1, kw=1, stride=1, pad=0, cin=n.c * n.h * n.w,
                 cout=n.cout, act=0, flags=0, woff=woff, wbytes=wbytes, boff=boff, wrows=cout_p)
        elif n.kind == "dethead":
            A = n.num_anchors
            _, h_, w_ = shp[n.name]
            src_t = tensors[tid[n.src]]
            s = float(P[n.wname + ".bbox.scale"][0])
            W = np.concatenate([P[n.wname + ".cls.weight"], P[n.wname + ".bbox.weight"] * s,
                                P[n.wname + ".kps.weight"]], axis=0).astype(np.float64)
            b = np.concatenate([P[n.wname + ".cls.bias"], P[n.wname + ".bbox.bias"] * s,
                                P[n.wname + ".kps.bias"]]).astype(np.float64)
            cout = 15 * A
            cout_p = _rup(cout, CPAD)
            Wp = pack_weights(W, src_t[1], cout_p)
            woff, wbytes = blob.add(Wp)
            boff, _ = blob.add(padded(b, cout_p)[None, :])
            dst = new_tensor(n.name, cout, h_, w_, dtype=1)
            emit(n.name, type=OP_CONV, src=tid[n.src], dst=dst, kh=n.k, kw=n.k, stride=1, pad=n.k // 2, cin=n.cin,
                 cout=cout, act=0, flags=0, nsig=A, woff=woff, wbytes=wbytes, boff=boff, wrows=cout_p)
            out.heads[n.name] = dict(stride=n.stride, anchors=A, cp=cout_p, h=h_, w=w_,
                                     score=(0, 1), bbox=(A, 4), kps=(5 * A, 10))
        else:
            raise ValueError(f"cannot lower node {n}")

    n_t = len(tensors)
    base = list(range(n_t))
    for t in range(n_t):
        if tensors[t][5] <= -2:
            base[t] = -2 - tensors[t][5]
    last_use = [-1] * n_t
    for oi, rec in enumerate(ops):
        for w in (1, 3):
            if rec[w] >= 0:
                last_use[base[rec[w]]] = oi
        if rec[0] == OP_CONV and rec[23] > 0:
            last_use[base[rec[23] - 1]] = oi
    keep = {tid[o] for o in net.outputs}
    slot_of = [-1] * n_t
    slot_size: List[int] = []
    free: List[int] = []

    def nbytes(t):
        return tensors[t][1] * tensors[t][2] * tensors[t][3] * (4 if tensors[t][4] == 1 else 2)

    for oi, rec in enumerate(ops):
        dsts = [rec[2]] + ([rec[20] - 1] if rec[0] == OP_CONV and rec[20] > 0 else [])
        if rec[0] == OP_STEMBLOCK and rec[24] > 0:
            dsts.append(rec[24] - 1)
        if rec[0] == OP_LATFPN and rec[22] > 0:
            dsts.append(rec[22] - 1)
        for d in dsts:
            need = nbytes(d)
            if d in keep or not free:
                slot_size.append(need)
                slot_of[d] = len(slot_size) - 1
            else:
                best = min(free, key=lambda s: (slot_size[s] < need, abs(slot_size[s] - need)))
                free.remove(best)
                slot_size[best] = max(slot_size[best], need)
                slot_of[d] = best
        for t in range(n_t):
            if base[t] == t and slot_of[t] >= 0 and last_use[t] == oi and t not in keep and t not in dsts:
                free.append(slot_of[t])
        for d in dsts:
            if last_use[d] < 0 and d not in keep:
                free.append(slot_of[d])
    for t in range(n_t):
        tensors[t][5] = slot_of[base[t]]
        if t in keep:
            tensors[t][6] = 1
        assert tensors[t][5] >= 0, t

    out.ops = np.asarray(ops, dtype=np.int32).reshape(-1, OP_WORDS)
    out.tensors = np.asarray(tensors, dtype=np.int32).reshape(-1, TENSOR_WORDS)
    out.blob = blob.bytes()
    out.tensor_id = tid
    out.op_names = op_names
    out.op_nodes = op_nodes
    out.outputs = list(net.outputs)
    out.in_hw = net.in_hw
    return out
```

Before: 18800 faces/s.

## Chain three independent head-level 3x3 convs into one persistent kernel launch

Reorders the SCRFD detection head so that the same-depth conv from each of the three FPN levels sits in consecutive ops. These triples are tagged as chains and can run as one kernel that executes three producer/consumer conv bodies back to back, with a barrier between them and rotated block ids. The aim is to cut launch overhead and fill the CUs better on small per-level convs. Whether a chain is used is decided per batch by timing it against separate launches during autotune, and the choice is stored in the plan file. The change also extends liveness so buffers stay valid across the chain.

```diff
diff --git a/scrfd_arcface_facerecognition_amd/csrc/conv.h b/scrfd_arcface_facerecognition_amd/csrc/conv.h
--- a/scrfd_arcface_facerecognition_amd/csrc/conv.h
+++ b/scrfd_arcface_facerecognition_amd/csrc/conv.h
@@ -65,6 +65,9 @@
 bool conv_pc_applicable(const ConvArgs &a);
 int conv_pc_launch(fid_ctx *ctx, const ConvArgs &a, int cb, int ring);
 
+bool conv_chain_applicable(const ConvArgs *m, int cb);
+int conv_chain_launch(fid_ctx *ctx, const ConvArgs *m, int cb);
+
 bool conv_pc2_applicable(const ConvArgs &a);
 int conv_pc2_launch(fid_ctx *ctx, const ConvArgs &a);
 bool conv_pcr_applicable(const ConvArgs &a);
diff --git a/scrfd_arcface_facerecognition_amd/csrc/conv_chain.hip b/scrfd_arcface_facerecognition_amd/csrc/conv_chain.hip
--- /dev/null
+++ b/scrfd_arcface_facerecognition_amd/csrc/conv_chain.hip
@@ -0,0 +1,81 @@
+#define FID_PC_BODY_ONLY
+#include "conv_pc.hip"
+
+namespace fid {
+namespace {
+
+template <int NI, int WD, int PD, bool F32>
+struct PcBody {
+    typedef PCArgs Args;
+    static constexpr int THREADS = (N_CONS + N_PROD) * 64;
+    static constexpr size_t LDS = (size_t)WD * 9 * 2 * NI * 16 * 64 + (size_t)PD * P_BYTES;
+    static __device__ __forceinline__ void run(const Args &a, int bid, int nblk) { pc_body<NI, WD, PD, F32, false>(a, bid, nblk); }
+};
+
+template <class A, class B, class C>
+struct ChainArgs {
+    typename A::Args a;
+    typename B::Args b;
+    typename C::Args c;
+    int rot[3];
+};
+
+__device__ __forceinline__ void chain_seam() {
+    asm volatile("s_waitcnt vmcnt(0) lgkmcnt(0)\n\ts_barrier" ::: "memory");
+}
+
+template <class A, class B, class C>
+__global__ void __launch_bounds__(A::THREADS, 3) conv_chain3(const ChainArgs<A, B, C> k) {
+    static_assert(A::THREADS == B::THREADS && A::THREADS == C::THREADS, "the bodies of a chain share the workgroup size");
+    const int nblk = (int)gridDim.x, bid = xcd_major_id(blockIdx.x, gridDim.x);
+    A::run(k.a, bid, nblk);
+    chain_seam();
+    const int b1 = bid - k.rot[1];
+    B::run(k.b, b1 < 0 ? b1 + nblk : b1, nblk);
+    chain_seam();
+    const int b2 = bid - k.rot[2];
+    C::run(k.c, b2 < 0 ? b2 + nblk : b2, nblk);
+}
+
+template <class Body>
+int launch_chain3(fid_ctx *ctx, const ConvArgs *m, int cb) {
+    ChainArgs<Body, Body, Body> k{};
+    pc_fill_args(k.a, m[0], cb);
+    pc_fill_args(k.b, m[1], cb);
+    pc_fill_args(k.c, m[2], cb);
+    int grid = 1;
+    for (const PCArgs *a : {&k.a, &k.b, &k.c}) {
+        FID_REQUIRE(a->in_bytes <= OOB && a->w_bytes <= OOB, "conv: tensor larger than 2 GiB");
+        grid = std::max(grid, std::min(a->n_items, ctx->num_cus));
+    }
+    k.rot[0] = 0;
+    k.rot[1] = k.a.n_items % grid;
+    k.rot[2] = (int)(((long long)k.a.n_items + k.b.n_items) % grid);
+    const void *fn = (const void *)conv_chain3<Body, Body, Body>;
+    FID_TRY(ensure_dyn_lds(ctx, fn, (int)Body::LDS));
+    hipLaunchKernelGGL((conv_chain3<Body, Body, Body>), dim3(grid), dim3(Body::THREADS), Body::LDS, ctx->stream, k);
+    FID_HIP(hipGetLastError());
+    return FID_OK;
+}
+
+}
+
+bool conv_chain_applicable(const ConvArgs *m, int cb) {
+    if (cb != 32 && cb != 64 && cb != 96) return false;
+    for (int i = 0; i < 3; i++) {
+        const ConvArgs &a = m[i];
+        if (!conv_pc_applicable(a) || a.in2 != nullptr || a.out2 != nullptr || a.res != nullptr) return false;
+        if (((a.flags & CF_OUT_F32) != 0) != (cb == 32)) return false;
+        if (cb == 96 && a.Cout_p % 96 != 0) return false;
+    }
+    return true;
+}
+
+int conv_chain_launch(fid_ctx *ctx, const ConvArgs *m, int cb) {
+    FID_REQUIRE(conv_chain_applicable(m, cb), "chain launch: cb=%d does not apply to its members", cb);
+    if (cb == 32) return launch_chain3<PcBody<1, 2, 3, true>>(ctx, m, cb);
+    if (cb == 64) return launch_chain3<PcBody<2, 2, 3, false>>(ctx, m, cb);
+    return launch_chain3<PcBody<3, 2, 2, false>>(ctx, m, cb);
+}
+
+}
diff --git a/scrfd_arcface_facerecognition_amd/csrc/conv_pc.hip b/scrfd_arcface_facerecognition_amd/csrc/conv_pc.hip
--- a/scrfd_arcface_facerecognition_amd/csrc/conv_pc.hip
+++ b/scrfd_arcface_facerecognition_amd/csrc/conv_pc.hip
@@ -64,7 +64,7 @@
 }
 
 template <int NI, int WD, int PD, bool F32 = false, bool RS = false>
-__global__ void __launch_bounds__((N_CONS + N_PROD) * 64, 3) conv3x3_pc(const PCArgs a) {
+__device__ __forceinline__ void pc_body(const PCArgs &a, const int bid, const int nblk) {
     constexpr int CB = 2 * NI * 16, MI = 4;
     constexpr int W_BLKS = 9 * CB * 64 / 1024, W_BYTES = W_BLKS * 1024;
     constexpr int AW = WD - 1, AP = PD - 1;
@@ -73,8 +73,7 @@
     char *sWr = smem, *sPr = smem + WD * W_BYTES;
 
     const int tid = threadIdx.x, lane = tid & 63, wave = __builtin_amdgcn_readfirstlane(tid >> 6);
-    const int bid = (a.ablate & 256) ? (int)blockIdx.x : xcd_major_id(blockIdx.x, gridDim.x);
-    const int my_items = bid < a.n_items ? (a.n_items - 1 - bid) / gridDim.x + 1 : 0;
+    const int my_items = bid < a.n_items ? (a.n_items - 1 - bid) / nblk + 1 : 0;
     const int n_steps = my_items * a.n_chunks;
     if (n_steps == 0) return;
 
@@ -228,7 +227,7 @@
         auto cursor_next = [&](Cursor &c) {
             if (++c.ck == a.n_chunks) {
                 c.ck = 0;
-                c.item += gridDim.x;
+                c.item += nblk;
                 cursor_decode(c);
             }
         };
@@ -346,14 +345,14 @@
                     }
                     raw_barrier();
                     read_tile(stage);
-                    store_tile(item - gridDim.x);
+                    store_tile(item - nblk);
                 }
                 STAMP(0, 3);
                 fetch(s + AW < n_steps, (s + AW) % WD, s + AP < n_steps, (s + AP) % PD);
                 if (has_res && ck == a.n_chunks - 1) load_residual(item);
                 lds_done();
                 STAMP(0, 4);
-                if (++ck == a.n_chunks) { ck = 0; item += gridDim.x; }
+                if (++ck == a.n_chunks) { ck = 0; item += nblk; }
             }
             if (F32) return;
             raw_barrier();
@@ -363,7 +362,7 @@
             }
             raw_barrier();
             read_tile(sWr + ((n_steps - 1) % WD) * W_BYTES);
-            store_tile(item - gridDim.x);
+            store_tile(item - nblk);
             return;
         }
         issue_weights(cw, 0);
@@ -395,7 +394,7 @@
                 raw_barrier();
                 read_tile(stage);
                 if (have_w) issue_weights(cw, (s + AW) % WD);
-                const bool all_stores = store_tile(item - gridDim.x);
+                const bool all_stores = store_tile(item - nblk);
                 if (all_stores) young = MAX_S + ((AW == 2 && have_w) ? my_w : 0);
             } else {
                 if (AW == 2) {
@@ -414,7 +413,7 @@
             if (have_w && s + AW + 1 < n_steps) cursor_next(cw);
             if (have_p && s + AP + 1 < n_steps) cursor_next(cp);
             STAMP(0, 4);
-            if (++ck == a.n_chunks) { ck = 0; item += gridDim.x; }
+            if (++ck == a.n_chunks) { ck = 0; item += nblk; }
         }
         if (F32) return;
         raw_barrier();
@@ -425,7 +424,7 @@
         }
         raw_barrier();
         read_tile(sWr + ((n_steps - 1) % WD) * W_BYTES);
-        store_tile(item - gridDim.x);
+        store_tile(item - nblk);
         return;
     }
 
@@ -503,7 +502,7 @@
 
     int li = 0, ck = 0;
     for (int s = 0; s < n_steps; s++) {
-        const int item = bid + li * gridDim.x;
+        const int item = bid + li * nblk;
         [[maybe_unused]] const int who = wave == 0 ? 1 : 2;
         if (wave == 0 || wave == 7) STAMP(who, 0);
         raw_barrier();
@@ -596,6 +595,11 @@
     }
     epi_stage(sWr + ((n_steps - 1) % WD) * W_BYTES);
     raw_barrier();
+}
+
+template <int NI, int WD, int PD, bool F32 = false, bool RS = false>
+__global__ void __launch_bounds__((N_CONS + N_PROD) * 64, 3) conv3x3_pc(const PCArgs a) {
+    pc_body<NI, WD, PD, F32, RS>(a, (a.ablate & 256) ? (int)blockIdx.x : xcd_major_id(blockIdx.x, gridDim.x), (int)gridDim.x);
 }
 
 template <int NI, int WD, int PD, bool F32 = false, bool RS = false>
@@ -628,20 +632,7 @@
     return FID_OK;
 }
 
-}
-
-bool conv_pc_applicable(const ConvArgs &a) {
-    if (getenv("FID_NO_PC")) return false;
-    const bool shape = a.kh == 3 && a.kw == 3 && a.stride == 1 && a.pad == 1 && a.Cin_p % 32 == 0 && a.Cin_p >= 64 &&
-                       a.w_rows == a.Cout_p && a.H == a.Ho && a.W == a.Wo && a.H >= 12 && a.W >= 12 && !(a.flags & (CF_RES_UP2 | CF_ARGMAX));
-    if (!shape) return false;
-    if (a.flags & CF_OUT_F32)
-        return a.Cout_p == 32 && a.act == ACT_NONE && a.res == nullptr && !(a.flags & CF_BORDER);
-    return a.Cout_p >= 64 && a.nsig == 0 && (a.res == nullptr || (a.res_H == a.Ho && a.res_W == a.Wo));
-}
-
-int conv_pc_launch(fid_ctx *ctx, const ConvArgs &c, int cb, int ring) {
-    PCArgs a{};
+inline void pc_fill_args(PCArgs &a, const ConvArgs &c, int cb) {
     a.in = c.in; a.w = c.w; a.bias = c.bias; a.slope = c.slope; a.res = c.res; a.out = c.out;
     a.H = c.H; a.W = c.W; a.Cin_p = c.Cin_p; a.Cout_p = c.Cout_p;
     a.act = c.act; a.flags = c.flags; a.res_Cp = c.res_Cp; a.nsig = c.nsig;
@@ -654,6 +645,24 @@
     a.d_cblk = fastdiv_make(a.n_cblk); a.d_tpi = fastdiv_make(a.tiles_per_img); a.d_tx = fastdiv_make(a.tiles_x);
     a.in_bytes = c.in_bytes;
     a.w_bytes = (unsigned)std::min<size_t>(c.w_bytes, (size_t)c.w_rows * 9 * c.Cin_p * 2);
+}
+
+}
+
+#ifndef FID_PC_BODY_ONLY
+bool conv_pc_applicable(const ConvArgs &a) {
+    if (getenv("FID_NO_PC")) return false;
+    const bool shape = a.kh == 3 && a.kw == 3 && a.stride == 1 && a.pad == 1 && a.Cin_p % 32 == 0 && a.Cin_p >= 64 &&
+                       a.w_rows == a.Cout_p && a.H == a.Ho && a.W == a.Wo && a.H >= 12 && a.W >= 12 && !(a.flags & (CF_RES_UP2 | CF_ARGMAX));
+    if (!shape) return false;
+    if (a.flags & CF_OUT_F32)
+        return a.Cout_p == 32 && a.act == ACT_NONE && a.res == nullptr && !(a.flags & CF_BORDER);
+    return a.Cout_p >= 64 && a.nsig == 0 && (a.res == nullptr || (a.res_H == a.Ho && a.res_W == a.Wo));
+}
+
+int conv_pc_launch(fid_ctx *ctx, const ConvArgs &c, int cb, int ring) {
+    PCArgs a{};
+    pc_fill_args(a, c, cb);
     if (const char *e = getenv("FID_PC_ABLATE")) a.ablate = atoi(e);
     FID_REQUIRE(a.in_bytes <= OOB && a.w_bytes <= OOB, "conv: tensor larger than 2 GiB");
     const bool dma = getenv("FID_PC_RS") == nullptr;
@@ -664,5 +673,6 @@
     set_error("producer/consumer conv: cb=%d unsupported", cb);
     return FID_E_INVALID;
 }
-
-}
+#endif
+
+}
diff --git a/scrfd_arcface_facerecognition_amd/csrc/net.h b/scrfd_arcface_facerecognition_amd/csrc/net.h
--- a/scrfd_arcface_facerecognition_amd/csrc/net.h
+++ b/scrfd_arcface_facerecognition_amd/csrc/net.h
@@ -25,6 +25,7 @@
     W_SOFF = 16,
     W_WROWS = 17,
     W_GROUPS = 18,
+    W_CHAIN = 19,
     W_F_W0 = 20, W_F_B0 = 21, W_F_W1 = 22, W_F_B1 = 23, W_F_W2 = 24, W_F_B2 = 25,
     W_F_MACS_LO = 26, W_F_MACS_HI = 27,
     W_B_W1 = 20, W_B_B1 = 21, W_B_W2 = 22, W_B_B2 = 23, W_B_S1 = 24, W_B_ACT1 = 25,
diff --git a/scrfd_arcface_facerecognition_amd/csrc/net.hip b/scrfd_arcface_facerecognition_amd/csrc/net.hip
--- a/scrfd_arcface_facerecognition_amd/csrc/net.hip
+++ b/scrfd_arcface_facerecognition_amd/csrc/net.hip
@@ -28,6 +28,8 @@
     unsigned long long table_hash = 0;
     std::string device_key, plan_path;
     std::map<std::pair<int, int>, void *> alt_w;
+    std::vector<std::map<int, int>> chain_pick;
+    int chains = 1;
 };
 
 namespace fid {
@@ -377,7 +379,7 @@
     return TensorView{(char *)net->slots[t[T_SLOT]] + per_image * first, t[T_C], t[T_CP], t[T_H], t[T_W], t[T_DTYPE]};
 }
 
-constexpr int FID_PLAN_REV = 5;
+constexpr int FID_PLAN_REV = 6;
 
 unsigned long long fnv1a(const void *p, size_t n, unsigned long long h = 1469598103934665603ull) {
     const unsigned char *b = (const unsigned char *)p;
@@ -386,8 +388,12 @@
 }
 
 void plan_line(const fid_net *net, int oi, int batch, const ConvPlan &c, char *buf, size_t cap) {
-    snprintf(buf, cap, "%s|%016llx|%d|%d|%d %d %d %d %d %d %zu\n", net->device_key.c_str(), net->table_hash, oi, batch, c.gen, c.bm, c.bn,
-             c.bk, c.ksplit, c.ns, c.partial_bytes);
+    int n = snprintf(buf, cap, "%s|%016llx|%d|%d|%d %d %d %d %d %d %zu", net->device_key.c_str(), net->table_hash, oi, batch, c.gen, c.bm, c.bn,
+                     c.bk, c.ksplit, c.ns, c.partial_bytes);
+    const auto &cp = net->chain_pick[oi];
+    auto it = cp.find(batch);
+    if (it != cp.end() && n > 0 && (size_t)n < cap) n += snprintf(buf + n, cap - n, " %d", it->second);
+    if (n > 0 && (size_t)n < cap) snprintf(buf + n, cap - n, "\n");
 }
 
 int plan_load(fid_net *net, const char *path, int *n_loaded) {
@@ -400,12 +406,15 @@
             unsigned long long h = 0;
             int oi = 0, batch = 0;
             ConvPlan c{};
-            if (sscanf(line, "%255[^|]|%llx|%d|%d|%d %d %d %d %d %d %zu", dev, &h, &oi, &batch, &c.gen, &c.bm, &c.bn, &c.bk, &c.ksplit, &c.ns,
-                       &c.partial_bytes) != 11)
+            int chain = -1;
+            if (sscanf(line, "%255[^|]|%llx|%d|%d|%d %d %d %d %d %d %zu %d", dev, &h, &oi, &batch, &c.gen, &c.bm, &c.bn, &c.bk, &c.ksplit, &c.ns,
+                       &c.partial_bytes, &chain) < 11)
                 continue;
             if (h != net->table_hash || net->device_key != dev || oi < 0 || oi >= net->n_ops || batch <= 0) continue;
             net->tuned[oi][batch] = c;
             net->plan_ok[oi].erase(batch);
+            net->chain_pick[oi].erase(batch);
+            if (chain >= 0 && net->ops[(size_t)oi * FID_OP_WORDS + W_CHAIN] > 0) net->chain_pick[oi][batch] = chain;
             n++;
         }
         fclose(f);
@@ -445,6 +454,109 @@
         it = net->alt_w.emplace(key, p).first;
     }
     a.w_alt = it->second;
+    return FID_OK;
+}
+
+ConvArgs conv_args(const fid_net *net, int oi, int first, int batch) {
+    const int32_t *op = &net->ops[(size_t)oi * FID_OP_WORDS];
+    const char *blob = (const char *)net->blob;
+    const TensorView src = view(net, op[W_SRC], first), dst = view(net, op[W_DST], first);
+    ConvArgs a{};
+    a.in = src.ptr;
+    a.w = blob + op[W_WOFF];
+    a.bias = op[W_BOFF] >= 0 ? (const float *)(blob + op[W_BOFF]) : nullptr;
+    a.slope = op[W_SOFF] >= 0 ? (const float *)(blob + op[W_SOFF]) : nullptr;
+    a.out = dst.ptr;
+    a.H = src.H; a.W = src.W; a.Cin_p = src.Cp;
+    a.Ho = dst.H; a.Wo = dst.W; a.Cout_p = dst.Cp;
+    a.w_rows = op[W_WROWS];
+    a.kh = op[W_KH]; a.kw = op[W_KW]; a.stride = op[W_STRIDE]; a.pad = op[W_PAD];
+    a.M = batch * dst.H * dst.W;
+    a.act = op[W_ACT]; a.flags = op[W_FLAGS]; a.nsig = op[W_NSIG];
+    if (dst.dtype == 1) a.flags |= CF_OUT_F32;
+    if (op[W_RES] >= 0) {
+        const TensorView r = view(net, op[W_RES], first);
+        a.res = r.ptr; a.res_H = r.H; a.res_W = r.W; a.res_Cp = r.Cp;
+    }
+    a.in_bytes = (unsigned)((size_t)batch * src.H * src.W * src.Cp * 2);
+    a.w_bytes = (unsigned)op[W_WBYTES];
+    return a;
+}
+
+constexpr int CHAIN_N = 3;
+
+int chain_cb(const fid_net *net, int leader, int first, int batch, ConvArgs *m) {
+    if (!net->chains) return 0;
+    auto it = net->chain_pick[leader].find(batch);
+    if (it == net->chain_pick[leader].end() || it->second <= 0) return 0;
+    for (int k = 0; k < CHAIN_N; k++) m[k] = conv_args(net, leader + k, first, batch);
+    return conv_chain_applicable(m, it->second) ? it->second : 0;
+}
+
+int set_alt_weights(fid_ctx *ctx, fid_net *net, int oi, ConvArgs &a, const ConvPlan &plan);
+
+int decide_chain(fid_ctx *ctx, fid_net *net, int leader, int first, int batch, void *partial_ws) {
+    ConvArgs m[CHAIN_N];
+    ConvPlan p[CHAIN_N];
+    for (int k = 0; k < CHAIN_N; k++) {
+        const int32_t *op = &net->ops[(size_t)(leader + k) * FID_OP_WORDS];
+        m[k] = conv_args(net, leader + k, first, batch);
+        m[k].partial = (float *)partial_ws;
+        m[k].rev = net->alternate && op[W_SRC] >= 0 && !net->tdir[op[W_SRC]];
+        p[k] = net->tuned[leader + k][batch];
+        FID_TRY(set_alt_weights(ctx, net, leader + k, m[k], p[k]));
+    }
+    static const bool cold_tune = !getenv("FID_TUNE_HOT");
+    static const int tune_reps = getenv("FID_TUNE_REPS") ? std::max(2, atoi(getenv("FID_TUNE_REPS"))) : 5;
+    void *flush = nullptr;
+    constexpr size_t FLUSH_BYTES = 320ull << 20;
+    if (cold_tune) { FID_TRY(get_scratch(ctx, 4, FLUSH_BYTES, &flush)); net->tuned_now = true; }
+    hipEvent_t e0, e1;
+    FID_HIP(hipEventCreate(&e0));
+    FID_HIP(hipEventCreate(&e1));
+    auto timed = [&](int cb, float *us) -> int {
+        float tmin = 1e30f;
+        for (int rep = 0; rep < tune_reps; rep++) {
+            if (flush) {
+                FID_HIP(hipMemsetAsync(flush, rep & 1, FLUSH_BYTES, ctx->stream));
+                for (int k = 0; k < CHAIN_N; k++)
+                    if (m[k].in_bytes <= (128u << 20))
+                        hipLaunchKernelGGL(touch_kernel, dim3(ctx->num_cus * 4), dim3(256), 0, ctx->stream, (const uint4 *)m[k].in, (size_t)m[k].in_bytes / 16, (unsigned *)nullptr);
+            }
+            FID_HIP(hipEventRecord(e0, ctx->stream));
+            if (cb) FID_TRY(conv_chain_launch(ctx, m, cb));
+            else for (int k = 0; k < CHAIN_N; k++) FID_TRY(conv_launch(ctx, m[k], p[k]));
+            FID_HIP(hipEventRecord(e1, ctx->stream));
+            FID_HIP(hipEventSynchronize(e1));
+            float ms = 0;
+            FID_HIP(hipEventElapsedTime(&ms, e0, e1));
+            if (rep > 0) tmin = std::min(tmin, ms);
+        }
+        *us = tmin * 1e3f;
+        return FID_OK;
+    };
+    float t_single = 0.f, best = 1e30f;
+    int pick = 0;
+    int rc = timed(0, &t_single);
+    for (int cb : {32, 64, 96}) {
+        if (rc != FID_OK || !conv_chain_applicable(m, cb)) continue;
+        float t = 0.f;
+        rc = timed(cb, &t);
+        if (getenv("FID_TUNE_LOG")) fprintf(stderr, "[chain] ops %d..%d batch %d: one by one %.1f us, chained (cb %d) %.1f us\n", leader, leader + CHAIN_N - 1, batch, t_single, cb, t);
+        if (rc == FID_OK && t < t_single && t < best) { best = t; pick = cb; }
+    }
+    (void)hipEventDestroy(e0);
+    (void)hipEventDestroy(e1);
+    FID_TRY(rc);
+    net->chain_pick[leader][batch] = pick;
+    if (!net->plan_path.empty()) {
+        if (FILE *pf = fopen(net->plan_path.c_str(), "a")) {
+            char line[512];
+            plan_line(net, leader, batch, p[0], line, sizeof(line));
+            fputs(line, pf);
+            fclose(pf);
+        }
+    }
     return FID_OK;
 }
 
@@ -498,33 +610,25 @@
                 auto itc = net->tuned[cons].find(batch);
                 if (itc != net->tuned[cons].end() && itc->second.gen == 12 && net->plan_ok[cons].count(batch)) break;
             }
+            if (op[W_CHAIN] != 0) {
+                ConvArgs m[CHAIN_N];
+                const int leader = op[W_CHAIN] > 0 ? oi : oi + op[W_CHAIN];
+                if (const int cb = chain_cb(net, leader, first, batch, m)) {
+                    if (leader != oi) break;
+                    FID_TRY(conv_chain_launch(ctx, m, cb));
+                    for (int k = 0; k < CHAIN_N; k++) net->tdir[net->ops[(size_t)(oi + k) * FID_OP_WORDS + W_DST]] = 0;
+                    break;
+                }
+            }
             const TensorView src = view(net, op[W_SRC], first);
-            ConvArgs a{}, af{};
+            ConvArgs a = conv_args(net, oi, first, batch), af{};
             bool has_sc = false;
-            a.in = src.ptr;
-            a.w = blob + op[W_WOFF];
-            a.bias = bias;
-            a.slope = slope;
-            a.out = dst.ptr;
             if (op[W_X_DST2] > 0) {
                 const TensorView d2 = view(net, op[W_X_DST2] - 1, first);
                 FID_REQUIRE(d2.H == dst.H && d2.W == dst.W && d2.Cp == dst.Cp && d2.dtype == dst.dtype && op[W_X_ACT2] == ACT_NONE &&
                             op[W_X_COUT1P] == dst.Cp, "op %d: bad fused shortcut record", oi);
                 a.out2 = d2.ptr;
             }
-            a.H = src.H; a.W = src.W; a.Cin_p = src.Cp;
-            a.Ho = dst.H; a.Wo = dst.W; a.Cout_p = dst.Cp;
-            a.w_rows = op[W_WROWS];
-            a.kh = op[W_KH]; a.kw = op[W_KW]; a.stride = op[W_STRIDE]; a.pad = op[W_PAD];
-            a.M = batch * dst.H * dst.W;
-            a.act = op[W_ACT]; a.flags = op[W_FLAGS]; a.nsig = op[W_NSIG];
-            if (dst.dtype == 1) a.flags |= CF_OUT_F32;
-            if (op[W_RES] >= 0) {
-                const TensorView r = view(net, op[W_RES], first);
-                a.res = r.ptr; a.res_H = r.H; a.res_W = r.W; a.res_Cp = r.Cp;
-            }
-            a.in_bytes = (unsigned)((size_t)batch * src.H * src.W * src.Cp * 2);
-            a.w_bytes = (unsigned)op[W_WBYTES];
             if (op[W_X_SRC2] > 0) {
                 const TensorView x2 = view(net, op[W_X_SRC2] - 1, first);
                 FID_REQUIRE(x2.dtype == 0 && op[W_X_T2] >= 1 && op[W_X_KW2] >= 1 && op[W_X_S2] >= 1 && op[W_X_DST2] == 0 &&
@@ -649,7 +753,8 @@
                 cache[batch] = plan;
                 net->plan_ok[oi].insert(batch);
                 drop_unused_alt_weights(ctx, net, oi);
-                if (!net->plan_path.empty()) {
+                const bool leads = op[W_CHAIN] > 0 && net->chains;
+                if (!net->plan_path.empty() && !leads) {
                     if (FILE *pf = fopen(net->plan_path.c_str(), "a")) {
                         char line[512];
                         plan_line(net, oi, batch, plan, line, sizeof(line));
@@ -668,6 +773,12 @@
             FID_TRY(launch_plan(plan));
             net->tdir[op[W_DST]] = (char)(a.rev && conv_walks_reverse(plan));
             if (op[W_X_DST2] > 0) net->tdir[op[W_X_DST2] - 1] = net->tdir[op[W_DST]];
+            if (op[W_CHAIN] == -(CHAIN_N - 1) && net->chains && net->autotune && partial_ws) {
+                const int leader = oi + op[W_CHAIN];
+                bool ready = !net->chain_pick[leader].count(batch);
+                for (int k = 0; k < CHAIN_N; k++) ready = ready && net->tuned[leader + k].count(batch) && net->plan_ok[leader + k].count(batch);
+                if (ready) FID_TRY(decide_chain(ctx, net, leader, first, batch, partial_ws));
+            }
             break;
         }
         case OP_STEMFUSED: {
@@ -956,6 +1067,16 @@
                     }
                 } else if (ok && op[W_X_W2OFF] != 0) {
                     ok = op[W_X_W2OFF] > oi + 1 && op[W_X_W2OFF] <= n_ops;
+                }
+                if (ok && op[W_CHAIN] != 0) {
+                    const int leader = op[W_CHAIN] > 0 ? oi : oi + op[W_CHAIN];
+                    ok = leader >= 0 && leader + CHAIN_N <= n_ops && net->ops[(size_t)leader * FID_OP_WORDS + W_CHAIN] == CHAIN_N &&
+                         net->ops[(size_t)leader * FID_OP_WORDS + W_TYPE] == OP_CONV &&
+                         (op[W_CHAIN] > 0 || op[W_CHAIN] > -CHAIN_N) && op[W_X_DST2] == 0 && op[W_X_SRC2] == 0 && op[W_X_W2OFF] == 0;
+                    for (int k = 1; ok && k < CHAIN_N; k++) {
+                        const int32_t *mk = &net->ops[(size_t)(leader + k) * FID_OP_WORDS];
+                        ok = mk[W_TYPE] == OP_CONV && mk[W_CHAIN] == -k;
+                    }
                 }
                 break;
             }
@@ -1032,6 +1153,8 @@
     if (const char *e = getenv("FID_GRAPH")) net->graphs = atoi(e);
     net->tuned.resize(n_ops);
     net->plan_ok.resize(n_ops);
+    net->chain_pick.resize(n_ops);
+    if (getenv("FID_NO_CHAIN")) net->chains = 0;
     net->tdir.assign(n_tensors, 0);
     if (getenv("FID_NO_REV")) net->alternate = 0;
     {
diff --git a/scrfd_arcface_facerecognition_amd/engine.py b/scrfd_arcface_facerecognition_amd/engine.py
--- a/scrfd_arcface_facerecognition_amd/engine.py
+++ b/scrfd_arcface_facerecognition_amd/engine.py
@@ -85,7 +85,7 @@
                     v = [int(x) for x in parts[4].split()]
                     oi = int(parts[2])
                     out.append(dict(op=oi, name=self.low.op_names[oi], batch=int(parts[3]), gen=v[0], bm=v[1], bn=v[2], bk=v[3],
-                                    ksplit=v[4], ns=v[5]))
+                                    ksplit=v[4], ns=v[5], chain=v[7] if len(v) > 7 else None))
             return out
         finally:
             os.unlink(path)
diff --git a/scrfd_arcface_facerecognition_amd/lower.py b/scrfd_arcface_facerecognition_amd/lower.py
--- a/scrfd_arcface_facerecognition_amd/lower.py
+++ b/scrfd_arcface_facerecognition_amd/lower.py
@@ -129,6 +129,31 @@
     if rup(81 * (cin_p * 2 + 16)) + rup(81 * (gp * 2 + 16)) + ((to * to + 15) // 16 * 16) * (gp * 2 + 16) > 160 * 1024:
         return None
     return d, m
+
+
+def _head_stages(net):
+    nd = net.nodes
+    heads = [i for i, n in enumerate(nd) if n.kind == "dethead"]
+    if len(heads) != 3 or heads[2] != len(nd) - 1 or heads[2] - heads[1] != heads[1] - heads[0]:
+        return None
+    L = heads[1] - heads[0]
+    start = heads[0] - L + 1
+    if start < 0:
+        return None
+    cols = [nd[start + l * L: start + (l + 1) * L] for l in range(3)]
+    names = {n.name for col in cols for n in col}
+    for col in cols:
+        for j, n in enumerate(col):
+            if (n.src in names) != (j > 0) or (j > 0 and n.src != col[j - 1].name):
+                return None
+            if j < L - 1 and not (n.kind == "conv" and n.groups == 1 and n.k == 3 and n.stride == 1 and n.pad == 1 and n.res is None
+                                  and not n.pre_avgpool and not n.res_up2):
+                return None
+            if j == L - 1 and n.k != 3:
+                return None
+    if any(getattr(x, "src", None) in names or getattr(x, "res", None) in names for x in nd[:start]):
+        return None
+    return start, [[cols[l][j].name for l in range(3)] for j in range(L)]
 
 
 def _latfpn(net, i, tensors, tid):
@@ -163,7 +188,14 @@
 
 
 def lower(net: Net, P: Dict[str, np.ndarray]) -> Lowered:
+    import copy
+    import os
     shp = infer_shapes(net)
+    stages = _head_stages(net)
+    if stages is not None:
+        by_name = {n.name: n for n in net.nodes}
+        net = copy.copy(net)
+        net.nodes = net.nodes[:stages[0]] + [by_name[x] for st in stages[1] for x in st]
     blob = _Blob()
     ops: List[List[int]] = []
     op_names: List[str] = []
@@ -662,6 +694,19 @@
         else:
             raise ValueError(f"cannot lower node {n}")
 
+    chain_end = list(range(len(ops)))
+    if stages is not None and not os.environ.get("FID_NO_CHAIN"):
+        for st in stages[1]:
+            if not all(x in op_names for x in st):
+                continue
+            i0 = op_names.index(st[0])
+            recs = ops[i0:i0 + 3]
+            plain = all(r[0] == OP_CONV and (r[4], r[5], r[6], r[7], r[18]) == (3, 3, 1, 1, 1) and r[3] < 0 and not any(r[19:32]) for r in recs)
+            if [op_names.index(x) for x in st] != [i0, i0 + 1, i0 + 2] or not plain or any(a[1] == b[2] for a in recs for b in recs):
+                continue
+            ops[i0][19], ops[i0 + 1][19], ops[i0 + 2][19] = 3, -1, -2
+            chain_end[i0] = chain_end[i0 + 1] = chain_end[i0 + 2] = i0 + 2
+
     n_t = len(tensors)
     base = list(range(n_t))
     for t in range(n_t):
@@ -671,7 +716,7 @@
     for oi, rec in enumerate(ops):
         for w in (1, 3):
             if rec[w] >= 0:
-                last_use[base[rec[w]]] = oi
+                last_use[base[rec[w]]] = chain_end[oi]
         if rec[0] == OP_CONV and rec[23] > 0:
             last_use[base[rec[23] - 1]] = oi
     keep = {tid[o] for o in net.outputs}
```

After: 18590 faces/s. 0.989x the previous value.
